# lauradarcy/gym-craftingworld

Hardware: AMD Instinct MI355X
Metric: env-steps/sec at 65536 envs, 1/2/4/8 MI355X; bit-exact vs CPU ref (higher is better)
Workload: dtype u8

## Files before the change

### gym_craftingworld_amd/_lib.py

```python
import ctypes as C
import os

_HERE = os.path.dirname(os.path.abspath(__file__))
LIB_PATH = os.path.join(_HERE, 'libcraftingworld.so')


def lib_path():
    return os.environ.get('CW_LIB_PATH') or LIB_PATH

CW_ABI_VERSION = 5
CW_MT_N = 624
CW_MAX_TASKS = 16
CW_MAX_MENUS = 256

CW_OK, CW_ERR_INVALID, CW_ERR_HIP, CW_ERR_STATE = 0, -1, -2, -3
CW_OBS_STATE, CW_OBS_PIXELS_FULL, CW_OBS_PIXELS_DIRTY = 0, 1, 2
CW_ACT_I32, CW_ACT_I64, CW_ACT_U8 = 0, 1, 2
CW_RASTER_RAY, CW_RASTER_ALT = 0, 1


class cw_task_menu(C.Structure):
    _fields_ = [('n_selected', C.c_int32), ('number_of_tasks', C.c_int32), ('stacking', C.c_int32),
                ('reward_subset', C.c_int32), ('selected_bits', C.c_int32 * CW_MAX_TASKS)]


class cw_config(C.Structure):
    _fields_ = [('abi_version', C.c_int32), ('num_envs', C.c_int32), ('size', C.c_int32),
                ('max_steps', C.c_int32), ('n_task_list', C.c_int32), ('fixed_init_state', C.c_int32),
                ('obs_mode', C.c_int32), ('auto_reset', C.c_int32), ('keep_terminal_obs', C.c_int32),
                ('raster', C.c_int32), ('host_outputs', C.c_int32), ('n_menus', C.c_int32),
                ('menus', C.POINTER(cw_task_menu)), ('env_menu', C.POINTER(C.c_uint8))]


class cw_buffer_table(C.Structure):
    _fields_ = [('obs', C.c_void_p), ('desired_goal', C.c_void_p), ('init_obs', C.c_void_p), ('terminal_obs', C.c_void_p),
                ('reward', C.c_void_p), ('done', C.c_void_p), ('achieved', C.c_void_p),
                ('desired', C.c_void_p), ('episode_length', C.c_void_p), ('episode_return', C.c_void_p), ('hdr', C.c_void_p),
                ('slot_pos', C.c_void_p), ('counters', C.c_void_p), ('frame_bytes', C.c_size_t),
                ('host_actions', C.c_void_p), ('host_onehot', C.c_void_p)]


class cw_state_view(C.Structure):
    _fields_ = [('grid', C.c_void_p), ('init_grid', C.c_void_p), ('goal_grid', C.c_void_p),
                ('agent_rc', C.c_void_p), ('init_agent_rc', C.c_void_p), ('goal_agent_rc', C.c_void_p),
                ('hold', C.c_void_p), ('achieved', C.c_void_p), ('desired', C.c_void_p),
                ('step_num', C.c_void_p), ('ep_no', C.c_void_p)]


class cw_profile(C.Structure):
    _fields_ = [('steps', C.c_int32), ('ms_step_kernel', C.c_float), ('ms_reset_kernel', C.c_float),
                ('ms_render_kernel', C.c_float), ('ms_render_kernel_max', C.c_float), ('ms_render_kernel_min', C.c_float),
                ('ms_render_kernel_median', C.c_float)]


class cw_tuner_state(C.Structure):
    _fields_ = [('period16', C.c_int32), ('period16_head', C.c_int32), ('period16_busy', C.c_int32), ('lookahead', C.c_int32), ('resident', C.c_int32),
                ('guard_slowdowns', C.c_int32)]


_VP = C.c_void_p
ABI = {
    'cw_create': (C.c_int, [C.POINTER(cw_config), C.c_int, C.POINTER(_VP)]),
    'cw_destroy': (C.c_int, [_VP]),
    'cw_seed_mt': (C.c_int, [_VP, _VP, _VP]),
    'cw_seed_int': (C.c_int, [_VP, _VP]),
    'cw_get_mt': (C.c_int, [_VP, _VP, _VP]),
    'cw_generate_fixed_states': (C.c_int, [_VP, _VP]),
    'cw_get_fixed_states': (C.c_int, [_VP, _VP]),
    'cw_reset': (C.c_int, [_VP, _VP]),
    'cw_reset_masked': (C.c_int, [_VP, _VP, _VP]),
    'cw_imagine_masked': (C.c_int, [_VP, _VP, _VP, C.c_int32, _VP, _VP, _VP]),
    'cw_sample_state_masked': (C.c_int, [_VP, _VP, C.c_int32, _VP, _VP]),
    'cw_step': (C.c_int, [_VP, _VP, C.c_int, _VP]),
    'cw_step_many': (C.c_int, [_VP, _VP, C.c_int, C.c_int32, _VP]),
    'cw_rollout': (C.c_int, [_VP, _VP, C.c_int32, _VP, _VP, _VP]),
    'cw_render': (C.c_int, [_VP, _VP, _VP]),
    'cw_render_onehot': (C.c_int, [_VP, _VP, C.c_int32, _VP, _VP]),
    'cw_export_grid': (C.c_int, [_VP, _VP, _VP]),
    'cw_export_onehot': (C.c_int, [_VP, _VP, _VP]),
    'cw_export_onehot_of': (C.c_int, [_VP, C.c_int, _VP, _VP]),
    'cw_get_state': (C.c_int, [_VP, C.POINTER(cw_state_view)]),
    'cw_set_state': (C.c_int, [_VP, C.POINTER(cw_state_view)]),
    'cw_checkpoint_bytes': (C.c_size_t, [_VP]),
    'cw_checkpoint_save': (C.c_int, [_VP, _VP, C.c_size_t]),
    'cw_checkpoint_load': (C.c_int, [_VP, _VP, C.c_size_t]),
    'cw_profile_begin': (C.c_int, [_VP, C.c_int]),
    'cw_profile_end': (C.c_int, [_VP, C.POINTER(cw_profile)]),
    'cw_tuner': (C.c_int, [_VP, C.POINTER(cw_tuner_state)]),
    'cw_step_resident': (C.c_int, [_VP, C.c_int32, C.c_int32]),
    'cw_resident_stop': (C.c_int, [_VP]),
    'cw_render_kernel_name': (C.c_char_p, [_VP]),
    'cw_buffers': (C.c_int, [_VP, C.POINTER(cw_buffer_table)]),
    'cw_synchronize': (C.c_int, [_VP, _VP]),
    'cw_num_envs': (C.c_int, [_VP]),
    'cw_abi_version': (C.c_int, []),
    'cw_last_error': (C.c_char_p, []),
}
class cwh_guard(C.Structure):
    _fields_ = [('rate', C.c_double), ('rate_top', C.c_double), ('ms_sum', C.c_double), ('prev_mean', C.c_double), ('ref_ms', C.c_double),
                ('ref_prev', C.c_double), ('ms_n', C.c_int32), ('late', C.c_int32), ('good', C.c_int32), ('slowdowns', C.c_int32),
                ('probes', C.c_int32), ('probe_need', C.c_int32), ('recover_need', C.c_int32), ('probing', C.c_int32), ('recovering', C.c_int32)]


class cwh_tuning(C.Structure):
    _fields_ = [(f, C.c_int32) for f in ('render_chunk_rounds', 'step_envs_per_wave', 'gather', 'gather_max_size', 'small_frame_bytes',
                                         'small_blocks_per_cu', 'small_launch_mb', 'reset_blocks_per_cu', 'guard', 'verbose', 'lookahead',
                                         'la_period', 'rollout_segment', 'pad')] + \
              [(f, C.c_double) for f in ('head_notch', 'busy_notch', 'period_ns', 'rate_tbs')]


cwh_lookup = C.CFUNCTYPE(_VP, _VP, C.c_char_p)

CWH_GUARD_NONE, CWH_GUARD_SLOWDOWN, CWH_GUARD_TRIAL_UP, CWH_GUARD_TRIAL_KEPT, CWH_GUARD_TRIAL_UNDONE = range(5)
CWH_CKPT_SECTIONS = 22

HOST_HELPERS = {
    'cwh_mt_from_numpy': (C.c_int, [_VP, C.c_int]),
    'cwh_mt_to_numpy': (None, [_VP, C.c_int, _VP]),
    'cwh_mt_init_genrand': (None, [_VP, C.c_uint32]),
    'cwh_mt_untwist': (None, [_VP]),
    'cwh_mt_rewind': (None, [_VP, C.POINTER(C.c_int32), C.c_uint32]),
    'cwh_dlpack_make': (_VP, [_VP, C.c_int, C.c_int, C.c_int, C.c_int, C.POINTER(C.c_int64)]),
    'cwh_slots_to_grid': (None, [_VP, C.c_uint32, C.c_int, _VP]),
    'cwh_ckpt_section_bytes': (C.c_int, [C.c_int64, C.c_int32, C.c_int32, C.POINTER(C.c_size_t), C.POINTER(C.c_uint64)]),
    'cwh_guard_init': (None, [C.POINTER(cwh_guard), C.c_double]),
    'cwh_guard_step': (C.c_int, [C.POINTER(cwh_guard), C.c_double, C.c_double]),
    'cwh_sweep_periods': (None, [C.c_double, C.c_int32, C.c_double, C.c_double, C.POINTER(C.c_int32), C.POINTER(C.c_int32), C.POINTER(C.c_int32)]),
    'cwh_guard_scheduled_ms': (C.c_double, [C.c_double, C.c_int32, C.c_int32, C.c_double]),
    'cwh_la_adapt': (C.c_int32, [C.c_int32, C.c_int32, C.c_uint64, C.POINTER(C.c_int32)]),
    'cwh_read_tuning': (None, [cwh_lookup, _VP, C.POINTER(cwh_tuning)]),
}


def bind_host_helpers(lib):
    for name, (res, args) in HOST_HELPERS.items():
        fn = getattr(lib, name)
        fn.restype = res
        fn.argtypes = args
    return lib

_libs = {}
_lib = None


class CraftingWorldError(RuntimeError):
    pass


def load():
    global _lib
    path = lib_path()
    if path in _libs:
        _lib = _libs[path]
        return _lib
    if not os.path.exists(path):
        raise CraftingWorldError(
            'HIP extension %s is missing; build it (python -c "import __graft_entry__ as g; g.build()"). '
            'There is no CPU fallback.' % path)
    try:
        import torch
    except ImportError:
        pass
    lib = C.CDLL(path)
    for table in (ABI, HOST_HELPERS):
        for name, (res, args) in table.items():
            fn = getattr(lib, name)
            fn.restype = res
            fn.argtypes = args
    if lib.cw_abi_version() != CW_ABI_VERSION:
        raise CraftingWorldError('%s ABI %d != binding %d' % (os.path.basename(path), lib.cw_abi_version(), CW_ABI_VERSION))
    _libs[path] = _lib = lib
    return lib


def check(rc, what, lib=None):
    if rc == CW_OK:
        return
    msg = ((lib or _lib or load()).cw_last_error() or b'').decode(errors='replace')
    if rc == CW_ERR_INVALID:
        raise ValueError('%s: %s' % (what, msg))
    raise CraftingWorldError('%s failed (%d): %s' % (what, rc, msg))
```

### gym_craftingworld_amd/csrc/cw_engine.cpp

```cpp
#include <hip/hip_runtime.h>

#include <cstdarg>
#include <climits>
#include <cstdio>
#include <cstdlib>
#include <cstring>
#include <new>
#include <algorithm>
#include <vector>

#include "../../include/craftingworld.h"
#include "cw_layout.h"
#include "cw_host.h"

extern "C" {
hipError_t cwk_launch_step(const CwParams *P, const CwTuning *T, const void *actions, int act_dtype, int obs_mode, int auto_reset, hipStream_t st,
                           hipEvent_t *ev);
hipError_t cwk_launch_refill(const CwParams *P, const CwTuning *T, int all_envs, hipStream_t st);
hipError_t cwk_launch_reset_all(const CwParams *P, const CwTuning *T, int obs_mode, hipStream_t st);
hipError_t cwk_launch_reset_masked(const CwParams *P, const CwTuning *T, const uint8_t *mask, int obs_mode, hipStream_t st);
hipError_t cwk_launch_imagine_masked(const CwParams *P, const CwTuning *T, const uint8_t *mask, const uint16_t *desired, int commit, int obs_mode,
                                     uint8_t *out_frames, uint8_t *out_onehot, hipStream_t st);
hipError_t cwk_launch_sample_state_masked(const CwParams *P, const CwTuning *T, const uint8_t *mask, int pooled, uint16_t *out_cells, hipStream_t st);
hipError_t cwk_launch_pool(const CwParams *P, const CwTuning *T, hipStream_t st);
hipError_t cwk_launch_seed(const CwParams *P, const uint32_t *seeds_dev, hipStream_t st);
hipError_t cwk_launch_resident(const CwParams *P, CwResident *R, uint32_t seq0, int paint_dirty, unsigned long long idle_ticks,
                               unsigned long long life_ticks, hipStream_t st);
hipError_t cwk_launch_render_onehot(const CwParams *P, const uint8_t *onehot, int n_states, uint16_t *out, hipStream_t st);
hipError_t cwk_launch_render_restore(const CwParams *P, const CwTuning *T, hipStream_t st);
hipError_t cwk_launch_rollout(const CwParams *P, const uint8_t *actions, int T, int32_t *rewards, uint8_t *dones, hipStream_t st);
hipError_t cwk_launch_render_ext(const CwParams *P, const CwTuning *T, uint8_t *out, hipStream_t st);
hipError_t cwk_launch_sweep_calib(const CwParams *P, const CwTuning *T, hipStream_t st);
void cwk_sweep_shape(const CwParams *P, const CwTuning *T, int *n_chunks, int *waves, int *jobs_per_wave);
hipError_t cwk_launch_idle(hipStream_t st);
hipError_t cwk_launch_export(const CwParams *P, const CwTuning *T, uint8_t *out, int onehot, int which, hipStream_t st);
}

#include <time.h>

static thread_local char g_err[512] = "";

static int fail(int code, const char *fmt, ...)
{
    va_list ap;
    va_start(ap, fmt);
    vsnprintf(g_err, sizeof(g_err), fmt, ap);
    va_end(ap);
    return code;
}

#define HIP_TRY(expr)                                                                           \
    do {                                                                                        \
        hipError_t _e = (expr);                                                                 \
        if (_e != hipSuccess)                                                                   \
            return fail(CW_ERR_HIP, "%s failed: %s (%s:%d)", #expr, hipGetErrorString(_e), __FILE__, __LINE__); \
    } while (0)

struct DeviceGuard {
    int prev = -1;
    bool ok = true;
    explicit DeviceGuard(int dev)
    {
        if (hipGetDevice(&prev) != hipSuccess) prev = -1;
        if (prev != dev) ok = (hipSetDevice(dev) == hipSuccess);
    }
    ~DeviceGuard()
    {
        int cur = -1;
        if (prev >= 0 && hipGetDevice(&cur) == hipSuccess && cur != prev) (void)hipSetDevice(prev);
    }
};

struct cw_engine {
    int device = 0;
    int obs_mode = 0;
    int auto_reset = 1;
    bool has_reset = false;
    CwParams P{};
    CwTuning tune{};
    std::vector<void *> allocs;
    std::vector<void *> host_allocs;
    int32_t *host_actions = nullptr;
    std::vector<CwMenuDev> menus;
    uint32_t *seed_scratch = nullptr;
    int n = 0, S = 0, ncell = 0, K = 0;
    CwResident *res = nullptr;
    hipStream_t res_stream = nullptr;
    bool res_running = false;
    uint32_t res_seq = 0;
    hipEvent_t last_work = nullptr;
    bool last_work_set = false;
    unsigned long long res_ticks_per_us = 100;
    std::vector<hipEvent_t> prof_ev;
    bool la_refill_all = false;
    unsigned la_steps = 0;
    unsigned la_period = 16;
    unsigned la_period_max = 16;
    bool la_adaptive = true;
    int rollout_segment = -1;
    unsigned long long *la_feedback = nullptr;
    unsigned long long la_slow_seen = 0;
    int32_t la_quiet = 0;
    bool in_step_many = false;
    bool capturing_now = false;
    int sweep_waves = 1024;
    double sweep_jobs = 0, sweep_rate = 0, sweep_beside_ms = 0;
    bool guard_on = false;
    double head_notch = 0.4, busy_notch = 0.75, tune_period_ns = -1, tune_rate_tbs = -1;
    bool tune_guard = true, tune_lookahead = true, verbose = false;
    enum { GUARD_RING = 32 };
    struct GuardSample { hipEvent_t ev[6]; int period16; } guard_ring[GUARD_RING] = {};
    unsigned guard_head = 0, guard_tail = 0;
    unsigned guard_step = 0;
    cwh_guard guard{};
    int prof_cap = 0, prof_n = 0;
    hipStream_t aux = nullptr;
    hipStream_t work[4] = {nullptr, nullptr, nullptr, nullptr};
    int n_work = 0;
    bool work_overflow = false;
    bool captured = false;
};
static inline bool stream_capturing(hipStream_t st)
{
    hipStreamCaptureStatus cap = hipStreamCaptureStatusNone;
    return hipStreamIsCapturing(st, &cap) == hipSuccess && cap != hipStreamCaptureStatusNone;
}
static inline void note_work(cw_engine *e, hipStream_t st)
{
    for (int i = 0; i < e->n_work; i++) if (e->work[i] == st) return;
    if (e->n_work < 4) e->work[e->n_work++] = st; else e->work_overflow = true;
}
static hipError_t quiesce(cw_engine *e)
{
    bool all = e->work_overflow || e->captured;
    for (int i = 0; i < e->n_work && !all; i++)
        if (hipStreamSynchronize(e->work[i]) != hipSuccess) { (void)hipGetLastError(); all = true; }
    e->n_work = 0;
    e->work_overflow = false;
    if (all) return hipDeviceSynchronize();
    return e->aux ? hipStreamSynchronize(e->aux) : hipSuccess;
}
struct AuxDrain {
    cw_engine *e;
    explicit AuxDrain(cw_engine *e_) : e(e_) {}
    ~AuxDrain() { if (e && e->aux) (void)hipStreamSynchronize(e->aux); }
};
static inline hipError_t aux_copy(cw_engine *e, void *dst, const void *src, size_t bytes, hipMemcpyKind kind)
{
    return bytes ? hipMemcpyAsync(dst, src, bytes, kind, e->aux) : hipSuccess;
}
static int la_period_for(int max_steps) { const int p = max_steps / 4; return p < 8 ? 8 : p > 64 ? 64 : p; }
static void la_adapt(cw_engine *e)
{
    const unsigned long long slow = __atomic_load_n(e->la_feedback, __ATOMIC_RELAXED);
    const unsigned long long delta = slow >= e->la_slow_seen ? slow - e->la_slow_seen : 0;
    e->la_slow_seen = slow;
    e->la_period = (unsigned)cwh_la_adapt((int32_t)e->la_period, (int32_t)e->la_period_max, delta, &e->la_quiet);
}

static int resident_park(cw_engine *e)
{
    if (!e->res_running) return CW_OK;
    const unsigned long long low = __atomic_load_n(&e->res->bell, __ATOMIC_RELAXED) & 0xFFFFFFFFull;
    __atomic_store_n(&e->res->bell, low | (1ull << 32), __ATOMIC_RELEASE);
    HIP_TRY(hipStreamSynchronize(e->res_stream));
    e->res_running = false;
    __atomic_store_n(&e->res->bell, low, __ATOMIC_RELEASE);
    __atomic_store_n(&e->res->exited, 0u, __ATOMIC_RELEASE);
    return CW_OK;
}
#define PARK(e) do { if ((e)->res_running) { const int _rc = resident_park(e); if (_rc != CW_OK) return _rc; } } while (0)


template <typename T>
static int dev_alloc(cw_engine *e, T **out, size_t count)
{
    void *p = nullptr;
    size_t bytes = count * sizeof(T);
    if (bytes == 0) bytes = 16;
    HIP_TRY(hipMalloc(&p, bytes));
    HIP_TRY(hipMemset(p, 0, bytes));
    e->allocs.push_back(p);
    *out = (T *)p;
    return CW_OK;
}

template <typename T>
static int host_alloc(cw_engine *e, T **out, size_t count)
{
    void *p = nullptr, *d = nullptr;
    size_t bytes = count * sizeof(T);
    if (bytes == 0) bytes = 16;
    HIP_TRY(hipHostMalloc(&p, bytes, hipHostMallocCoherent));
    e->host_allocs.push_back(p);
    memset(p, 0, bytes);
    HIP_TRY(hipHostGetDevicePointer(&d, p, 0));
    if (d != p) return fail(CW_ERR_HIP, "cw_create: mapped host memory has a different device address (no unified addressing)");
    *out = (T *)p;
    return CW_OK;
}

static void prof_free(cw_engine *e)
{
    for (hipEvent_t ev : e->prof_ev) (void)hipEventDestroy(ev);
    e->prof_ev.clear();
    e->prof_cap = e->prof_n = 0;
}

static int timed_render_stats(cw_engine *e, double *median, double *p90, double *mean = nullptr)
{
    enum { LAUNCHES = 24, SKIP = 4 };
    hipEvent_t evs[2 * LAUNCHES] = {};
    bool ok = true;
    for (hipEvent_t &ev : evs) ok = ok && hipEventCreate(&ev) == hipSuccess;
    for (int rep = 0; rep < LAUNCHES && ok; rep++)
        ok = hipEventRecord(evs[2 * rep], e->aux) == hipSuccess && cwk_launch_sweep_calib(&e->P, &e->tune, e->aux) == hipSuccess &&
             hipEventRecord(evs[2 * rep + 1], e->aux) == hipSuccess && cwk_launch_idle(e->aux) == hipSuccess;
    ok = ok && hipStreamSynchronize(e->aux) == hipSuccess;
    float ms[LAUNCHES];
    for (int rep = 0; rep < LAUNCHES && ok; rep++) ok = hipEventElapsedTime(&ms[rep], evs[2 * rep], evs[2 * rep + 1]) == hipSuccess;
    for (hipEvent_t &ev : evs) if (ev) (void)hipEventDestroy(ev);
    if (!ok) return fail(CW_ERR_HIP, "cw_create: render calibration failed");
    std::sort(ms + SKIP, ms + LAUNCHES);
    const int n = LAUNCHES - SKIP;
    *median = ms[SKIP + n / 2];
    *p90 = ms[SKIP + (9 * n) / 10 - 1];
    if (mean) { double acc = 0; for (int i = SKIP; i < LAUNCHES; i++) acc += ms[i]; *mean = acc / n; }
    return CW_OK;
}

static double sweep_period_ns(const cw_engine *e, double tb_per_s) { return (double)e->sweep_waves * 4096.0 / (tb_per_s * 1e12) * 1e9; }
static void set_sweep_rate(cw_engine *e, double tb_per_s)
{
    cwh_sweep_periods(tb_per_s, e->sweep_waves, e->head_notch, e->busy_notch, &e->tune.period16, &e->tune.period16_head, &e->tune.period16_busy);
}

static int calibrate_sweep(cw_engine *e)
{
    CwTuning &tn = e->tune;
    int n_chunks = 1, jobs_per_wave = 1;
    cwk_sweep_shape(&e->P, &tn, &n_chunks, &e->sweep_waves, &jobs_per_wave);
    e->sweep_jobs = (double)n_chunks * jobs_per_wave;
    if (e->tune_period_ns >= 0) {
        const double ns = e->tune_period_ns;
        set_sweep_rate(e, ns > 0 ? (double)e->sweep_waves * 4096.0 / (ns * 1e-9) * 1e-12 : 0.0);
        if (ns > 0) tn.period16 = (int)(ns * 1.6 + 0.5);
        return CW_OK;
    }
    set_sweep_rate(e, 7.0);
    if (e->host_actions) { set_sweep_rate(e, 0); return CW_OK; }
    if (e->obs_mode != CW_OBS_PIXELS_FULL || (double)e->n * e->P.frame_bytes < (double)(64ll << 20)) return CW_OK;
    static const double rates[] = {7.7, 7.4, 7.2, 7.0, 6.8, 6.6, 0.0};
    char log[1024] = "";
    size_t len = 0;
    int rc = CW_OK;
    double best_p90 = 0, med = 0, p90 = 0, mean = 0;
    rc = timed_render_stats(e, &med, &p90);
    set_sweep_rate(e, 6.4);
    if (rc == CW_OK) rc = timed_render_stats(e, &med, &p90);
    e->sweep_beside_ms = med - e->sweep_jobs * sweep_period_ns(e, 6.4) * 1e-6;
    if (e->tune_rate_tbs >= 0) e->sweep_rate = e->tune_rate_tbs;
    for (size_t i = 0; i < sizeof(rates) / sizeof(rates[0]) && rc == CW_OK && e->tune_rate_tbs < 0; i++) {
        set_sweep_rate(e, rates[i]);
        rc = timed_render_stats(e, &med, &p90, &mean);
        if (len < sizeof(log) - 56) len += (size_t)snprintf(log + len, sizeof(log) - len, " %.1f TB/s (%.0f ns): %.4f/%.4f/%.4f |", rates[i], tn.period16 / 1.6, med, p90, mean);
        if (rc == CW_OK && (best_p90 == 0 || p90 < 0.995 * best_p90)) { best_p90 = p90; e->sweep_rate = rates[i]; }
    }
    set_sweep_rate(e, e->sweep_rate);
    cwh_guard_init(&e->guard, e->sweep_rate);
    e->guard_on = rc == CW_OK && e->sweep_rate > 0 && e->auto_reset && e->tune_guard;
    if (e->guard_on)
        for (auto &smp : e->guard_ring)
            for (hipEvent_t &ev : smp.ev)
                if (hipEventCreate(&ev) != hipSuccess) e->guard_on = false;
    if (e->verbose)
        fprintf(stderr, "[craftingworld] sweep clock, ms per sweep (median/90th percentile/mean of 20; 0.0 TB/s = unclocked):%s -> %s%.0f ns\n", log,
                tn.period16 ? "" : "unclocked, ", tn.period16 / 1.6);
    return rc;
}

enum { CW_GUARD_EVERY = 64 };
static hipEvent_t *sweep_guard_tick(cw_engine *e, hipStream_t st)
{
    if (++e->guard_step % CW_GUARD_EVERY) return nullptr;
    while (e->guard_tail != e->guard_head && hipEventQuery(e->guard_ring[e->guard_tail % cw_engine::GUARD_RING].ev[5]) == hipSuccess) {
        cw_engine::GuardSample &smp = e->guard_ring[e->guard_tail++ % cw_engine::GUARD_RING];
        float ms = 0.f;
        if (hipEventElapsedTime(&ms, smp.ev[4], smp.ev[5]) != hipSuccess || ms <= 0.f || smp.period16 != e->tune.period16) continue;
        const double scheduled = cwh_guard_scheduled_ms(e->sweep_jobs, e->tune.period16, e->tune.period16_busy, e->sweep_beside_ms);
        const double rate_before = e->guard.rate, prev_mean = e->guard.prev_mean;
        const int recovering = e->guard.recovering;
        const int action = cwh_guard_step(&e->guard, ms, scheduled);
        if (e->guard.rate != rate_before) set_sweep_rate(e, e->guard.rate);
        if (e->verbose && action != CWH_GUARD_NONE) {
            static const char *what[] = {"", "three samples in a row late: a notch down", "trying a notch up", "the trial pays: kept", "the trial does not pay: undone"};
            fprintf(stderr, "[craftingworld] sweep clock: %s%s -- %.4f ms against %.4f scheduled (mean at the rate left %.4f): %.1f -> %.1f TB/s (%.0f ns)\n", what[action],
                    recovering ? " (on the way back to the best rate known)" : "", ms, scheduled, prev_mean, rate_before, e->guard.rate, e->tune.period16 / 1.6);
        }
    }
    if (e->guard_head - e->guard_tail >= (unsigned)cw_engine::GUARD_RING) return nullptr;
    cw_engine::GuardSample &slot = e->guard_ring[e->guard_head++ % cw_engine::GUARD_RING];
    slot.period16 = e->tune.period16;
    return slot.ev;
}

static void read_tuning(cw_engine *e)
{
    CwTuning &tn = e->tune;
    cwh_tuning t{};
    t.render_chunk_rounds = tn.render_chunk_rounds;
    t.step_envs_per_wave = tn.step_envs_per_wave;
    t.gather = tn.gather;
    t.gather_max_size = tn.gather_max_size;
    t.small_frame_bytes = tn.small_frame_bytes;
    t.small_blocks_per_cu = tn.small_blocks_per_cu;
    t.small_launch_mb = (int32_t)(tn.small_launch_bytes >> 20);
    t.reset_blocks_per_cu = tn.reset_blocks_per_cu;
    t.guard = 1;
    t.verbose = 0;
    t.lookahead = 1;
    t.la_period = 0;
    t.rollout_segment = e->rollout_segment;
    t.head_notch = e->head_notch;
    t.busy_notch = e->busy_notch;
    t.period_ns = -1;
    t.rate_tbs = -1;
    cwh_read_tuning([](void *, const char *k) -> const char * { return getenv(k); }, nullptr, &t);
    tn.render_chunk_rounds = t.render_chunk_rounds;
    tn.step_envs_per_wave = t.step_envs_per_wave;
    tn.gather = t.gather;
    tn.gather_max_size = t.gather_max_size;
    tn.small_frame_bytes = t.small_frame_bytes;
    tn.small_blocks_per_cu = t.small_blocks_per_cu;
    tn.small_launch_bytes = (long long)t.small_launch_mb << 20;
    tn.reset_blocks_per_cu = t.reset_blocks_per_cu;
    e->head_notch = t.head_notch;
    e->busy_notch = t.busy_notch;
    e->tune_period_ns = t.period_ns;
    e->tune_rate_tbs = t.rate_tbs;
    e->tune_guard = t.guard != 0;
    e->verbose = t.verbose != 0;
    e->tune_lookahead = t.lookahead != 0;
    e->la_adaptive = t.la_period == 0;
    e->la_period = e->la_period_max = (unsigned)(t.la_period ? t.la_period : la_period_for(e->P.max_steps));
    e->rollout_segment = t.rollout_segment;
}

extern "C" {

const char *cw_last_error(void) { return g_err; }
int cw_abi_version(void) { return CW_ABI_VERSION; }
int cw_num_envs(const cw_engine *e) { return e ? e->n : 0; }

int cw_create(const cw_config *cfg, int device, cw_engine **out)
{
    if (!cfg || !out) return fail(CW_ERR_INVALID, "cw_create: null argument");
    *out = nullptr;
    if (cfg->abi_version != CW_ABI_VERSION)
        return fail(CW_ERR_INVALID, "cw_create: abi_version %d != %d", cfg->abi_version, CW_ABI_VERSION);
    if (cfg->num_envs < 1) return fail(CW_ERR_INVALID, "cw_create: num_envs must be >= 1");
    if (cfg->size < 4 || cfg->size > 255)
        return fail(CW_ERR_INVALID, "cw_create: size must be in 4..255 (square grids only; non-square is a reference defect)");
    if (cfg->max_steps < 1 || cfg->max_steps > 65535) return fail(CW_ERR_INVALID, "cw_create: max_steps must be in 1..65535");
    if (cfg->n_task_list < 9 || cfg->n_task_list > CW_MAX_TASKS)
        return fail(CW_ERR_INVALID, "cw_create: len(task_list) must be in 9..%d", CW_MAX_TASKS);
    if (cfg->fixed_init_state < 0 || cfg->fixed_init_state > 64)
        return fail(CW_ERR_INVALID, "cw_create: fixed_init_state must be in 0..64");
    if (cfg->obs_mode < CW_OBS_STATE || cfg->obs_mode > CW_OBS_PIXELS_DIRTY) return fail(CW_ERR_INVALID, "cw_create: bad obs_mode");
    if (cfg->raster != CW_RASTER_RAY && cfg->raster != CW_RASTER_ALT) return fail(CW_ERR_INVALID, "cw_create: bad raster");
    if (cfg->n_menus < 1 || cfg->n_menus > CW_MAX_MENUS || !cfg->menus) return fail(CW_ERR_INVALID, "cw_create: n_menus must be in 1..%d", CW_MAX_MENUS);
    if ((double)cfg->num_envs * 48.0 * cfg->size * cfg->size > 1.0e12)
        return fail(CW_ERR_INVALID, "cw_create: num_envs x frame size exceeds 1 TB");

    std::vector<CwMenuDev> menus(cfg->n_menus);
    for (int m = 0; m < cfg->n_menus; m++) {
        const cw_task_menu &src = cfg->menus[m];
        if (src.n_selected < 1 || src.n_selected > CW_MAX_TASKS)
            return fail(CW_ERR_INVALID, "cw_create: menu %d: len(selected_tasks) must be in 1..%d", m, CW_MAX_TASKS);
        if (src.number_of_tasks < 1) return fail(CW_ERR_INVALID, "cw_create: menu %d: number_of_tasks must be >= 1", m);
        CwMenuDev d{};
        d.n_selected = src.n_selected;
        d.number_of_tasks = src.number_of_tasks > src.n_selected ? src.n_selected : src.number_of_tasks;
        d.stacking = src.stacking ? 1 : 0;
        d.reward_subset = src.reward_subset ? 1 : 0;
        for (int i = 0; i < src.n_selected; i++) {
            if (src.selected_bits[i] < 0 || src.selected_bits[i] >= cfg->n_task_list)
                return fail(CW_ERR_INVALID, "cw_create: menu %d: selected task %d is not in task_list", m, i);
            d.sel_bits |= (uint64_t)src.selected_bits[i] << (4 * i);
        }
        menus[m] = d;
    }
    if (cfg->env_menu)
        for (int i = 0; i < cfg->num_envs; i++)
            if (cfg->env_menu[i] >= cfg->n_menus) return fail(CW_ERR_INVALID, "cw_create: env_menu[%d] out of range", i);

    int ndev = 0;
    HIP_TRY(hipGetDeviceCount(&ndev));
    if (device < 0 || device >= ndev) return fail(CW_ERR_INVALID, "cw_create: device %d not present (%d devices)", device, ndev);
    DeviceGuard guard(device);
    if (!guard.ok) return fail(CW_ERR_HIP, "cw_create: hipSetDevice(%d) failed", device);

    cw_engine *e = new (std::nothrow) cw_engine();
    if (!e) return fail(CW_ERR_INVALID, "cw_create: out of host memory");
    e->device = device;
    e->obs_mode = cfg->obs_mode;
    e->auto_reset = cfg->auto_reset ? 1 : 0;
    e->n = cfg->num_envs;
    e->S = cfg->size;
    e->ncell = cfg->size * cfg->size;
    e->K = cfg->fixed_init_state;
    e->menus = menus;
    CwParams &P = e->P;
    const size_t N = (size_t)e->n;
    P.n_envs = e->n;
    P.size = e->S;
    P.ncell = e->ncell;
    P.max_steps = cfg->max_steps;
    read_tuning(e);
    hipDeviceProp_t prop;
    if (hipGetDeviceProperties(&prop, device) == hipSuccess && prop.multiProcessorCount > 0) e->tune.n_cu = prop.multiProcessorCount;
    P.task_mask = (1u << cfg->n_task_list) - 1u;
    P.pool_k = e->K;
    P.div_magic = (uint32_t)((1ull << 32) / (uint64_t)e->S) + 1u;
    P.raster = cfg->raster;
    P.frame_bytes = cfg->raster == CW_RASTER_ALT ? 27u * (uint32_t)e->S * (uint32_t)(e->S + 1) : 48u * (uint32_t)e->ncell;

    int rc = CW_OK;
#define ALLOC(field, count)                                     \
    if (rc == CW_OK) rc = dev_alloc(e, &P.field, (count))
    ALLOC(hdr, N);
    ALLOC(pos, N);
    ALLOC(init_pos, N);
    ALLOC(init_agent, N);
    ALLOC(goal_pos, N);
    ALLOC(goal_codes, N);
    ALLOC(goal_agent, N);
    ALLOC(ep_no, N);
    ALLOC(mt, N * CW_MT_N);
    ALLOC(mt_idx, N);
    ALLOC(pool, N * (size_t)e->K * 9);
    if (rc == CW_OK) rc = dev_alloc(e, &e->seed_scratch, N);
#define ALLOC_OUT(field, count)                                 \
    if (rc == CW_OK) rc = cfg->host_outputs ? host_alloc(e, &P.field, (count)) : dev_alloc(e, &P.field, (count))
    ALLOC_OUT(reward, N);
    ALLOC_OUT(done, N);
    ALLOC_OUT(achieved_out, N);
    ALLOC_OUT(desired_out, N);
    ALLOC_OUT(episode_length, N);
    ALLOC_OUT(episode_return, N);
    ALLOC(counters, 8);
    if (rc == CW_OK) {
        int pr_least = 0, pr_greatest = 0;
        if (hipDeviceGetStreamPriorityRange(&pr_least, &pr_greatest) != hipSuccess) pr_least = pr_greatest = 0;
        if (hipStreamCreateWithPriority(&e->aux, hipStreamNonBlocking, pr_greatest) != hipSuccess &&
            hipStreamCreateWithFlags(&e->aux, hipStreamNonBlocking) != hipSuccess)
            rc = fail(CW_ERR_HIP, "cw_create: no private stream");
    }
    if (cfg->obs_mode != CW_OBS_STATE) {
        ALLOC_OUT(obs, N * P.frame_bytes);
        ALLOC_OUT(desired_img, N * P.frame_bytes);
        ALLOC_OUT(init_img, N * P.frame_bytes);
        if (cfg->keep_terminal_obs && cfg->auto_reset) ALLOC_OUT(terminal_img, N * P.frame_bytes);
    }
    if (cfg->host_outputs && rc == CW_OK) rc = host_alloc(e, &e->host_actions, N);
    P.lookahead = (cfg->auto_reset && !cfg->host_outputs && e->tune_lookahead) ? 1 : 0;
    ALLOC(nx_init_pos, P.lookahead ? N * CW_LA_DEPTH : 1);
    ALLOC(nx_goal_pos, P.lookahead ? N * CW_LA_DEPTH : 1);
    ALLOC(nx_misc, P.lookahead ? N * CW_LA_DEPTH : 1);
    ALLOC(nx_ctl, P.lookahead ? N : 1);
    if (rc == CW_OK && P.lookahead && e->la_adaptive) {
        void *fb = nullptr;
        if (hipHostMalloc(&fb, 64, hipHostMallocCoherent) == hipSuccess) {
            memset(fb, 0, 64);
            e->host_allocs.push_back(fb);
            e->la_feedback = P.la_feedback = (unsigned long long *)fb;
        }
    }
#undef ALLOC_OUT
#undef ALLOC
    CwMenuDev *dmenus = nullptr;
    if (rc == CW_OK) rc = dev_alloc(e, &dmenus, menus.size());
    if (rc == CW_OK && hipMemcpy(dmenus, menus.data(), menus.size() * sizeof(CwMenuDev), hipMemcpyHostToDevice) != hipSuccess)
        rc = fail(CW_ERR_HIP, "cw_create: menu upload failed");
    P.menus = dmenus;
    if (rc == CW_OK) {
        std::vector<uint32_t> h(N * 4, 0u);
        for (size_t i = 0; i < N; i++) {
            h[i * 4 + 0] = (uint32_t)(cfg->env_menu ? cfg->env_menu[i] : 0) << 24;
            h[i * 4 + 3] = CW_CODES_INITIAL;
        }
        if (hipMemcpy(P.hdr, h.data(), h.size() * 4, hipMemcpyHostToDevice) != hipSuccess)
            rc = fail(CW_ERR_HIP, "cw_create: header upload failed");
    }
    if (rc != CW_OK) {
        if (e->aux) (void)hipStreamDestroy(e->aux);
        for (void *p : e->allocs) (void)hipFree(p);
        for (void *p : e->host_allocs) (void)hipHostFree(p);
        delete e;
        return rc;
    }
    if (cfg->host_outputs && e->n == 1 && !e->auto_reset && e->obs_mode != CW_OBS_PIXELS_FULL) {
        void *p = nullptr;
        if (hipHostMalloc(&p, sizeof(CwResident), hipHostMallocCoherent) == hipSuccess &&
            hipStreamCreateWithFlags(&e->res_stream, hipStreamNonBlocking) == hipSuccess) {
            memset(p, 0, sizeof(CwResident));
            e->host_allocs.push_back(p);
            e->res = (CwResident *)p;
            if (host_alloc(e, &e->P.res_onehot, (size_t)e->ncell * 12) != CW_OK) e->P.res_onehot = nullptr;
            int khz = 0;
            if (hipDeviceGetAttribute(&khz, hipDeviceAttributeWallClockRate, device) == hipSuccess && khz >= 1000) e->res_ticks_per_us = (unsigned long long)khz / 1000ull;
            if (hipEventCreateWithFlags(&e->last_work, hipEventDisableTiming) != hipSuccess) {
                e->last_work = nullptr;
                e->res = nullptr;
            }
        } else {
            if (p) (void)hipHostFree(p);
            e->res_stream = nullptr;
        }
    }
    *out = e;
    std::vector<uint32_t> seeds(N);
    for (size_t i = 0; i < N; i++) seeds[i] = (uint32_t)i;
    rc = cw_seed_int(e, seeds.data());
    if (rc == CW_OK) rc = calibrate_sweep(e);
    if (rc != CW_OK) {
        cw_destroy(e);
        *out = nullptr;
    }
    return rc;
}

int cw_destroy(cw_engine *e)
{
    if (!e) return CW_OK;
    DeviceGuard guard(e->device);
    if (!guard.ok) return fail(CW_ERR_HIP, "hipSetDevice(%d) failed", e->device);
    PARK(e);
    (void)resident_park(e);
    (void)quiesce(e);
    prof_free(e);
    if (e->aux) (void)hipStreamDestroy(e->aux);
    if (e->res_stream) (void)hipStreamDestroy(e->res_stream);
    if (e->last_work) (void)hipEventDestroy(e->last_work);
    for (auto &smp : e->guard_ring) for (hipEvent_t ev : smp.ev) if (ev) (void)hipEventDestroy(ev);
    for (void *p : e->allocs) (void)hipFree(p);
    for (void *p : e->host_allocs) (void)hipHostFree(p);
    delete e;
    return CW_OK;
}

static hipError_t lookahead_drop(cw_engine *e)
{
    if (!e->P.lookahead) return hipSuccess;
    hipError_t rc = hipMemsetAsync(e->P.nx_misc, 0, (size_t)e->n * CW_LA_DEPTH * sizeof(uint4), e->aux);
    if (rc == hipSuccess) rc = hipMemsetAsync(e->P.nx_ctl, 0, (size_t)e->n * sizeof(uint32_t), e->aux);
    e->la_refill_all = true;
    return rc;
}

int cw_seed_mt(cw_engine *e, const uint32_t *keys, const int32_t *pos)
{
    if (!e || !keys || !pos) return fail(CW_ERR_INVALID, "cw_seed_mt: null argument");
    DeviceGuard guard(e->device);
    if (!guard.ok) return fail(CW_ERR_HIP, "hipSetDevice(%d) failed", e->device);
    PARK(e);
    const size_t N = (size_t)e->n;
    for (size_t i = 0; i < N; i++)
        if (pos[i] < 0 || pos[i] > CW_MT_N) return fail(CW_ERR_INVALID, "cw_seed_mt: pos[%zu]=%d outside 0..624", i, pos[i]);
    HIP_TRY(quiesce(e));
    AuxDrain drain(e);
    HIP_TRY(aux_copy(e, e->P.mt, keys, N * CW_MT_N * sizeof(uint32_t), hipMemcpyHostToDevice));
    HIP_TRY(aux_copy(e, e->P.mt_idx, pos, N * sizeof(int32_t), hipMemcpyHostToDevice));
    HIP_TRY(cwk_launch_seed(&e->P, nullptr, e->aux));
    HIP_TRY(lookahead_drop(e));
    HIP_TRY(hipStreamSynchronize(e->aux));
    return CW_OK;
}

int cw_seed_int(cw_engine *e, const uint32_t *seeds)
{
    if (!e || !seeds) return fail(CW_ERR_INVALID, "cw_seed_int: null argument");
    DeviceGuard guard(e->device);
    if (!guard.ok) return fail(CW_ERR_HIP, "hipSetDevice(%d) failed", e->device);
    PARK(e);
    HIP_TRY(quiesce(e));
    AuxDrain drain(e);
    HIP_TRY(aux_copy(e, e->seed_scratch, seeds, (size_t)e->n * sizeof(uint32_t), hipMemcpyHostToDevice));
    HIP_TRY(cwk_launch_seed(&e->P, e->seed_scratch, e->aux));
    HIP_TRY(lookahead_drop(e));
    HIP_TRY(hipStreamSynchronize(e->aux));
    return CW_OK;
}

int cw_get_mt(cw_engine *e, uint32_t *keys, int32_t *pos)
{
    if (!e || !keys || !pos) return fail(CW_ERR_INVALID, "cw_get_mt: null argument");
    DeviceGuard guard(e->device);
    if (!guard.ok) return fail(CW_ERR_HIP, "hipSetDevice(%d) failed", e->device);
    PARK(e);
    const size_t N = (size_t)e->n;
    std::vector<uint32_t> words(N * CW_MT_N);
    std::vector<uint32_t> misc(e->P.lookahead ? N * 4 * CW_LA_DEPTH : 0);
    HIP_TRY(quiesce(e));
    AuxDrain drain(e);
    HIP_TRY(aux_copy(e, words.data(), e->P.mt, words.size() * sizeof(uint32_t), hipMemcpyDeviceToHost));
    HIP_TRY(aux_copy(e, pos, e->P.mt_idx, N * sizeof(int32_t), hipMemcpyDeviceToHost));
    if (e->P.lookahead) HIP_TRY(aux_copy(e, misc.data(), e->P.nx_misc, N * 16 * CW_LA_DEPTH, hipMemcpyDeviceToHost));
    HIP_TRY(hipStreamSynchronize(e->aux));
    for (size_t i = 0; i < N; i++) cwh_mt_to_numpy(&words[i * CW_MT_N], pos[i], keys + i * CW_MT_N);
    if (e->P.lookahead) {
        for (size_t i = 0; i < N; i++) {
            uint32_t ahead = 0;
            for (size_t d = 0; d < CW_LA_DEPTH; d++)
                if (misc[(d * N + i) * 4 + 2] >> 31) ahead += misc[(d * N + i) * 4 + 3];
            if (ahead) cwh_mt_rewind(keys + i * CW_MT_N, &pos[i], ahead);
        }
    }
    for (size_t i = 0; i < N; i++)
        if (pos[i] == 0) { cwh_mt_untwist(keys + i * CW_MT_N); pos[i] = CW_MT_N; }
    return CW_OK;
}

int cw_generate_fixed_states(cw_engine *e, cw_stream_t stream)
{
    if (!e) return fail(CW_ERR_INVALID, "cw_generate_fixed_states: null engine");
    if (e->K == 0) return CW_OK;
    DeviceGuard guard(e->device);
// ... 19 lines not shown
    PARK(e);
    note_work(e, (hipStream_t)stream);
    HIP_TRY(cwk_launch_reset_all(&e->P, &e->tune, e->obs_mode, (hipStream_t)stream));
    if (e->P.lookahead) {
        HIP_TRY(cwk_launch_refill(&e->P, &e->tune, 1, (hipStream_t)stream));
        e->la_refill_all = false;
        e->la_steps = 0;
    }
    e->has_reset = true;
    if (e->res && hipEventRecord(e->last_work, (hipStream_t)stream) == hipSuccess) e->last_work_set = true;
    return CW_OK;
}

int cw_reset_masked(cw_engine *e, const uint8_t *mask, cw_stream_t stream)
{
    if (!e || !mask) return fail(CW_ERR_INVALID, "cw_reset_masked: null %s", !e ? "engine" : "mask");
    if (!e->has_reset) return fail(CW_ERR_STATE, "cw_reset_masked called before cw_reset");
    DeviceGuard guard(e->device);
    if (!guard.ok) return fail(CW_ERR_HIP, "hipSetDevice(%d) failed", e->device);
    PARK(e);
    if (stream_capturing((hipStream_t)stream)) e->captured = true; else note_work(e, (hipStream_t)stream);
    HIP_TRY(cwk_launch_reset_masked(&e->P, &e->tune, mask, e->obs_mode, (hipStream_t)stream));
    if (e->res && hipEventRecord(e->last_work, (hipStream_t)stream) == hipSuccess) e->last_work_set = true;
    return CW_OK;
}

static int rewind_streams(cw_engine *e, hipStream_t st, const char *who)
{
    if (!e->P.lookahead) return CW_OK;
    if (stream_capturing(st)) return fail(CW_ERR_STATE, "%s: an engine that keeps look-ahead records rewinds its streams through the host and cannot be captured", who);
    std::vector<uint32_t> keys((size_t)e->n * CW_MT_N);
    std::vector<int32_t> pos((size_t)e->n);
    int rc = cw_get_mt(e, keys.data(), pos.data());
    if (rc == CW_OK) rc = cw_seed_mt(e, keys.data(), pos.data());
    return rc;
}

int cw_imagine_masked(cw_engine *e, const uint8_t *mask, const uint16_t *desired, int32_t commit, uint8_t *out_frames, uint8_t *out_onehot,
                      cw_stream_t stream)
{
    if (!e) return fail(CW_ERR_INVALID, "cw_imagine_masked: null engine");
    if (!commit && !out_frames && !out_onehot) return fail(CW_ERR_INVALID, "cw_imagine_masked: commit == 0 and no output pointer: nothing to do");
    if (!e->has_reset) return fail(CW_ERR_STATE, "cw_imagine_masked called before cw_reset");
    DeviceGuard guard(e->device);
    if (!guard.ok) return fail(CW_ERR_HIP, "hipSetDevice(%d) failed", e->device);
    PARK(e);
    const int rc = rewind_streams(e, (hipStream_t)stream, "cw_imagine_masked");
    if (rc != CW_OK) return rc;
    if (stream_capturing((hipStream_t)stream)) e->captured = true; else note_work(e, (hipStream_t)stream);
    HIP_TRY(cwk_launch_imagine_masked(&e->P, &e->tune, mask, desired, commit != 0, e->obs_mode, out_frames, out_onehot, (hipStream_t)stream));
    if (e->res && hipEventRecord(e->last_work, (hipStream_t)stream) == hipSuccess) e->last_work_set = true;
    return CW_OK;
}

int cw_sample_state_masked(cw_engine *e, const uint8_t *mask, int32_t pooled, uint16_t *out_cells, cw_stream_t stream)
{
    if (!e || !out_cells) return fail(CW_ERR_INVALID, "cw_sample_state_masked: null %s", !e ? "engine" : "out_cells");
    if (pooled && e->K == 0) return fail(CW_ERR_INVALID, "cw_sample_state_masked: pooled with fixed_init_state == 0");
    if (!e->has_reset) return fail(CW_ERR_STATE, "cw_sample_state_masked called before cw_reset");
    DeviceGuard guard(e->device);
    if (!guard.ok) return fail(CW_ERR_HIP, "hipSetDevice(%d) failed", e->device);
    PARK(e);
    const int rc = rewind_streams(e, (hipStream_t)stream, "cw_sample_state_masked");
    if (rc != CW_OK) return rc;
    if (stream_capturing((hipStream_t)stream)) e->captured = true; else note_work(e, (hipStream_t)stream);
    HIP_TRY(cwk_launch_sample_state_masked(&e->P, &e->tune, mask, pooled != 0, out_cells, (hipStream_t)stream));
    if (e->res && hipEventRecord(e->last_work, (hipStream_t)stream) == hipSuccess) e->last_work_set = true;
    return CW_OK;
}

int cw_step(cw_engine *e, const void *actions, int action_dtype, cw_stream_t stream)
{
    if (!e || !actions) return fail(CW_ERR_INVALID, "cw_step: null argument");
    if (action_dtype < CW_ACT_I32 || action_dtype > CW_ACT_U8) return fail(CW_ERR_INVALID, "cw_step: bad action dtype %d", action_dtype);
    if (!e->has_reset) return fail(CW_ERR_STATE, "cw_step called before cw_reset");
    DeviceGuard guard(e->device);
    if (!guard.ok) return fail(CW_ERR_HIP, "hipSetDevice(%d) failed", e->device);
    PARK(e);
    const bool capturing = e->in_step_many ? e->capturing_now : stream_capturing((hipStream_t)stream);
    if (capturing) e->captured = true;
    else if (e->n_work != 1 || e->work[0] != (hipStream_t)stream) note_work(e, (hipStream_t)stream);
    hipEvent_t *ev = (e->prof_n < e->prof_cap) ? &e->prof_ev[(size_t)e->prof_n * 6] : nullptr;
    const bool profiled = ev != nullptr;
    if (e->guard_on && !ev && !capturing) ev = sweep_guard_tick(e, (hipStream_t)stream);
    if (capturing && e->P.lookahead && !e->la_refill_all && e->la_steps + 1 < e->la_period && !e->in_step_many) e->la_steps = e->la_period;
    if (e->P.lookahead && (e->la_refill_all || ++e->la_steps >= e->la_period)) {
        if (e->la_feedback && !capturing) la_adapt(e);
        HIP_TRY(cwk_launch_refill(&e->P, &e->tune, e->la_refill_all ? 1 : 0, (hipStream_t)stream));
        e->la_refill_all = false;
        e->la_steps = 0;
    }
    HIP_TRY(cwk_launch_step(&e->P, &e->tune, actions, action_dtype, e->obs_mode, e->auto_reset, (hipStream_t)stream, ev));
    if (profiled) e->prof_n++;
    if (e->res && hipEventRecord(e->last_work, (hipStream_t)stream) == hipSuccess) e->last_work_set = true;
    return CW_OK;
}

int cw_step_many(cw_engine *e, const void *actions, int action_dtype, int32_t n_steps, cw_stream_t stream)
{
    if (!e || !actions) return fail(CW_ERR_INVALID, "cw_step_many: null argument");
    if (n_steps < 1) return fail(CW_ERR_INVALID, "cw_step_many: n_steps must be >= 1");
    if (action_dtype < CW_ACT_I32 || action_dtype > CW_ACT_U8) return fail(CW_ERR_INVALID, "cw_step_many: bad action dtype %d", action_dtype);
    e->capturing_now = stream_capturing((hipStream_t)stream);
    if (e->P.lookahead && e->capturing_now) e->la_steps = e->la_period;
    const size_t row = (size_t)e->n * (action_dtype == CW_ACT_I32 ? 4 : action_dtype == CW_ACT_I64 ? 8 : 1);
    e->in_step_many = true;
    int rc = CW_OK;
    for (int32_t t = 0; t < n_steps && rc == CW_OK; t++) rc = cw_step(e, (const unsigned char *)actions + (size_t)t * row, action_dtype, stream);
    e->in_step_many = false;
    return rc;
}

int cw_step_resident(cw_engine *e, int32_t action, int32_t want_onehot)
{
    if (!e) return fail(CW_ERR_INVALID, "cw_step_resident: null engine");
    if (!e->res) return fail(CW_ERR_INVALID, "cw_step_resident needs num_envs == 1, host_outputs, auto_reset == 0 and obs_mode state or pixels_dirty");
    if (!e->has_reset) return fail(CW_ERR_STATE, "cw_step_resident called before cw_reset");
    if (action < 0 || action > 127) return fail(CW_ERR_INVALID, "cw_step_resident: action %d outside 0..127", action);
    if (want_onehot && !e->P.res_onehot) return fail(CW_ERR_INVALID, "cw_step_resident: no host one-hot buffer on this engine");
    CwResident *R = e->res;
    const uint32_t seq = (++e->res_seq) & 0xFFFFFFu;
    __atomic_store_n(&R->bell, (unsigned long long)((seq << 8) | (want_onehot ? 0x80u : 0u) | (uint32_t)action), __ATOMIC_RELEASE);
    struct timespec t0;
    clock_gettime(CLOCK_MONOTONIC, &t0);
    for (unsigned spins = 0;; spins++) {
        if (e->res_running && __atomic_load_n(&R->ack, __ATOMIC_ACQUIRE) == seq) return CW_OK;
        if (!e->res_running || __atomic_load_n(&R->exited, __ATOMIC_ACQUIRE) != 0) {
            DeviceGuard guard(e->device);
            if (!guard.ok) return fail(CW_ERR_HIP, "hipSetDevice(%d) failed", e->device);
            if (e->res_running) HIP_TRY(hipStreamSynchronize(e->res_stream));
            e->res_running = false;
            if (__atomic_load_n(&R->ack, __ATOMIC_ACQUIRE) == seq) {
                __atomic_store_n(&R->exited, 0u, __ATOMIC_RELEASE);
                return CW_OK;
            }
            if (e->last_work_set) { HIP_TRY(hipStreamWaitEvent(e->res_stream, e->last_work, 0)); e->last_work_set = false; }
            __atomic_store_n(&R->exited, 0u, __ATOMIC_RELEASE);
            __atomic_store_n(&R->ack, (seq - 1u) & 0xFFFFFFu, __ATOMIC_RELEASE);
            HIP_TRY(cwk_launch_resident(&e->P, R, (seq - 1u) & 0xFFFFFFu, e->obs_mode == CW_OBS_PIXELS_DIRTY ? 1 : 0,
                                        500ull * e->res_ticks_per_us , 200000ull * e->res_ticks_per_us , e->res_stream));
            e->res_running = true;
            continue;
        }
        __builtin_ia32_pause();
        if ((spins & 1023u) == 1023u) {
            struct timespec t1;
            clock_gettime(CLOCK_MONOTONIC, &t1);
            if ((t1.tv_sec - t0.tv_sec) + 1e-9 * (t1.tv_nsec - t0.tv_nsec) > 5.0) {
                const uint32_t acked = __atomic_load_n(&R->ack, __ATOMIC_ACQUIRE);
                __atomic_store_n(&R->bell, (1ull << 32) | ((unsigned long long)acked << 8), __ATOMIC_RELEASE);
                const hipError_t he = hipStreamSynchronize(e->res_stream);
                e->res_running = false;
                const uint32_t now_acked = __atomic_load_n(&R->ack, __ATOMIC_ACQUIRE);
                __atomic_store_n(&R->bell, (unsigned long long)now_acked << 8, __ATOMIC_RELEASE);
                __atomic_store_n(&R->exited, 0u, __ATOMIC_RELEASE);
                e->res_seq = now_acked;
                if (he == hipSuccess && now_acked == seq) return CW_OK;
                return fail(CW_ERR_HIP, "cw_step_resident: no answer from the resident kernel within 5 s (request withdrawn, kernel parked: the step was not taken)");
            }
        }
    }
}

int cw_resident_stop(cw_engine *e)
{
    if (!e) return fail(CW_ERR_INVALID, "cw_resident_stop: null engine");
    DeviceGuard guard(e->device);
// ... 64 lines not shown

int cw_export_onehot(cw_engine *e, uint8_t *out, cw_stream_t stream)
{
    if (!e || !out) return fail(CW_ERR_INVALID, "cw_export_onehot: null argument");
    DeviceGuard guard(e->device);
    if (!guard.ok) return fail(CW_ERR_HIP, "hipSetDevice(%d) failed", e->device);
    PARK(e);
    note_work(e, (hipStream_t)stream);
    HIP_TRY(cwk_launch_export(&e->P, &e->tune, out, 1, 0, (hipStream_t)stream));
    return CW_OK;
}

int cw_export_onehot_of(cw_engine *e, int which, uint8_t *out, cw_stream_t stream)
{
    if (!e || !out) return fail(CW_ERR_INVALID, "cw_export_onehot_of: null argument");
    if (which < CW_STATE_CURRENT || which > CW_STATE_INIT) return fail(CW_ERR_INVALID, "cw_export_onehot_of: which must be CW_STATE_*");
    if (!e->has_reset) return fail(CW_ERR_STATE, "cw_export_onehot_of called before cw_reset");
    DeviceGuard guard(e->device);
    if (!guard.ok) return fail(CW_ERR_HIP, "hipSetDevice(%d) failed", e->device);
    PARK(e);
    note_work(e, (hipStream_t)stream);
    HIP_TRY(cwk_launch_export(&e->P, &e->tune, out, 1, which, (hipStream_t)stream));
    return CW_OK;
}

int cw_profile_begin(cw_engine *e, int max_steps)
{
    if (!e || max_steps < 1 || max_steps > 100000) return fail(CW_ERR_INVALID, "cw_profile_begin: bad argument");
    DeviceGuard guard(e->device);
    if (!guard.ok) return fail(CW_ERR_HIP, "hipSetDevice(%d) failed", e->device);
    PARK(e);
    prof_free(e);
    e->prof_ev.resize((size_t)max_steps * 6);
    for (auto &ev : e->prof_ev) HIP_TRY(hipEventCreate(&ev));
    e->prof_cap = max_steps;
    return CW_OK;
}

int cw_profile_end(cw_engine *e, cw_profile *out)
{
    if (!e || !out) return fail(CW_ERR_INVALID, "cw_profile_end: null argument");
    DeviceGuard guard(e->device);
    if (!guard.ok) return fail(CW_ERR_HIP, "hipSetDevice(%d) failed", e->device);
    PARK(e);
    memset(out, 0, sizeof(*out));
    const int n = e->prof_n;
    if (n > 0) {
        const bool side_recorded = e->obs_mode != CW_OBS_PIXELS_FULL;
        for (int k = 0; k < 6; k++)
            if (side_recorded || k >= 4) HIP_TRY(hipEventSynchronize(e->prof_ev[(size_t)(n - 1) * 6 + k]));
        double acc[3] = {0, 0, 0};
        float rmax = 0.f, rmin = 1e30f;
        std::vector<float> render_ms;
        render_ms.reserve((size_t)n);
        for (int i = 0; i < n; i++)
            for (int k = 0; k < 3; k++) {
                if (k != 2 && !side_recorded) continue;
                float ms = 0.f;
                HIP_TRY(hipEventElapsedTime(&ms, e->prof_ev[(size_t)i * 6 + 2 * k], e->prof_ev[(size_t)i * 6 + 2 * k + 1]));
                acc[k] += ms;
                if (k == 2) { rmax = ms > rmax ? ms : rmax; rmin = ms < rmin ? ms : rmin; render_ms.push_back(ms); }
            }
        out->steps = n;
        out->ms_step_kernel = (float)(acc[0] / n);
        out->ms_reset_kernel = (float)(acc[1] / n);
        out->ms_render_kernel = (float)(acc[2] / n);
        out->ms_render_kernel_max = rmax;
        out->ms_render_kernel_min = rmin;
        std::sort(render_ms.begin(), render_ms.end());
        out->ms_render_kernel_median = render_ms.empty() ? 0.f : render_ms[render_ms.size() / 2];
    }
    prof_free(e);
    return CW_OK;
}

const char *cw_render_kernel_name(const cw_engine *e)
{
    if (!e || e->obs_mode == CW_OBS_STATE) return "";
    if (e->obs_mode == CW_OBS_PIXELS_DIRTY) return e->auto_reset ? "cw_step_fused_kernel" : "cw_step_kernel";
    if (e->tune.gather && e->P.raster == CW_RASTER_RAY && e->S <= e->tune.gather_max_size) return "cw_render_gather_kernel";
    return "cw_render_pieces_kernel";
}

int cw_tuner(const cw_engine *e, cw_tuner_state *out)
{
    if (!e || !out) return fail(CW_ERR_INVALID, "cw_tuner: null argument");
    out->period16 = e->tune.period16;
    out->period16_head = e->tune.period16_head;
    out->period16_busy = e->tune.period16_busy;
    out->lookahead = e->P.lookahead;
    out->resident = e->res ? 1 : 0;
    out->guard_slowdowns = e->guard_on ? e->guard.slowdowns : -1;
    return CW_OK;
}

int cw_buffers(cw_engine *e, cw_buffer_table *out)
{
    if (!e || !out) return fail(CW_ERR_INVALID, "cw_buffers: null argument");
    const CwParams &P = e->P;
    out->obs = P.obs;
    out->desired_goal = P.desired_img;
    out->init_obs = P.init_img;
    out->terminal_obs = P.terminal_img;
    out->reward = P.reward;
    out->done = P.done;
    out->achieved = P.achieved_out;
    out->desired = P.desired_out;
    out->episode_length = P.episode_length;
    out->episode_return = P.episode_return;
    out->hdr = (uint8_t *)P.hdr;
    out->slot_pos = (uint16_t *)P.pos;
    out->counters = (uint64_t *)P.counters;
    out->frame_bytes = P.frame_bytes;
    out->host_actions = e->host_actions;
    out->host_onehot = P.res_onehot;
    return CW_OK;
}

int cw_synchronize(cw_engine *e, cw_stream_t stream)
{
    if (!e) return fail(CW_ERR_INVALID, "cw_synchronize: null engine");
    DeviceGuard guard(e->device);
    if (!guard.ok) return fail(CW_ERR_HIP, "hipSetDevice(%d) failed", e->device);
    PARK(e);
    HIP_TRY(hipStreamSynchronize((hipStream_t)stream));
    for (int i = 0; i < e->n_work; i++)
        if (e->work[i] == (hipStream_t)stream) { e->work[i] = e->work[--e->n_work]; break; }
    return CW_OK;
}

int cw_get_fixed_states(cw_engine *e, uint16_t *out)
{
    if (!e || !out) return fail(CW_ERR_INVALID, "cw_get_fixed_states: null argument");
    if (e->K == 0) return fail(CW_ERR_INVALID, "cw_get_fixed_states: the engine was created with fixed_init_state = 0");
    DeviceGuard guard(e->device);
    if (!guard.ok) return fail(CW_ERR_HIP, "hipSetDevice(%d) failed", e->device);
    PARK(e);
    HIP_TRY(quiesce(e));
    AuxDrain drain(e);
    HIP_TRY(aux_copy(e, out, e->P.pool, (size_t)e->n * e->K * 9 * sizeof(uint16_t), hipMemcpyDeviceToHost));
    HIP_TRY(hipStreamSynchronize(e->aux));
    return CW_OK;
}

int cw_get_state(cw_engine *e, cw_state_view *v)
{
    if (!e || !v) return fail(CW_ERR_INVALID, "cw_get_state: null argument");
    DeviceGuard guard(e->device);
    if (!guard.ok) return fail(CW_ERR_HIP, "hipSetDevice(%d) failed", e->device);
    PARK(e);
    const size_t N = (size_t)e->n;
    const int S = e->S, nc = e->ncell;
    std::vector<uint32_t> hdr(N * 4), goal_codes(N);
    std::vector<uint16_t> pos(N * 8), ipos(N * 8), gpos(N * 8), iagent(N), gagent(N);
    std::vector<int32_t> epno(N);
    HIP_TRY(quiesce(e));
    AuxDrain drain(e);
    HIP_TRY(aux_copy(e, hdr.data(), e->P.hdr, N * 16, hipMemcpyDeviceToHost));
    HIP_TRY(aux_copy(e, pos.data(), e->P.pos, N * 16, hipMemcpyDeviceToHost));
    HIP_TRY(aux_copy(e, ipos.data(), e->P.init_pos, N * 16, hipMemcpyDeviceToHost));
    HIP_TRY(aux_copy(e, gpos.data(), e->P.goal_pos, N * 16, hipMemcpyDeviceToHost));
    HIP_TRY(aux_copy(e, goal_codes.data(), e->P.goal_codes, N * 4, hipMemcpyDeviceToHost));
    HIP_TRY(aux_copy(e, iagent.data(), e->P.init_agent, N * 2, hipMemcpyDeviceToHost));
    HIP_TRY(aux_copy(e, gagent.data(), e->P.goal_agent, N * 2, hipMemcpyDeviceToHost));
    HIP_TRY(aux_copy(e, epno.data(), e->P.ep_no, N * 4, hipMemcpyDeviceToHost));
    HIP_TRY(hipStreamSynchronize(e->aux));
    for (size_t i = 0; i < N; i++) {
        const uint32_t *h = &hdr[i * 4];
        if (v->grid) cwh_slots_to_grid(&pos[i * 8], h[3], nc, v->grid + i * nc);
        if (v->init_grid) cwh_slots_to_grid(&ipos[i * 8], CW_CODES_INITIAL, nc, v->init_grid + i * nc);
        if (v->goal_grid) cwh_slots_to_grid(&gpos[i * 8], goal_codes[i], nc, v->goal_grid + i * nc);
        if (v->agent_rc) { v->agent_rc[i * 2] = h[0] & 0xFF; v->agent_rc[i * 2 + 1] = (h[0] >> 8) & 0xFF; }
        if (v->init_agent_rc) { v->init_agent_rc[i * 2] = (uint8_t)(iagent[i] / S); v->init_agent_rc[i * 2 + 1] = (uint8_t)(iagent[i] % S); }
        if (v->goal_agent_rc) { v->goal_agent_rc[i * 2] = (uint8_t)(gagent[i] / S); v->goal_agent_rc[i * 2 + 1] = (uint8_t)(gagent[i] % S); }
        if (v->hold) v->hold[i] = (h[0] >> 16) & 0xFF;
// ... 275 lines not shown
```

### gym_craftingworld_amd/csrc/cw_host.cpp

```cpp
#include "cw_host.h"

#include <algorithm>
#include <cerrno>
#include <climits>
#include <cmath>
#include <cstdlib>
#include <cstring>

static inline uint32_t mt_twist(uint32_t cur, uint32_t nxt, uint32_t far)
{
    const uint32_t y = (cur & 0x80000000u) | (nxt & 0x7fffffffu);
    return far ^ (y >> 1) ^ ((y & 1u) ? 0x9908b0dfu : 0u);
}

extern "C" {

int cwh_mt_from_numpy(uint32_t *s, int pos)
{
    if (pos < 0) pos = 0;
    if (pos > CWH_MT_N) pos = CWH_MT_N;
    for (int k = 0; k < pos; k++)
        s[k] = mt_twist(s[k], s[(k + 1) % CWH_MT_N], s[(k + 397) % CWH_MT_N]);
    return pos % CWH_MT_N;
}
// ... 25 lines not shown
    memset(prev, 0, sizeof(prev));
    for (int k = CWH_MT_N - 1; k >= 0; k--) {
        uint32_t t = key[k] ^ (k == CWH_MT_N - 1 ? key[396] : k >= CWH_MT_N - 397 ? key[k - (CWH_MT_N - 397)] : prev[k + 397]);
        const uint32_t odd = t >> 31;
        if (odd) t ^= 0x9908b0dfu;
        const uint32_t y = (t << 1) | odd;
        prev[k] |= y & 0x80000000u;
        if (k == CWH_MT_N - 1) key[0] = (key[0] & 0x80000000u) | (y & 0x7fffffffu);
        else prev[k + 1] |= y & 0x7fffffffu;
    }
    uint32_t t = prev[CWH_MT_N - 1] ^ prev[396];
    const uint32_t odd = t >> 31;
    if (odd) t ^= 0x9908b0dfu;
    prev[0] |= ((t << 1) | odd) & 0x7fffffffu;
    memcpy(key, prev, sizeof(prev));
}
void cwh_mt_rewind(uint32_t *key, int32_t *pos, uint32_t n)
{
    while (n > 0) {
        if ((uint32_t)*pos >= n) { *pos -= (int32_t)n; n = 0; }
        else { n -= (uint32_t)*pos; cwh_mt_untwist(key); *pos = CWH_MT_N; }
    }
}

struct CwDLDevice { int32_t device_type, device_id; };
struct CwDLDataType { uint8_t code, bits; uint16_t lanes; };
struct CwDLTensor { void *data; CwDLDevice device; int32_t ndim; CwDLDataType dtype; int64_t *shape, *strides; uint64_t byte_offset; };
struct CwDLManagedTensor { CwDLTensor dl_tensor; void *manager_ctx; void (*deleter)(CwDLManagedTensor *); };

static void cw_dl_deleter(CwDLManagedTensor *m)
{
    if (!m) return;
    free(m->dl_tensor.shape);
    free(m);
}

void *cwh_dlpack_make(void *data, int device_id, int code, int bits, int ndim, const int64_t *shape)
{
    CwDLManagedTensor *m = (CwDLManagedTensor *)calloc(1, sizeof(CwDLManagedTensor));
    int64_t *shp = (int64_t *)malloc(sizeof(int64_t) * (size_t)(ndim > 0 ? ndim : 1));
    if (!m || !shp) { free(m); free(shp); return nullptr; }
    for (int i = 0; i < ndim; i++) shp[i] = shape[i];
    m->dl_tensor.data = data;
    m->dl_tensor.device = CwDLDevice{10, device_id};
    m->dl_tensor.ndim = ndim;
    m->dl_tensor.dtype = CwDLDataType{(uint8_t)code, (uint8_t)bits, 1};
    m->dl_tensor.shape = shp;
    m->dl_tensor.strides = nullptr;
    m->dl_tensor.byte_offset = 0;
    m->deleter = cw_dl_deleter;
    return m;
}

void cwh_mt_init_genrand(uint32_t *s, uint32_t seed)
{
    s[0] = seed;
    for (int i = 1; i < CWH_MT_N; i++) s[i] = 1812433253u * (s[i - 1] ^ (s[i - 1] >> 30)) + (uint32_t)i;
}

}


extern "C" {

void cwh_slots_to_grid(const uint16_t *pos, uint32_t codes, int ncell, uint8_t *grid)
{
    memset(grid, 0, (size_t)ncell);
    for (int k = 0; k < 8; k++)
        if (pos[k] < (uint32_t)ncell) grid[pos[k]] = (uint8_t)((codes >> (4 * k)) & 15u);
}

int cwh_ckpt_section_bytes(int64_t n, int32_t k, int32_t la_depth, size_t *sizes, uint64_t *total)
{
    const size_t N = n > 0 ? (size_t)n : 0, K = k > 0 ? (size_t)k : 0, D = la_depth > 0 ? (size_t)la_depth : 0, la = D ? 1 : 0;
    const size_t sz[CWH_CKPT_SECTIONS] = {N * 16, N * 16, N * 16, N * 16, N * 4, N * 2, N * 2, N * 4, N * CWH_MT_N * 4, N * 4, N * K * 9 * 2,
                                          N * 4, N, N * 2, N * 2, N * 4, N * 4, 5 * 8,
                                          D * N * 16, D * N * 16, D * N * 16, la * N * 4};
    uint64_t sum = 0;
    for (int i = 0; i < CWH_CKPT_SECTIONS; i++) { if (sizes) sizes[i] = sz[i]; sum += sz[i]; }
    if (total) *total = sum;
    return CWH_CKPT_SECTIONS;
}

static double period_ns(int32_t sweep_waves, double tb_per_s) { return (double)sweep_waves * 4096.0 / (tb_per_s * 1e12) * 1e9; }
void cwh_sweep_periods(double rate, int32_t sweep_waves, double head_notch, double busy_notch, int32_t *period16, int32_t *period16_head, int32_t *period16_busy)
{
    const double head = rate - head_notch > CWH_GUARD_RATE_FLOOR ? rate - head_notch : CWH_GUARD_RATE_FLOOR;
    const double busy = rate - busy_notch > CWH_GUARD_RATE_FLOOR ? rate - busy_notch : CWH_GUARD_RATE_FLOOR;
    *period16 = rate > 0 ? (int32_t)(period_ns(sweep_waves, rate) * 1.6 + 0.5) : 0;
    *period16_head = rate > 0 ? (int32_t)(period_ns(sweep_waves, head) * 1.6 + 0.5) : 0;
    *period16_busy = rate > 0 ? (int32_t)(period_ns(sweep_waves, busy) * 1.6 + 0.5) : 0;
}
double cwh_guard_scheduled_ms(double sweep_jobs, int32_t period16, int32_t period16_busy, double beside_ms)
{
    return (sweep_jobs * (period16 / 1.6) + CWH_HEAD_JOBS * ((period16_busy - period16) / 1.6)) * 1e-6 + beside_ms;
}

static void guard_set_rate(cwh_guard *g, double rate)
{
    g->rate = rate;
    g->ms_sum = 0;
    g->ms_n = 0;
    g->good = g->late = 0;
    g->ref_ms = 0;
}
void cwh_guard_init(cwh_guard *g, double rate)
{
    memset(g, 0, sizeof(*g));
    g->rate = g->rate_top = rate;
    g->probe_need = CWH_GUARD_RECOVER;
    g->recover_need = CWH_GUARD_RECOVER;
}
int cwh_guard_step(cwh_guard *g, double ms, double scheduled)
{
    const double ref = std::max(scheduled, g->probing ? g->prev_mean : g->ref_ms);
    const bool late = ms > (g->probing ? 1.15 : 1.06) * ref;
    g->late = late ? g->late + 1 : 0;
    g->good = late ? std::max(0, g->good - 8) : g->good + 1;
    if (g->ms_n >= 128) { g->ms_sum *= 0.5; g->ms_n /= 2; }
    g->ms_sum += ms;
    g->ms_n++;
    const bool verdict_due = g->probing && g->ms_n >= CWH_GUARD_PROBE_SAMPLES;
    const double mean = g->ms_sum / g->ms_n;
    if (g->probing && (g->late >= 3 || (verdict_due && mean >= 0.998 * g->prev_mean))) {
        const double ref_prev = g->ref_prev;
        guard_set_rate(g, g->rate - CWH_GUARD_NOTCH);
        g->ref_ms = ref_prev;
        int32_t &need = g->recovering ? g->recover_need : g->probe_need;
        need = std::min(2 * need, (int32_t)CWH_GUARD_NEED_MAX);
        g->probing = g->recovering = 0;
        return CWH_GUARD_TRIAL_UNDONE;
    }
    if (verdict_due) {
        if (g->recovering) g->recover_need = CWH_GUARD_RECOVER;
        else { g->rate_top = g->rate; g->probe_need = CWH_GUARD_RECOVER / 4; }
        g->ref_ms = mean;
        g->probing = g->recovering = 0;
        return CWH_GUARD_TRIAL_KEPT;
    }
    if (!g->probing && g->late >= 3 && g->rate > CWH_GUARD_RATE_FLOOR + 0.1) {
        guard_set_rate(g, g->rate - CWH_GUARD_NOTCH);
        g->slowdowns++;
        return CWH_GUARD_SLOWDOWN;
    }
    if (!g->probing && g->ms_n >= CWH_GUARD_PROBE_SAMPLES && g->rate + 0.05 < CWH_GUARD_RATE_CEILING &&
        g->good >= (g->rate + 0.1 < g->rate_top ? g->recover_need : g->probe_need)) {
        g->recovering = g->rate + 0.1 < g->rate_top;
        g->prev_mean = mean;
        g->ref_prev = g->ref_ms;
        guard_set_rate(g, std::min(g->rate + CWH_GUARD_NOTCH, CWH_GUARD_RATE_CEILING));
        g->probing = 1;
        if (!g->recovering) g->probes++;
        return CWH_GUARD_TRIAL_UP;
    }
    return CWH_GUARD_NONE;
}

int32_t cwh_la_adapt(int32_t period, int32_t period_max, uint64_t slow_delta, int32_t *quiet)
{
    if (slow_delta * 8ull > (uint64_t)period) {
        *quiet = 0;
        if (period > CWH_LA_PERIOD_MIN) period = period / 2 < CWH_LA_PERIOD_MIN ? CWH_LA_PERIOD_MIN : period / 2;
    } else if (slow_delta * 32ull <= (uint64_t)period && ++*quiet >= CWH_LA_QUIET) {
        *quiet = 0;
        if (period < period_max) period = period * 2 > period_max ? period_max : period * 2;
    }
    return period;
}

}

static bool tail_is_blank(const char *end)
{
    while (*end == ' ' || (*end >= '\t' && *end <= '\r')) end++;
    return *end == '\0';
}
static void tune_int(cwh_lookup lookup, void *ctx, const char *name, int32_t *field, long lo, long hi)
{
    const char *s = lookup(ctx, name);
    if (!s) return;
    char *end = nullptr;
    errno = 0;
    const long v = strtol(s, &end, 10);
    if (end == s || errno == ERANGE || !tail_is_blank(end) || v < lo || v > hi) return;
    *field = (int32_t)v;
}
static void tune_real(cwh_lookup lookup, void *ctx, const char *name, double *field, double lo)
{
    const char *s = lookup(ctx, name);
    if (!s) return;
    char *end = nullptr;
    errno = 0;
    const double v = strtod(s, &end);
    if (end == s || errno == ERANGE || !tail_is_blank(end) || !std::isfinite(v) || v < lo) return;
    *field = v;
}

extern "C" void cwh_read_tuning(cwh_lookup lookup, void *ctx, cwh_tuning *t)
{
    tune_int(lookup, ctx, "CW_TUNE_RENDER_CHUNK_ROUNDS", &t->render_chunk_rounds, 0, INT32_MAX);
    int32_t epw = t->step_envs_per_wave;
    tune_int(lookup, ctx, "CW_TUNE_STEP_ENVS_PER_WAVE", &epw, 8, 64);
    if (epw == 8 || epw == 16 || epw == 32 || epw == 64) t->step_envs_per_wave = epw;
    tune_int(lookup, ctx, "CW_TUNE_GATHER", &t->gather, INT32_MIN, INT32_MAX);
    tune_int(lookup, ctx, "CW_TUNE_GATHER_MAX_SIZE", &t->gather_max_size, 0, 9);
    tune_int(lookup, ctx, "CW_TUNE_SMALL_FRAME_BYTES", &t->small_frame_bytes, 0, INT32_MAX);
    tune_int(lookup, ctx, "CW_TUNE_SMALL_BLOCKS", &t->small_blocks_per_cu, 1, 8);
    tune_int(lookup, ctx, "CW_TUNE_SMALL_LAUNCH_MB", &t->small_launch_mb, 0, INT32_MAX);
    tune_int(lookup, ctx, "CW_TUNE_RESET_BLOCKS", &t->reset_blocks_per_cu, 1, 16);
    tune_real(lookup, ctx, "CW_TUNE_HEAD_NOTCH", &t->head_notch, 0);
    tune_real(lookup, ctx, "CW_TUNE_BUSY_NOTCH", &t->busy_notch, 0);
    tune_real(lookup, ctx, "CW_TUNE_PERIOD_NS", &t->period_ns, 0);
    tune_real(lookup, ctx, "CW_TUNE_RATE_TBS", &t->rate_tbs, 0);
    tune_int(lookup, ctx, "CW_TUNE_GUARD", &t->guard, INT32_MIN, INT32_MAX);
    t->guard = t->guard != 0;
    if (lookup(ctx, "CW_TUNE_VERBOSE")) t->verbose = 1;
    tune_int(lookup, ctx, "CW_TUNE_LOOKAHEAD", &t->lookahead, INT32_MIN, INT32_MAX);
    t->lookahead = t->lookahead != 0;
    tune_int(lookup, ctx, "CW_TUNE_LA_PERIOD", &t->la_period, 1, INT32_MAX);
    tune_int(lookup, ctx, "CW_TUNE_ROLLOUT_SEGMENT", &t->rollout_segment, -1, INT32_MAX);
}
```

### gym_craftingworld_amd/csrc/cw_host.h

```cpp
#pragma once
#include <stddef.h>
#include <stdint.h>

#define CWH_MT_N 624

#ifdef __cplusplus
extern "C" {
#endif

int cwh_mt_from_numpy(uint32_t *s, int pos);
void cwh_mt_to_numpy(const uint32_t *s, int idx, uint32_t *key);
void cwh_mt_untwist(uint32_t *key);
void cwh_mt_rewind(uint32_t *key, int32_t *pos, uint32_t n);
void cwh_mt_init_genrand(uint32_t *s, uint32_t seed);

void *cwh_dlpack_make(void *data, int device_id, int code, int bits, int ndim, const int64_t *shape);

void cwh_slots_to_grid(const uint16_t *pos, uint32_t codes, int ncell, uint8_t *grid);

#define CWH_CKPT_SECTIONS 22
int cwh_ckpt_section_bytes(int64_t n, int32_t k, int32_t la_depth, size_t *sizes, uint64_t *total);

typedef struct cwh_guard {
    double rate;
    double rate_top;
    double ms_sum;
    double prev_mean;
    double ref_ms;
    double ref_prev;
    int32_t ms_n;
    int32_t late;
    int32_t good;
    int32_t slowdowns;
    int32_t probes;
    int32_t probe_need;
    int32_t recover_need;
    int32_t probing;
    int32_t recovering;
} cwh_guard;

enum { CWH_GUARD_NONE = 0, CWH_GUARD_SLOWDOWN = 1, CWH_GUARD_TRIAL_UP = 2, CWH_GUARD_TRIAL_KEPT = 3, CWH_GUARD_TRIAL_UNDONE = 4 };
#define CWH_GUARD_RECOVER 64
#define CWH_GUARD_PROBE_SAMPLES 32
#define CWH_GUARD_NEED_MAX 2048
#define CWH_GUARD_RATE_FLOOR 5.0
#define CWH_GUARD_RATE_CEILING 7.7
#define CWH_GUARD_NOTCH 0.2

void cwh_guard_init(cwh_guard *g, double rate);
int cwh_guard_step(cwh_guard *g, double ms, double scheduled_ms);
#define CWH_HEAD_JOBS 64
void cwh_sweep_periods(double rate, int32_t sweep_waves, double head_notch, double busy_notch, int32_t *period16, int32_t *period16_head, int32_t *period16_busy);
double cwh_guard_scheduled_ms(double sweep_jobs, int32_t period16, int32_t period16_busy, double beside_ms);

#define CWH_LA_PERIOD_MIN 8
#define CWH_LA_QUIET 8
int32_t cwh_la_adapt(int32_t period, int32_t period_max, uint64_t slow_delta, int32_t *quiet);

typedef struct cwh_tuning {
    int32_t render_chunk_rounds;
    int32_t step_envs_per_wave;
    int32_t gather;
    int32_t gather_max_size;
    int32_t small_frame_bytes;
    int32_t small_blocks_per_cu;
    int32_t small_launch_mb;
    int32_t reset_blocks_per_cu;
    int32_t guard;
    int32_t verbose;
    int32_t lookahead;
    int32_t la_period;
    int32_t rollout_segment;
    int32_t pad;
    double head_notch;
    double busy_notch;
    double period_ns;
    double rate_tbs;
} cwh_tuning;
typedef const char *(*cwh_lookup)(void *ctx, const char *name);
void cwh_read_tuning(cwh_lookup lookup, void *ctx, cwh_tuning *t);

#ifdef __cplusplus
}
#endif
```

### gym_craftingworld_amd/csrc/cw_kernels.hip

```cpp
#include <hip/hip_runtime.h>
#include <stdint.h>

#include "cw_layout.h"
#include "cw_mt.h"

#define CW_WAVE 64
#define CW_BALLOT(p) __builtin_amdgcn_ballot_w64(p)
#define CW_ALT_FRAME_PACE 2

#ifdef CW_TRACE
__device__ unsigned long long cw_trace_buf[1024 * 8];
#define CW_STAMP(env, k) do { if (lane == 0) { cw_trace_buf[((env) & 1023) * 8 + (k)] = wall_clock64(); \
                                               if ((k) == 0 || (k) == 5) cw_trace_buf[((env) & 1023) * 8 + 6 + ((k) ? 1 : 0)] = clock64(); } } while (0)
extern "C" hipError_t cwk_trace_read(unsigned long long *dst) { return hipMemcpyFromSymbol(dst, HIP_SYMBOL(cw_trace_buf), sizeof(cw_trace_buf)); }
#else
#define CW_STAMP(env, k) do { } while (0)
#endif

enum { EMPTY = 0, STICKS = 1, AXE = 2, HAMMER = 3, ROCK = 4, TREE = 5, BREAD = 6, HOUSE = 7, WHEAT = 8 };
enum { T_MAKEBREAD = 0, T_EATBREAD = 1, T_BUILDHOUSE = 2, T_CHOPTREE = 3, T_CHOPROCK = 4,
       T_GOTOHOUSE = 5, T_MOVEAXE = 6, T_MOVEHAMMER = 7, T_MOVESTICKS = 8 };

typedef uint32_t u32x3 __attribute__((ext_vector_type(3)));
typedef u32x3 u32x3_a4 __attribute__((aligned(4)));

__device__ __forceinline__ void unpack_pos(const uint4 &v, uint32_t sp[8])
{
    sp[0] = v.x & 0xFFFFu; sp[1] = v.x >> 16;
    sp[2] = v.y & 0xFFFFu; sp[3] = v.y >> 16;
    sp[4] = v.z & 0xFFFFu; sp[5] = v.z >> 16;
    sp[6] = v.w & 0xFFFFu; sp[7] = v.w >> 16;
}
__device__ __forceinline__ uint4 pack_pos(const uint32_t sp[8])
{
    return make_uint4(sp[0] | (sp[1] << 16), sp[2] | (sp[3] << 16), sp[4] | (sp[5] << 16), sp[6] | (sp[7] << 16));
}
__device__ __forceinline__ int slot_at(const uint32_t sp[8], uint32_t cell)
{
    int idx = -1;
#pragma unroll
    for (int k = 0; k < 8; k++) idx = (sp[k] == cell) ? k : idx;
    return idx;
}
__device__ __forceinline__ uint32_t code_of(uint32_t codes, int idx)
{
    return idx < 0 ? 0u : ((codes >> (4 * idx)) & 15u);
}
__device__ __forceinline__ uint32_t rgb_of_code(uint32_t code)
{
    uint32_t c = 0;
    c = code == 1 ? (110u | (69u << 8) | (39u << 16)) : c;
    c = code == 2 ? (255u | (105u << 8) | (180u << 16)) : c;
    c = code == 3 ? (100u | (100u << 8) | (200u << 16)) : c;
    c = code == 4 ? (100u | (100u << 8) | (100u << 16)) : c;
    c = code == 5 ? (0u | (128u << 8) | (0u << 16)) : c;
    c = code == 6 ? (205u | (133u << 8) | (63u << 16)) : c;
    c = code == 7 ? (197u | (91u << 8) | (97u << 16)) : c;
    c = code == 8 ? (240u | (230u << 8) | (140u << 16)) : c;
    return c;
}

__device__ __forceinline__ u32x3 cell_row_dwords(uint32_t rgb)
{
    u32x3 d;
    d.x = rgb | (rgb << 24);
    d.y = (rgb >> 8) | (rgb << 16);
    d.z = (rgb >> 16) | (rgb << 8);
    return d;
}
__device__ __forceinline__ u32x3 overlay_dwords(u32x3 d, uint32_t o)
{
    d.x = (d.x & 0x00FFFFFFu) | (o << 24);
    d.y = (o >> 8) | (o << 16);
    d.z = (d.z & 0xFFFFFF00u) | (o >> 16);
    return d;
}
__device__ __forceinline__ u32x3 onehot_dwords(uint32_t bits)
{
    u32x3 d;
    d.x = (bits & 1u) | ((bits >> 1 & 1u) << 8) | ((bits >> 2 & 1u) << 16) | ((bits >> 3 & 1u) << 24);
    d.y = (bits >> 4 & 1u) | ((bits >> 5 & 1u) << 8) | ((bits >> 6 & 1u) << 16) | ((bits >> 7 & 1u) << 24);
    d.z = (bits >> 8 & 1u) | ((bits >> 9 & 1u) << 8) | ((bits >> 10 & 1u) << 16) | ((bits >> 11 & 1u) << 24);
    return d;
}

__device__ __forceinline__ void paint_cell(uint8_t *frame, int S, uint32_t cell, uint32_t code,
                                           bool agent_here, uint32_t hold, uint32_t div_magic, bool mark_rows_only = false)
{
    const uint32_t r = __umulhi(cell, div_magic);
// ... 587 lines not shown
#pragma unroll
    for (int k = 0; k < 8; k++) {
        fp[k] = __builtin_amdgcn_readlane(v_fp, k);
        goal_codes |= __builtin_amdgcn_readlane(v_fc, k) << (4 * k);
    }
    goal_pos = pack_pos(fp);
}

template <typename MenuFn>
__device__ __forceinline__ CwResetOut reset_env_wave(const CwParams &P, int env, MenuFn menu_fn, uint32_t *lds_mt, int lane)
{
    CW_STAMP(env, 0);
    const CwMtWave::Pending pend = CwMtWave::load_issue(P.mt + (size_t)env * CW_MT_WORDS, P.mt_idx + env, lane);
    const uint32_t menu_id = menu_fn();
    const CwMenuDev M = P.menus[menu_id];
    CwMtWave mt;
    mt.load_commit(lds_mt, pend, lane);
    CW_STAMP(env, 1);

    const uint32_t desired = draw_tasks_wave(mt, M);

    CW_STAMP(env, 2);
    const uint32_t v_tok = place_env_wave(P, env, mt, P.pool_k != 0, lane);
    const uint32_t init_agent = __builtin_amdgcn_readlane(v_tok, 8);
    uint32_t v_fp = lane < 8 ? v_tok : (uint32_t)CW_POS_GONE;
    uint32_t v_fc = lane < 8 ? (uint32_t)lane + 1u : 0u;
    uint32_t ip[8];
#pragma unroll
    for (int k = 0; k < 8; k++) ip[k] = __builtin_amdgcn_readlane(v_tok, k);
    const uint4 init_packed = pack_pos(ip);
    CW_STAMP(env, 3);

    const uint32_t agent = imagine_env_wave(P, mt, v_fp, v_fc, init_agent, init_agent, desired);

    CW_STAMP(env, 4);
    const uint32_t draws = mt.draws();
    mt.store(P.mt + (size_t)env * CW_MT_WORDS, P.mt_idx + env, lane);
    CW_STAMP(env, 5);
    CwResetOut r;
    r.init_pos = init_packed;
    r.init_agent = init_agent;
    pack_goal_wave(v_fp, v_fc, r.goal_pos, r.goal_codes);
    r.goal_agent = agent;
    r.desired = desired;
    r.subset = M.reward_subset ? 1u : 0u;
    r.draws = draws;
    return r;
}

__device__ __forceinline__ uint4 reset_header(const CwParams &P, const CwResetOut &r, uint32_t menu_id)
{
    const uint32_t ar = __umulhi(r.init_agent, P.div_magic);
    const uint32_t ac = r.init_agent - ar * P.size;
    uint4 h;
    h.x = ar | (ac << 8) | (menu_id << 24);
    h.y = r.desired << 16;
    h.z = (CW_FLAG_RESET | (r.subset ? CW_FLAG_SUBSET : 0u)) << 16;
    h.w = CW_CODES_INITIAL;
    return h;
}
__device__ __forceinline__ void store_episode_records(const CwParams &P, int env, const CwResetOut &r, bool count_episode)
{
    P.goal_pos[env] = r.goal_pos;
    P.goal_codes[env] = r.goal_codes;
    P.goal_agent[env] = (uint16_t)r.goal_agent;
    P.init_pos[env] = r.init_pos;
    P.init_agent[env] = (uint16_t)r.init_agent;
    if (count_episode) P.ep_no[env] += 1;
}

__device__ __forceinline__ void store_next_record(const CwParams &P, int env, int slot, const CwResetOut &r)
{
    const size_t at = (size_t)slot * P.n_envs + env;
    P.nx_init_pos[at] = r.init_pos;
    P.nx_goal_pos[at] = r.goal_pos;
    P.nx_misc[at] = make_uint4(r.init_agent | (r.goal_agent << 16), r.goal_codes, r.desired | (r.subset << 16) | 0x80000000u, r.draws);
}
__global__ __launch_bounds__(CW_RESET_WAVES *CW_WAVE) void cw_reset_kernel(CwParams P)
{
    __shared__ uint32_t s_mt[CW_RESET_WAVES][CW_MT_WORDS];
    const int lane = threadIdx.x & (CW_WAVE - 1);
    const int wave_in_block = __builtin_amdgcn_readfirstlane(threadIdx.x / CW_WAVE);
    const int n_waves = (int)gridDim.x * CW_RESET_WAVES;
    for (int env = (int)blockIdx.x * CW_RESET_WAVES + wave_in_block; env < P.n_envs; env += n_waves) {
        const uint4 v_h = P.hdr[env];
        const uint32_t menu_id = __builtin_amdgcn_readfirstlane(v_h.x) >> 24;
        const bool count_episode = (__builtin_amdgcn_readfirstlane(v_h.z) & 0xFFFFu) != 0;
        const uint32_t ctl = P.lookahead ? __builtin_amdgcn_readfirstlane(P.nx_ctl[env]) : 0u;
        if (P.lookahead && (__builtin_amdgcn_readfirstlane(P.nx_misc[(size_t)(ctl & 0xFFu) * P.n_envs + env].z) >> 31)) {
            if (lane == 0) {
                uint4 h = v_h;
                uint32_t sp[8];
                pop_next_episode(P, env, ctl, h, sp, count_episode);
                P.pos[env] = pack_pos(sp);
                P.hdr[env] = h;
                P.achieved_out[env] = 0;
                P.desired_out[env] = (uint16_t)(h.y >> 16);
            }
            continue;
        }
        const CwResetOut r = reset_env_wave(P, env, [&]() { return menu_id; }, s_mt[wave_in_block], lane);
        if (lane == 0) {
            store_episode_records(P, env, r, count_episode);
            P.pos[env] = r.init_pos;
            P.hdr[env] = reset_header(P, r, menu_id);
            P.achieved_out[env] = 0;
            P.desired_out[env] = (uint16_t)r.desired;
        }
    }
}

template <bool PAINT>
__global__ __launch_bounds__(CW_RESET_WAVES *CW_WAVE) void cw_reset_masked_kernel(CwParams P, const uint8_t *__restrict__ mask, int epb)
{
    __shared__ uint32_t s_mt[CW_RESET_WAVES][CW_MT_WORDS];
    const int lane = threadIdx.x & (CW_WAVE - 1);
    const int wave_in_block = __builtin_amdgcn_readfirstlane(threadIdx.x / CW_WAVE);
    for (int base = (int)blockIdx.x * epb; base < P.n_envs; base += (int)gridDim.x * epb) {
        const int mine = base + lane;
        const bool in_chunk = lane < epb && mine < P.n_envs;
        const uint32_t v_sel = in_chunk ? (uint32_t)mask[mine] : 0u;
        unsigned long long m = CW_BALLOT(v_sel != 0u);
        for (int rank = 0; m; rank++) {
            const int l = __builtin_ctzll(m);
            m &= m - 1;
            if ((rank & (CW_RESET_WAVES - 1)) != wave_in_block) continue;
            const int env = base + l;
            const uint4 v_h = P.hdr[env];
            const uint32_t menu_id = __builtin_amdgcn_readfirstlane(v_h.x) >> 24;
            const bool count_episode = (__builtin_amdgcn_readfirstlane(v_h.z) & 0xFFFFu) != 0;
            const uint32_t ctl = P.lookahead ? __builtin_amdgcn_readfirstlane(P.nx_ctl[env]) : 0u;
            uint4 ipos, gpos;
            uint32_t iagent, gagent, gcodes;
            if (P.lookahead && (__builtin_amdgcn_readfirstlane(P.nx_misc[(size_t)(ctl & 0xFFu) * P.n_envs + env].z) >> 31)) {
                uint4 h = v_h;
                uint32_t sp[8] = {0, 0, 0, 0, 0, 0, 0, 0};
                CwGoalState goal;
                goal.pos = make_uint4(0, 0, 0, 0); goal.codes = 0; goal.agent = 0;
                if (lane == 0) {
                    pop_next_episode(P, env, ctl, h, sp, count_episode, PAINT ? &goal : nullptr);
                    P.pos[env] = pack_pos(sp);
                    P.hdr[env] = h;
                    P.achieved_out[env] = 0;
                    P.desired_out[env] = (uint16_t)(h.y >> 16);
                }
                if constexpr (PAINT) {
                    const uint4 p0 = pack_pos(sp);
                    ipos = make_uint4(__builtin_amdgcn_readfirstlane(p0.x), __builtin_amdgcn_readfirstlane(p0.y), __builtin_amdgcn_readfirstlane(p0.z),
                                      __builtin_amdgcn_readfirstlane(p0.w));
                    gpos = make_uint4(__builtin_amdgcn_readfirstlane(goal.pos.x), __builtin_amdgcn_readfirstlane(goal.pos.y),
                                      __builtin_amdgcn_readfirstlane(goal.pos.z), __builtin_amdgcn_readfirstlane(goal.pos.w));
                    iagent = agent_cell_of(P, __builtin_amdgcn_readfirstlane(h.x));
                    gagent = __builtin_amdgcn_readfirstlane(goal.agent);
                    gcodes = __builtin_amdgcn_readfirstlane(goal.codes);
                }
            } else {
                const CwResetOut r = reset_env_wave(P, env, [&]() { return menu_id; }, s_mt[wave_in_block], lane);
                if (lane == 0) {
                    store_episode_records(P, env, r, count_episode);
                    P.pos[env] = r.init_pos;
                    P.hdr[env] = reset_header(P, r, menu_id);
                    P.achieved_out[env] = 0;
                    P.desired_out[env] = (uint16_t)r.desired;
                    if (P.lookahead) note_slow_reset(P, env, ctl);
                }
                ipos = r.init_pos; gpos = r.goal_pos;
// ... 324 lines not shown
        if (s_cnt[0]) atomicAdd(&P.counters[1], (unsigned long long)s_cnt[0]);
        if (s_cnt[1]) atomicAdd(&P.counters[2], (unsigned long long)s_cnt[1]);
        if (s_cnt[2]) atomicAdd(&P.counters[3], (unsigned long long)s_cnt[2]);
    }
    constexpr int jpe = TERM ? 3 : 2;
    int jmine = 0;
    if constexpr (PAINT != 0) {
        int jbase = 0;
        if (m_all) {
            if (lane == 0) jbase = atomicAdd(s_njobs, jpe * __popcll(m_all));
            jbase = __shfl(jbase, 0);
        }
        jmine = jbase + jpe * __popcll(m_all & ((1ull << lane) - 1ull));
        if constexpr (TERM) if (done) {
            CwPaintJob &j = s_jobs[jmine + 2];
            j.pos = pack_pos(sp_last);
            j.codes = h_last.w;
            j.agent_hold_kind = agent_cell_of(P, h_last.x) | (hold_of(h_last.x) << 16) | (CW_JOB_TERMINAL << 24);
            j.env = (uint32_t)env;
        }
        if (popped) {
            CwPaintJob &j0 = s_jobs[jmine], &j1 = s_jobs[jmine + 1];
            j0.pos = pack_pos(sp);
            j0.codes = CW_CODES_INITIAL;
            j0.agent_hold_kind = agent_cell_of(P, h.x) | (CW_JOB_INIT << 24);
            j0.env = (uint32_t)env;
            j1.pos = goal.pos;
            j1.codes = goal.codes;
            j1.agent_hold_kind = goal.agent | (CW_JOB_GOAL << 24);
            j1.env = (uint32_t)env;
        }
    }
    unsigned long long m = m_all & ~m_pop;
    while (m) {
        const int l = __builtin_ctzll(m);
        m &= m - 1;
        const int env_l = env0 + l;
        const uint32_t menu_id = __builtin_amdgcn_readlane(h.x, l) >> 24;
        const CwResetOut r = reset_env_wave(P, env_l, [&]() { return menu_id; }, s_mt_wave, lane);
        if (lane == 0) {
            store_episode_records(P, env_l, r, true);
            if (P.lookahead) note_slow_reset(P, env_l, __builtin_amdgcn_readlane(ctl, l));
        }
        if (lane == l) {
            h = reset_header(P, r, menu_id);
            unpack_pos(r.init_pos, sp);
            if constexpr (PAINT != 0) {
                CwPaintJob &j0 = s_jobs[jmine], &j1 = s_jobs[jmine + 1];
                j0.pos = r.init_pos; j0.codes = CW_CODES_INITIAL; j0.agent_hold_kind = r.init_agent | (CW_JOB_INIT << 24); j0.env = (uint32_t)env_l;
                j1.pos = r.goal_pos; j1.codes = r.goal_codes; j1.agent_hold_kind = r.goal_agent | (CW_JOB_GOAL << 24); j1.env = (uint32_t)env_l;
            }
        }
    }
    if (live) {
        P.hdr[env] = h;
        P.pos[env] = pack_pos(sp);
    }
    if constexpr (PAINT == 0) return;
    __syncthreads();
    const int n_jobs = *s_njobs;
    for (int jq = wave_in_block; jq < n_jobs; jq += CW_RESET_WAVES) {
        const CwPaintJob &j = s_jobs[jq];
        uint32_t jp[8];
        unpack_pos(make_uint4(__builtin_amdgcn_readfirstlane(j.pos.x), __builtin_amdgcn_readfirstlane(j.pos.y), __builtin_amdgcn_readfirstlane(j.pos.z),
                              __builtin_amdgcn_readfirstlane(j.pos.w)), jp);
        const uint32_t codes = __builtin_amdgcn_readfirstlane(j.codes), ahk = __builtin_amdgcn_readfirstlane(j.agent_hold_kind);
        const size_t off = (size_t)__builtin_amdgcn_readfirstlane(j.env) * P.frame_bytes;
        const uint32_t kind = ahk >> 24;
        uint8_t *d0, *d1 = nullptr;
        if (kind == CW_JOB_INIT) { d0 = P.init_img + off; if (paint == 1) d1 = P.obs + off; }
        else if (kind == CW_JOB_GOAL) d0 = P.desired_img + off;
        else d0 = P.terminal_img + off;
        paint_state_frame(P, d0, jp, codes, ahk & 0xFFFFu, (ahk >> 16) & 0xFFu, lane, d1);
    }
}
template <int PAINT, bool TERM>
__global__ __launch_bounds__(CW_RESET_WAVES *CW_WAVE) void cw_step_fused_kernel(CwParams P, const void *actions, int act_dtype, int epw)
{
    __shared__ uint32_t s_mt[CW_RESET_WAVES][CW_MT_WORDS];
    __shared__ CwPaintJob s_jobs[PAINT != 0 ? CW_RESET_WAVES * CW_WAVE * (TERM ? 3 : 2) : 1];
    __shared__ int s_njobs;
    __shared__ int s_cnt[3];
    const int wave_in_block = __builtin_amdgcn_readfirstlane(threadIdx.x / CW_WAVE);
    fused_step<PAINT, TERM>(P, actions, act_dtype, epw, blockIdx.x * CW_RESET_WAVES + wave_in_block, s_mt[wave_in_block], s_jobs, &s_njobs, s_cnt);
}
typedef void (*CwStepFusedKernel)(CwParams, const void *, int, int);
static CwStepFusedKernel cw_step_fused_variant(int paint, bool term)
{
    if (paint == 0) return cw_step_fused_kernel<0, false>;
    if (paint == 1) return term ? cw_step_fused_kernel<1, true> : cw_step_fused_kernel<1, false>;
    return term ? cw_step_fused_kernel<2, true> : cw_step_fused_kernel<2, false>;
}

__global__ __launch_bounds__(CW_RESET_WAVES *CW_WAVE) void cw_pool_kernel(CwParams P)
{
    __shared__ uint32_t s_mt[CW_RESET_WAVES][CW_MT_WORDS];
    const int lane = threadIdx.x & (CW_WAVE - 1);
    const int wave_in_block = __builtin_amdgcn_readfirstlane(threadIdx.x / CW_WAVE);
    const int n_waves = gridDim.x * CW_RESET_WAVES;
    for (int env = blockIdx.x * CW_RESET_WAVES + wave_in_block; env < P.n_envs; env += n_waves) {
        CwMtWave mt;
        mt.load(s_mt[wave_in_block], P.mt + (size_t)env * CW_MT_WORDS, P.mt_idx + env, lane);
        for (int k = 0; k < P.pool_k; k++) {
            const uint32_t v_tok = shuffle_tokens(mt, P.ncell);
            uint16_t *pp = P.pool + ((size_t)env * P.pool_k + k) * 9;
            if (lane < 9) pp[lane] = (uint16_t)v_tok;
        }
        mt.store(P.mt + (size_t)env * CW_MT_WORDS, P.mt_idx + env, lane);
    }
}

__global__ __launch_bounds__(256) void cw_render_frames_kernel(CwParams P, uint8_t *out)
{
    const int lane = threadIdx.x & (CW_WAVE - 1);
    const int wave = (blockIdx.x * blockDim.x + threadIdx.x) / CW_WAVE;
    const int n_waves = gridDim.x * blockDim.x / CW_WAVE;
    for (int env = wave; env < P.n_envs; env += n_waves) {
        uint32_t sp[8], codes, agent_cell, hold;
        load_state_uniform(P, env, CW_SRC_CURRENT, sp, codes, agent_cell, hold);
        paint_state_frame(P, out + (size_t)env * P.frame_bytes, sp, codes, agent_cell, hold, lane);
    }
}

#define CW_PIECE 4096u
#define CW_PIECE_STORES 4
#ifndef CW_HEAD_JOBS
#define CW_HEAD_JOBS 64
#endif
#define CW_BUSY_FINISHED 16ull
__device__ __attribute__((noinline)) void piece_fill_partial(uint8_t *dst_base, uint32_t a0, uint32_t a1, int lane)
{
    for (int s = 0; s < CW_PIECE_STORES; s++) {
        const uint32_t c = a0 + 1024u * s + 16u * lane;
        if (c + 16u <= a1) *(uint4 *)(dst_base + c) = make_uint4(0, 0, 0, 0);
        else for (uint32_t b = c; b < a1; b++) dst_base[b] = 0;
    }
}
template <int RASTER, int FPJ>
__device__ __forceinline__ void render_pieces(const CwParams &P, uint8_t *frames, int src, int period16, int head_extra16, int env_lo, int env_n)
{
    constexpr int JPB = CW_WAVE / FPJ;
    const int lane = threadIdx.x & (CW_WAVE - 1);
    const int wpb = blockDim.x / CW_WAVE;
    const int wave_in_block = __builtin_amdgcn_readfirstlane(threadIdx.x / CW_WAVE);
    const int n_waves = (int)gridDim.x * wpb;
    const int wave = (int)blockIdx.x * wpb + wave_in_block;
    const uint32_t S = (uint32_t)P.size, FB = P.frame_bytes, row_bytes = (RASTER == 1 ? 9u : 12u) * S;
    uint8_t *const dst_base = frames + (size_t)env_lo * FB;
    const uint32_t total = (uint32_t)env_n * FB;
    const int n_jobs = (int)((total + CW_PIECE - 1u) / CW_PIECE);
    if (wave >= n_jobs) return;
    const int q_mine = (n_jobs + n_waves - 1) / n_waves;
    const uint32_t half = (uint32_t)lane >> 5, pl = (uint32_t)lane & 31u;
    const uint32_t slot = RASTER == 1 ? (pl & 7u) : (pl >> 2), dy = pl & 3u;
    const uint32_t v_cpv = cpv_color(lane & 15), v_rgb = rgb_of_code((uint32_t)lane & 15u);
    const uint32_t m_slot = (RASTER != 1 || pl < 8u) ? 0xFFFFFFFFu : 0u, m_agent = pl == 8u ? 0xFFFFFFFFu : 0u, m_held = pl == 9u ? 0xFFFFFFFFu : 0u;
    const uint32_t m_flag = (pl >= 10u && pl < 19u) ? 0xFFFFFFFFu : 0u;
    const uint32_t sh_pos = 16u * (slot & 1u), sh_item = 4u * slot;
    const uint32_t m_p0 = (slot & 6u) == 0u ? 0xFFFFFFFFu : 0u, m_p1 = (slot & 6u) == 2u ? 0xFFFFFFFFu : 0u;
    const uint32_t m_p2 = (slot & 6u) == 4u ? 0xFFFFFFFFu : 0u, m_p3 = (slot & 6u) == 6u ? 0xFFFFFFFFu : 0u;
    const uint32_t fj = pl >= 10u ? pl - 10u : 0u, fjr = (fj >= 6u) ? 2u : (fj >= 3u) ? 1u : 0u;
    const uint32_t off_flag = (3u * S + fjr) * row_bytes + 9u + 3u * (fj - 3u * fjr);
    const bool marks = slot == 0u && (dy == 1u || dy == 2u);
    __builtin_amdgcn_s_setprio(3);
    struct Rec { int f; uint32_t hx, hw, o2; uint4 p; };
    auto fetch = [&](int base) {
        Rec r;
        const int i = base + lane / FPJ;
        const int id = i * n_waves + wave;
        r.f = -1; r.hx = 0; r.hw = 0; r.o2 = 0;
        r.p = make_uint4(0, 0, 0, 0);
        if (i < q_mine && id < n_jobs) {
            const int f = (int)(((uint32_t)id * CW_PIECE) / FB) + (lane % FPJ);
            if (f < env_n) {
                r.f = f;
                const int e = env_lo + f;
                if (src == CW_SRC_CURRENT) {
                    const uint32_t *h = (const uint32_t *)(P.hdr + e);
                    r.hx = h[0];
                    r.hw = h[3];
                    r.p = P.pos[e];
                } else {
                    r.hx = src == CW_SRC_INIT ? (uint32_t)P.init_agent[e] : (uint32_t)P.goal_agent[e];
                    r.hw = src == CW_SRC_INIT ? CW_CODES_INITIAL : P.goal_codes[e];
                    r.p = src == CW_SRC_INIT ? P.init_pos[e] : P.goal_pos[e];
                }
            }
        }
        if (src == CW_SRC_CURRENT) r.hx &= 0x00FFFFFFu;
        else { const uint32_t ar = __umulhi(r.hx, P.div_magic); r.hx = ar | ((r.hx - ar * S) << 8); }
        if (RASTER != 1) { const uint32_t hold = (r.hx >> 16) & 0xFFu; r.o2 = hold ? rgb_of_code(hold) : 0x00FFFFFFu; }
        return r;
    };
    Rec nxt = fetch(0);
    uint32_t t_next16 = ((uint32_t)__builtin_amdgcn_s_memrealtime() << 4) + (uint32_t)(((long long)wave * period16) / n_waves);
    for (int base = 0; base < q_mine; base += JPB) {
        const Rec cur = nxt;
        if (base + JPB < q_mine) nxt = fetch(base + JPB);
        const int in_batch = min(q_mine - base, JPB);
        for (int k = 0; k < in_batch; k++) {
            const int f0 = __builtin_amdgcn_readlane(cur.f, FPJ * k);
            if (f0 < 0) continue;
            const uint32_t a0 = (uint32_t)((base + k) * n_waves + wave) * CW_PIECE;
            const uint32_t a1 = min(a0 + CW_PIECE, total);
            const uint32_t win = a1 - a0;
            uint32_t hx = 0, hw = 0, o2 = 0, pd = 0;
            auto gather = [&](int pair) {
                const int from = (int)(((uint32_t)(FPJ * k + 2 * pair) + half) << 2);
                hx = (uint32_t)__builtin_amdgcn_ds_bpermute(from, (int)cur.hx);
                hw = (uint32_t)__builtin_amdgcn_ds_bpermute(from, (int)cur.hw);
                o2 = RASTER != 1 ? (uint32_t)__builtin_amdgcn_ds_bpermute(from, (int)cur.o2) : 0u;
                pd = ((uint32_t)__builtin_amdgcn_ds_bpermute(from, (int)cur.p.x) & m_p0) | ((uint32_t)__builtin_amdgcn_ds_bpermute(from, (int)cur.p.y) & m_p1) |
                     ((uint32_t)__builtin_amdgcn_ds_bpermute(from, (int)cur.p.z) & m_p2) | ((uint32_t)__builtin_amdgcn_ds_bpermute(from, (int)cur.p.w) & m_p3);
            };
            if (RASTER != 1) gather(0);
            if (period16) {
                const uint32_t now16 = (uint32_t)__builtin_amdgcn_s_memrealtime() << 4;
                const int wait16 = (int)(t_next16 - now16);
                if (wait16 > 0) {
                    for (int z = (wait16 * 5) >> 8; z > 0; z--) __builtin_amdgcn_s_sleep(1);
                    while ((int)(t_next16 - ((uint32_t)__builtin_amdgcn_s_memrealtime() << 4)) > 0) { }
                } else if (wait16 < -period16) t_next16 = now16 - (uint32_t)period16;
                t_next16 += (uint32_t)(period16 + (base + k < CW_HEAD_JOBS ? head_extra16 : 0));
            }
            uint8_t *const job = dst_base + a0;
            if (win == CW_PIECE) {
#pragma unroll
                for (int s = 0; s < CW_PIECE_STORES; s++) *(uint4 *)(job + 1024 * s + 16 * lane) = make_uint4(0, 0, 0, 0);
            } else piece_fill_partial(dst_base, a0, a1, lane);
#pragma unroll
            for (int pair = 0; pair < FPJ / 2; pair++) {
                if (FPJ > 2 && pair > 0 && ((uint32_t)f0 + 2u * pair >= (uint32_t)env_n || ((uint32_t)f0 + 2u * pair) * FB >= a1)) break;
                if (RASTER == 1 || pair > 0) gather(pair);
                const uint32_t fi = (uint32_t)f0 + 2u * (uint32_t)pair + half;
                const uint32_t f_base = __umul24(fi, FB);
                const bool frame_on = fi < (uint32_t)env_n && f_base < a1;
                const uint32_t hold = (hx >> 16) & 0xFFu;
                if (RASTER == 1) {
                    const uint32_t agent_cell = __umul24(hx & 0xFFu, S) + ((hx >> 8) & 0xFFu);
                    const uint32_t pos = (((pd >> sh_pos) & 0xFFFFu) & m_slot) | (agent_cell & ~m_slot);
                    const uint32_t item = (((hw >> sh_item) & 15u) & m_slot) | (9u & m_agent) | (hold & m_held);
                    const uint32_t r = __umulhi(pos, P.div_magic), c = pos - __umul24(r, S), kk = item - 1u;
                    const uint32_t k3 = (kk >= 6u) ? 2u : (kk >= 3u) ? 1u : 0u;
                    const uint32_t off_obj = __umul24(3u * r + k3, row_bytes) + 9u * c + 3u * (kk - 3u * k3);
                    const uint32_t col_obj = (uint32_t)__builtin_amdgcn_ds_bpermute((int)((kk & 15u) << 2), (int)v_cpv);
                    const bool is_obj = (m_flag == 0u) && pl < 10u && item != 0 && pos < (uint32_t)P.ncell;
                    const bool is_flag = (m_flag & hold) != 0;
                    uint32_t p_off = is_obj ? off_obj : is_flag ? off_flag : 0xFFFFFFFFu;
                    uint32_t p_val = is_obj ? col_obj : 0x00FFFFFFu;
                    const uint32_t held_off = (uint32_t)__builtin_amdgcn_ds_bpermute((int)((((uint32_t)lane & 32u) + 9u) << 2), (int)p_off);
                    const bool twice = pl < 8u && p_off != 0xFFFFFFFFu && p_off == held_off;
                    p_val = twice ? (((2u * (p_val & 0xFFu)) & 0xFFu) | ((2u * (p_val & 0xFF00u)) & 0xFF00u) | ((2u * (p_val & 0xFF0000u)) & 0xFF0000u)) : p_val;
                    const unsigned long long m_twice = CW_BALLOT(twice);
                    p_off = (pl == 9u && ((m_twice >> (32u * half)) & 0xFFFFFFFFull)) ? 0xFFFFFFFFu : p_off;
                    if (frame_on && p_off != 0xFFFFFFFFu) {
                        const uint32_t at = f_base + p_off;
                        if (at - a0 < win) dst_base[at] = (uint8_t)p_val;
                        if (at + 1u - a0 < win) dst_base[at + 1u] = (uint8_t)(p_val >> 8);
                        if (at + 2u - a0 < win) dst_base[at + 2u] = (uint8_t)(p_val >> 16);
                    }
                } else {
                    const uint32_t pos = (pd >> sh_pos) & 0xFFFFu, code = (hw >> sh_item) & 15u;
                    const uint32_t rgb = (uint32_t)__builtin_amdgcn_ds_bpermute((int)(code << 2), (int)v_rgb);
                    const uint32_t r = __umulhi(pos, P.div_magic), c = pos - __umul24(r, S);
                    const uint32_t seg = f_base + __umul24(4u * r + dy, row_bytes) + 12u * c;
                    const u32x3 d = cell_row_dwords(rgb);
                    const bool is_obj = frame_on && code != 0 && pos < (uint32_t)P.ncell;
                    const bool in0 = seg - a0 < win, in2 = seg + 8u - a0 < win;
                    if (is_obj && in0 && in2) *(u32x3_a4 *)(dst_base + seg) = d;
                    else if (is_obj) {
                        if (in0) *(uint32_t *)(dst_base + seg) = d.x;
                        if (seg + 4u - a0 < win) *(uint32_t *)(dst_base + seg + 4u) = d.y;
                        if (in2) *(uint32_t *)(dst_base + seg + 8u) = d.z;
                    }
                    const uint32_t aseg = f_base + __umul24(4u * (hx & 0xFFu) + dy, row_bytes) + 12u * ((hx >> 8) & 0xFFu);
                    const uint32_t o = dy == 2u ? o2 : 0x00FFFFFFu;
                    const bool is_mark = frame_on && marks;
                    if (is_mark && aseg - a0 < win) dst_base[aseg + 3u] = (uint8_t)o;
                    if (is_mark && aseg + 4u - a0 < win) *(uint32_t *)(dst_base + aseg + 4u) = (o >> 8) | (o << 16);
                    if (is_mark && aseg + 8u - a0 < win) dst_base[aseg + 8u] = (uint8_t)(o >> 16);
                }
            }
        }
    }
}
template <int RASTER, int FPJ>
__global__ __launch_bounds__(256) void cw_render_pieces_kernel(CwParams P, uint8_t *frames, int src, int period16, int period16_head, int period16_busy,
                                                               int chunk, int env_lo, int env_n)
{
    const unsigned long long done_now = P.counters[1];
    const unsigned long long finished = src == CW_SRC_CURRENT ? done_now - P.counters[4] : (unsigned long long)P.n_envs;
    const bool busy = finished >= CW_BUSY_FINISHED, storm = finished * 8ull >= (unsigned long long)P.n_envs;
    render_pieces<RASTER, FPJ>(P, frames, src, __builtin_amdgcn_readfirstlane(storm ? period16_busy : period16),
                               __builtin_amdgcn_readfirstlane(!storm && (chunk & 1) ? (busy ? period16_busy : period16_head) - period16 : 0), env_lo, env_n);
    if (src == CW_SRC_CURRENT && (chunk & 2) && blockIdx.x == 0 && threadIdx.x == 0) P.counters[4] = done_now;
}
#define CW_GATHER_MAX_S 9
template <int NF>
__global__ __launch_bounds__(256) void cw_render_gather_kernel(CwParams P, uint8_t *frames, int src, int period16, int env_lo, int env_n)
{
    constexpr int JPB = CW_WAVE / NF;
    constexpr int COL_WORDS = (NF * CW_GATHER_MAX_S * CW_GATHER_MAX_S + 255) / 256 * 256;
    __shared__ uint32_t s_col[256 / CW_WAVE][COL_WORDS];
    __shared__ uint32_t s_slot[CW_GATHER_MAX_S * CW_GATHER_MAX_S * 3];
    const int lane = threadIdx.x & (CW_WAVE - 1);
    const int wpb = blockDim.x / CW_WAVE;
    const int wave_in_block = __builtin_amdgcn_readfirstlane(threadIdx.x / CW_WAVE);
    const int n_waves = (int)gridDim.x * wpb;
    const int wave = (int)blockIdx.x * wpb + wave_in_block;
    const uint32_t S = (uint32_t)P.size, ncell = (uint32_t)P.ncell, FB = P.frame_bytes, row_bytes = 12u * S, Q = FB >> 4;
    for (uint32_t q = threadIdx.x; q < Q; q += blockDim.x) {
        const uint32_t o = 16u * q, y = o / row_bytes, x = o - y * row_bytes, c0 = x / 12u, ph = (x - 12u * c0) >> 2;
        const uint32_t cell_a = (y >> 2) * S + c0;
        uint32_t cell_b, dy_b;
        if (c0 + 1u < S) { cell_b = cell_a + 1u; dy_b = y & 3u; }
        else { const uint32_t y2 = min(y + 1u, 4u * S - 1u); cell_b = (y2 >> 2) * S; dy_b = y2 & 3u; }
        s_slot[q] = cell_a | (cell_b << 8) | ((y & 3u) << 16) | (dy_b << 18) | (ph << 20);
    }
    __syncthreads();
    uint8_t *const dst_base = frames + (size_t)env_lo * FB;
    const uint32_t total = (uint32_t)env_n * FB;
    const int n_jobs = (int)((total + CW_PIECE - 1u) / CW_PIECE);
    if (wave >= n_jobs) return;
    const int q_mine = (n_jobs + n_waves - 1) / n_waves;
    uint32_t *const col = s_col[wave_in_block];
    const uint32_t v_rgb = rgb_of_code((uint32_t)lane & 15u);
    const uint32_t fr = (uint32_t)lane >> 3, slot = (uint32_t)lane & 7u;
    const uint32_t sh_pos = 16u * (slot & 1u), sh_item = 4u * slot;
    const uint32_t m_p0 = (slot & 6u) == 0u ? 0xFFFFFFFFu : 0u, m_p1 = (slot & 6u) == 2u ? 0xFFFFFFFFu : 0u;
    const uint32_t m_p2 = (slot & 6u) == 4u ? 0xFFFFFFFFu : 0u, m_p3 = (slot & 6u) == 6u ? 0xFFFFFFFFu : 0u;
    const uint32_t q_magic = (uint32_t)((1ull << 32) / Q) + 1u;
    const int zero_rounds = __builtin_amdgcn_readfirstlane((int)((((CW_PIECE - 1u) / FB + 2u) * ncell + 255u) / 256u));
    __builtin_amdgcn_s_setprio(3);
    struct Rec { int f; uint32_t hx, hw; uint4 p; };
    auto fetch = [&](int base) {
        Rec r;
        const int i = base + lane / NF;
        const int id = i * n_waves + wave;
        r.f = -1; r.hx = 0; r.hw = 0;
        r.p = make_uint4(0, 0, 0, 0);
        if (i < q_mine && id < n_jobs) {
            const int f = (int)(((uint32_t)id * CW_PIECE) / FB) + (lane % NF);
            if (f < env_n) {
                r.f = f;
                const int e = env_lo + f;
                if (src == CW_SRC_CURRENT) {
                    const uint32_t *h = (const uint32_t *)(P.hdr + e);
                    r.hx = h[0];
                    r.hw = h[3];
                    r.p = P.pos[e];
                } else {
                    r.hx = src == CW_SRC_INIT ? (uint32_t)P.init_agent[e] : (uint32_t)P.goal_agent[e];
                    r.hw = src == CW_SRC_INIT ? CW_CODES_INITIAL : P.goal_codes[e];
                    r.p = src == CW_SRC_INIT ? P.init_pos[e] : P.goal_pos[e];
                }
            }
        }
        if (src == CW_SRC_CURRENT) r.hx &= 0x00FFFFFFu;
        else { const uint32_t ar = __umulhi(r.hx, P.div_magic); r.hx = ar | ((r.hx - ar * S) << 8); }
        return r;
    };
    Rec nxt = fetch(0);
    uint32_t t_next16 = ((uint32_t)__builtin_amdgcn_s_memrealtime() << 4) + (uint32_t)(((long long)wave * period16) / n_waves);
    for (int base = 0; base < q_mine; base += JPB) {
        const Rec cur = nxt;
        if (base + JPB < q_mine) nxt = fetch(base + JPB);
        const int in_batch = min(q_mine - base, JPB);
        for (int k = 0; k < in_batch; k++) {
            const int f0 = __builtin_amdgcn_readlane(cur.f, NF * k);
            if (f0 < 0) continue;
            const uint32_t a0 = (uint32_t)((base + k) * n_waves + wave) * CW_PIECE;
            const uint32_t a1 = min(a0 + CW_PIECE, total);
            for (int z = 0; z < zero_rounds; z++) *(uint4 *)(col + 256 * z + 4 * lane) = make_uint4(0, 0, 0, 0);
            {
                const int from = (int)(((uint32_t)(NF * k) + (fr & (uint32_t)(NF - 1))) << 2);
                const uint32_t hx = (uint32_t)__builtin_amdgcn_ds_bpermute(from, (int)cur.hx), hw = (uint32_t)__builtin_amdgcn_ds_bpermute(from, (int)cur.hw);
                const int ff = __builtin_amdgcn_ds_bpermute(from, cur.f);
                const uint32_t pd = ((uint32_t)__builtin_amdgcn_ds_bpermute(from, (int)cur.p.x) & m_p0) | ((uint32_t)__builtin_amdgcn_ds_bpermute(from, (int)cur.p.y) & m_p1) |
// ... 142 lines not shown
                const uint32_t cnt = (uint32_t)c[k] + (k < 3 ? (uint32_t)c[9 + k] : 0u), col = cpv_color(k);
                uint16_t *px = img + ((size_t)(3u * cr + k / 3) * row_px + 3u * cc + k % 3) * 3;
                px[0] = (uint16_t)(cnt * (col & 0xFFu)); px[1] = (uint16_t)(cnt * ((col >> 8) & 0xFFu)); px[2] = (uint16_t)(cnt * (col >> 16));
            }
        }
        for (uint32_t j = (uint32_t)lane; j < 3u * row_px; j += CW_WAVE) {
            const uint32_t x = j % row_px;
            const uint16_t v = (any_held && x >= 3u && x < 6u) ? 255 : 0;
            uint16_t *px = img + ((size_t)(3u * S) * row_px + j) * 3;
            px[0] = v; px[1] = v; px[2] = v;
        }
    }
}

__global__ __launch_bounds__(256) void cw_seed_kernel(CwParams P, const uint32_t *seeds)
{
    const int i = blockIdx.x * blockDim.x + threadIdx.x;
    if (i >= P.n_envs) return;
    uint32_t *s = P.mt + (size_t)i * CW_MT_WORDS;
    int pos;
    if (seeds) {
        uint32_t x = seeds[i];
        s[0] = x;
        for (int k = 1; k < CW_MT_WORDS; k++) {
            x = 1812433253u * (x ^ (x >> 30)) + (uint32_t)k;
            s[k] = x;
        }
        pos = CW_MT_WORDS;
    } else {
        pos = min(max(P.mt_idx[i], 0), CW_MT_WORDS);
    }
    uint32_t cur = s[0];
    for (int k = 0; k < pos; k++) {
        const uint32_t nxt = s[k + 1 == CW_MT_WORDS ? 0 : k + 1];
        const uint32_t far = s[k + 397 >= CW_MT_WORDS ? k + 397 - CW_MT_WORDS : k + 397];
        const uint32_t y = (cur & 0x80000000u) | (nxt & 0x7fffffffu);
        s[k] = far ^ (y >> 1) ^ ((y & 1u) ? 0x9908b0dfu : 0u);
        cur = nxt;
    }
    P.mt_idx[i] = pos == CW_MT_WORDS ? 0 : pos;
}

static inline int cw_frames_per_job(uint32_t frame_bytes)
{
    const int most = (int)((CW_PIECE - 1u) / frame_bytes) + 2;
    int fpj = 2;
    while (fpj < most) fpj <<= 1;
    return fpj;
}
static inline int cw_piece_chunks(const CwParams &P, const CwTuning &tn, int *per)
{
    const long long waves = (long long)tn.n_cu * (256 / CW_WAVE);
    const long long cap = (long long)(tn.render_chunk_rounds > 0 ? tn.render_chunk_rounds : 1 << 20) * waves * 3072;
    const long long bytes = (long long)P.n_envs * P.frame_bytes;
    int n = (int)((bytes + cap - 1) / cap);
    if (n < 1) n = 1;
    *per = (P.n_envs + n - 1) / n;
    if (n > 1 || bytes >= (1ll << 32)) {
        *per = (int)(((long long)*per + 4095) / 4096 * 4096);
        while ((long long)*per * P.frame_bytes >= (1ll << 32) && *per > 4096) *per = (*per / 2 + 4095) / 4096 * 4096;
    }
    return (P.n_envs + *per - 1) / *per;
}
static inline int cw_render_grid(const CwTuning &tn, long long jobs)
{
    long long blocks = (jobs + 3) / 4;
    if (blocks > tn.n_cu) blocks = tn.n_cu;
    if (blocks < 1) blocks = 1;
    return (int)blocks;
}
static inline bool cw_use_gather(const CwParams &P, const CwTuning &tn) { return tn.gather && P.raster == 0 && P.size <= tn.gather_max_size; }
static inline int cw_sweep_blocks(const CwParams &P, const CwTuning &tn, long long pieces)
{
    const bool small = (int)P.frame_bytes < tn.small_frame_bytes && (cw_use_gather(P, tn) || pieces * (long long)CW_PIECE < tn.small_launch_bytes);
    const int per_cu = small && pieces > 4ll * tn.n_cu * tn.small_blocks_per_cu ? tn.small_blocks_per_cu : 1;
    return cw_render_grid(tn, pieces) * per_cu;
}
typedef void (*CwSweepKernel)(CwParams, uint8_t *, int, int, int, int, int, int, int);
static CwSweepKernel cw_sweep_kernel(int raster, int fpj)
{
    if (raster == 1) return fpj <= 2 ? cw_render_pieces_kernel<1, 2> : fpj <= 4 ? cw_render_pieces_kernel<1, 4> : fpj <= 8 ? cw_render_pieces_kernel<1, 8> : cw_render_pieces_kernel<1, 16>;
    return fpj <= 2 ? cw_render_pieces_kernel<0, 2> : fpj <= 4 ? cw_render_pieces_kernel<0, 4> : fpj <= 8 ? cw_render_pieces_kernel<0, 8> : cw_render_pieces_kernel<0, 16>;
}
static void cw_launch_sweep(const CwParams &P, const CwTuning &tn, uint8_t *frames, int src, hipStream_t st)
{
    int per = 0;
    const int n_chunks = cw_piece_chunks(P, tn, &per);
    const CwSweepKernel k = cw_sweep_kernel(P.raster, cw_frames_per_job(P.frame_bytes));
    for (int c = 0; c < n_chunks; c++) {
        const int env_n = min(per, P.n_envs - c * per);
        const long long pieces = ((long long)env_n * P.frame_bytes + CW_PIECE - 1) / CW_PIECE;
        if (cw_use_gather(P, tn)) {
            const int grid = cw_sweep_blocks(P, tn, pieces);
            if (cw_frames_per_job(P.frame_bytes) <= 4)
                hipLaunchKernelGGL(cw_render_gather_kernel<4>, dim3(grid), dim3(256), 0, st, P, frames, src, tn.period16, c * per, env_n);
            else
                hipLaunchKernelGGL(cw_render_gather_kernel<8>, dim3(grid), dim3(256), 0, st, P, frames, src, tn.period16, c * per, env_n);
            continue;
        }
        hipLaunchKernelGGL(k, dim3(cw_sweep_blocks(P, tn, pieces)), dim3(256), 0, st, P, frames, src, tn.period16, tn.period16_head, tn.period16_busy, (c == 0 ? 1 : 0) | (c == n_chunks - 1 ? 2 : 0), c * per, env_n);
    }
}

static inline int cw_wave_blocks(int waves) { return (waves + CW_RESET_WAVES - 1) / CW_RESET_WAVES; }
static inline int cw_reset_grid(const CwTuning &tn, int jobs)
{
    int blocks = cw_wave_blocks(jobs);
    if (blocks > tn.n_cu * tn.reset_blocks_per_cu) blocks = tn.n_cu * tn.reset_blocks_per_cu;
    if (blocks < 1) blocks = 1;
    return blocks;
}

static int cw_envs_per_wave(int n, int most = 64)
{
    int epw = most;
    while (epw > 8 && (n + epw - 1) / epw < 1024) epw >>= 1;
    return epw;
}

extern "C" {

hipError_t cwk_launch_step(const CwParams *P, const CwTuning *T, const void *actions, int act_dtype, int obs_mode,
                           int auto_reset, hipStream_t st, hipEvent_t *ev )
{
    const CwTuning &tn = *T;
    const int n = P->n_envs;
    const bool ev_all = ev && obs_mode != 1;
    if (ev_all) (void)hipEventRecord(ev[0], st);
    if (auto_reset) {
        const int epw = cw_envs_per_wave(n, tn.step_envs_per_wave);
        const int waves = (n + epw - 1) / epw;
        const int paint = obs_mode == 2 ? 1 : obs_mode == 1 ? 2 : 0;
        hipLaunchKernelGGL(cw_step_fused_variant(paint, paint != 0 && P->terminal_img != nullptr), dim3(cw_wave_blocks(waves)), dim3(CW_RESET_WAVES * CW_WAVE),
                           0, st, *P, actions, act_dtype, epw);
    } else {
        hipLaunchKernelGGL(cw_step_kernel, dim3((n + 255) / 256), dim3(256), 0, st, *P, actions, act_dtype, obs_mode == 2 ? 1 : 0);
    }
    if (ev_all) (void)hipEventRecord(ev[1], st);
    if (ev) for (int k = 2; k < 5; k++) (void)hipEventRecord(ev[k], st);
    if (obs_mode == 1) cw_launch_sweep(*P, tn, P->obs, CW_SRC_CURRENT, st);
    if (ev) (void)hipEventRecord(ev[5], st);
    return hipGetLastError();
}

hipError_t cwk_launch_refill(const CwParams *P, const CwTuning *T, int all_envs, hipStream_t st)
{
    hipLaunchKernelGGL(cw_refill_kernel, dim3(cw_reset_grid(*T, P->n_envs)), dim3(CW_RESET_WAVES * CW_WAVE), 0, st, *P, all_envs);
    return hipGetLastError();
}

hipError_t cwk_launch_rollout(const CwParams *P, const uint8_t *actions, int T, int32_t *rewards, uint8_t *dones, hipStream_t st)
{
    const int epw = cw_envs_per_wave(P->n_envs);
    const int waves = (P->n_envs + epw - 1) / epw;
    hipLaunchKernelGGL(cw_rollout_kernel, dim3(cw_wave_blocks(waves)), dim3(CW_RESET_WAVES * CW_WAVE), 0, st, *P, actions, T, rewards, dones, epw);
    return hipGetLastError();
}

hipError_t cwk_launch_render_restore(const CwParams *P, const CwTuning *T, hipStream_t st)
{
    cw_launch_sweep(*P, *T, P->obs, CW_SRC_CURRENT, st);
    cw_launch_sweep(*P, *T, P->init_img, CW_SRC_INIT, st);
    cw_launch_sweep(*P, *T, P->desired_img, CW_SRC_GOAL, st);
    return hipGetLastError();
}

hipError_t cwk_launch_reset_all(const CwParams *P, const CwTuning *T, int obs_mode, hipStream_t st)
{
    hipLaunchKernelGGL(cw_reset_kernel, dim3(cw_reset_grid(*T, P->n_envs)), dim3(CW_RESET_WAVES * CW_WAVE), 0, st, *P);
    if (obs_mode != 0) return cwk_launch_render_restore(P, T, st);
    return hipGetLastError();
}

hipError_t cwk_launch_reset_masked(const CwParams *P, const CwTuning *T, const uint8_t *mask, int obs_mode, hipStream_t st)
{
    const int most = T->n_cu * T->reset_blocks_per_cu;
    int epb = CW_WAVE;
    while (epb > CW_RESET_WAVES && (P->n_envs + epb - 1) / epb < most) epb >>= 1;
    const int blocks = cw_reset_grid(*T, ((P->n_envs + epb - 1) / epb) * CW_RESET_WAVES);
    if (obs_mode != 0) hipLaunchKernelGGL(cw_reset_masked_kernel<true>, dim3(blocks), dim3(CW_RESET_WAVES * CW_WAVE), 0, st, *P, mask, epb);
    else hipLaunchKernelGGL(cw_reset_masked_kernel<false>, dim3(blocks), dim3(CW_RESET_WAVES * CW_WAVE), 0, st, *P, mask, epb);
    return hipGetLastError();
}

static int cw_masked_epb(const CwParams *P, const CwTuning *T)
{
    const int most = T->n_cu * T->reset_blocks_per_cu;
    int epb = CW_WAVE;
    while (epb > CW_RESET_WAVES && (P->n_envs + epb - 1) / epb < most) epb >>= 1;
    return epb;
}
hipError_t cwk_launch_imagine_masked(const CwParams *P, const CwTuning *T, const uint8_t *mask, const uint16_t *desired, int commit, int obs_mode,
                                     uint8_t *out_frames, uint8_t *out_onehot, hipStream_t st)
{
    const int epb = cw_masked_epb(P, T);
    const int blocks = cw_reset_grid(*T, ((P->n_envs + epb - 1) / epb) * CW_RESET_WAVES);
    const int paint_goal = obs_mode != 0;
    if (out_frames || (commit && paint_goal))
        hipLaunchKernelGGL(cw_imagine_masked_kernel<true>, dim3(blocks), dim3(CW_RESET_WAVES * CW_WAVE), 0, st, *P, mask, desired, commit, paint_goal,
                           out_frames, out_onehot, epb);
    else
        hipLaunchKernelGGL(cw_imagine_masked_kernel<false>, dim3(blocks), dim3(CW_RESET_WAVES * CW_WAVE), 0, st, *P, mask, desired, commit, paint_goal,
                           out_frames, out_onehot, epb);
    return hipGetLastError();
}
hipError_t cwk_launch_sample_state_masked(const CwParams *P, const CwTuning *T, const uint8_t *mask, int pooled, uint16_t *out_cells, hipStream_t st)
{
    const int epb = cw_masked_epb(P, T);
    const int blocks = cw_reset_grid(*T, ((P->n_envs + epb - 1) / epb) * CW_RESET_WAVES);
    hipLaunchKernelGGL(cw_sample_state_masked_kernel, dim3(blocks), dim3(CW_RESET_WAVES * CW_WAVE), 0, st, *P, mask, pooled, out_cells, epb);
    return hipGetLastError();
}

hipError_t cwk_launch_render_onehot(const CwParams *P, const uint8_t *onehot, int n_states, uint16_t *out, hipStream_t st)
{
    int blocks = (n_states + 3) / 4;
    if (blocks > 1024) blocks = 1024;
    if (blocks < 1) blocks = 1;
    if (P->raster == 1) hipLaunchKernelGGL(cw_render_onehot_alt_kernel, dim3(blocks), dim3(256), 0, st, onehot, n_states, P->size, P->div_magic, out);
    else hipLaunchKernelGGL(cw_render_onehot_kernel, dim3(blocks), dim3(256), 0, st, onehot, n_states, P->size, P->div_magic, out);
    return hipGetLastError();
}

hipError_t cwk_launch_resident(const CwParams *P, CwResident *R, uint32_t seq0, int paint_dirty, unsigned long long idle_ticks,
                               unsigned long long life_ticks, hipStream_t st)
{
    hipLaunchKernelGGL(cw_resident_kernel, dim3(1), dim3(CW_WAVE), 0, st, *P, R, seq0, paint_dirty, idle_ticks, life_ticks);
    return hipGetLastError();
}

hipError_t cwk_launch_seed(const CwParams *P, const uint32_t *seeds_dev, hipStream_t st)
{
    hipLaunchKernelGGL(cw_seed_kernel, dim3((P->n_envs + 255) / 256), dim3(256), 0, st, *P, seeds_dev);
    return hipGetLastError();
}

hipError_t cwk_launch_pool(const CwParams *P, const CwTuning *T, hipStream_t st)
{
    const int n = P->n_envs;
    hipLaunchKernelGGL(cw_pool_kernel, dim3(cw_reset_grid(*T, n)), dim3(CW_RESET_WAVES * CW_WAVE), 0, st, *P);
    return hipGetLastError();
}

void cwk_sweep_shape(const CwParams *P, const CwTuning *T, int *n_chunks, int *waves, int *jobs_per_wave)
{
    int per = 0;
    *n_chunks = cw_piece_chunks(*P, *T, &per);
    const long long pieces = ((long long)min(per, P->n_envs) * P->frame_bytes + CW_PIECE - 1) / CW_PIECE;
    *waves = cw_sweep_blocks(*P, *T, pieces) * (256 / CW_WAVE);
    *jobs_per_wave = (int)((pieces + *waves - 1) / *waves);
}

hipError_t cwk_launch_sweep_calib(const CwParams *P, const CwTuning *T, hipStream_t st)
{
    cw_launch_sweep(*P, *T, P->obs, CW_SRC_CURRENT, st);
    return hipGetLastError();
}

__global__ void cw_idle_kernel(int n)
{
    for (int i = 0; i < n; i++) __builtin_amdgcn_s_sleep(127);
}
hipError_t cwk_launch_idle(hipStream_t st)
{
    hipLaunchKernelGGL(cw_idle_kernel, dim3(1), dim3(64), 0, st, 3);
    return hipGetLastError();
}

hipError_t cwk_launch_render_ext(const CwParams *P, const CwTuning *T, uint8_t *out, hipStream_t st)
{
    if (((uintptr_t)out & 15u) == 0) cw_launch_sweep(*P, *T, out, CW_SRC_CURRENT, st);
    else hipLaunchKernelGGL(cw_render_frames_kernel, dim3(cw_render_grid(*T, P->n_envs)), dim3(256), 0, st, *P, out);
    return hipGetLastError();
}

hipError_t cwk_launch_export(const CwParams *P, const CwTuning *T, uint8_t *out, int onehot, int which, hipStream_t st)
{
    const size_t total = (size_t)P->n_envs * P->ncell;
    const size_t cap = (size_t)T->n_cu * 32;
    int blocks = (int)((total + 255) / 256 < cap ? (total + 255) / 256 : cap);
    if (blocks < 1) blocks = 1;
    if (onehot) hipLaunchKernelGGL(cw_export_onehot_kernel, dim3(blocks), dim3(256), 0, st, *P, out, which);
    else hipLaunchKernelGGL(cw_export_grid_kernel, dim3(blocks), dim3(256), 0, st, *P, out);
    return hipGetLastError();
}

}
```

### gym_craftingworld_amd/csrc/cw_layout.h

```cpp
#pragma once
#include <stdint.h>

#define CW_POS_GONE 0xFFFFu
#define CW_POS_HELD 0xFFFEu

#define CW_FLAG_RESET 0x1u
#define CW_FLAG_SUBSET 0x2u


#define CW_CODES_INITIAL 0x87654321u
#define CW_CTL_QUEUED 0x100u
#define CW_LA_DEPTH 4

struct CwMenuDev {
    uint64_t sel_bits;
    int32_t n_selected;
    int32_t number_of_tasks;
    int32_t stacking;
    int32_t reward_subset;
};

struct CwTuning {
    int n_cu = 256;
    int period16 = 0;
    int period16_head = 0;
    int period16_busy = 0;
    int render_chunk_rounds = 896;
    int gather = 1;
    int gather_max_size = 7;
    int small_frame_bytes = 4096;
    int small_blocks_per_cu = 4;
    long long small_launch_bytes = 320ll << 20;
    int step_envs_per_wave = 64;
    int reset_blocks_per_cu = 4;
};

struct CwResident {
    unsigned long long bell;
    uint32_t pad0[30];
    uint32_t ack;
    uint32_t exited;
    uint32_t pad1[30];
};

struct CwParams {
    uint4 *hdr;
    uint4 *pos;
    uint4 *init_pos;
    uint16_t *init_agent;
    uint4 *goal_pos;
    uint32_t *goal_codes;
    uint16_t *goal_agent;
    int32_t *ep_no;
    uint32_t *mt;
    int32_t *mt_idx;
    uint16_t *pool;
    int32_t *reward;
    uint8_t *done;
    uint16_t *achieved_out;
    uint16_t *desired_out;
    int32_t *episode_length;
    int32_t *episode_return;
    uint8_t *obs;
    uint8_t *desired_img;
    uint8_t *init_img;
    uint8_t *terminal_img;
    uint4 *nx_init_pos;
    uint4 *nx_goal_pos;
    uint4 *nx_misc;
    uint32_t *nx_ctl;
    int32_t lookahead;
    unsigned long long *la_feedback;
    unsigned long long *counters;
    const CwMenuDev *menus;
    int32_t n_envs;
    int32_t size;
    int32_t ncell;
    int32_t max_steps;
    uint32_t task_mask;
    int32_t pool_k;
    uint32_t div_magic;
    uint32_t frame_bytes;
    int32_t raster;
    uint8_t *res_onehot;
};
```

### gym_craftingworld_amd/vec_env.py

```python
import atexit
import ctypes as C
import sys
import weakref

import numpy as np
import torch

from . import _lib as L
from . import seeding
from ._wrap import tensor_view
from .spaces import Box, Dict, Discrete, MultiDiscrete, batch_space

TASK_LIST = ['MakeBread', 'EatBread', 'BuildHouse', 'ChopTree', 'ChopRock', 'GoToHouse', 'MoveAxe',
             'MoveHammer', 'MoveSticks']
OBJECTS = ['sticks', 'axe', 'hammer', 'rock', 'tree', 'bread', 'house', 'wheat']
PICKUPABLE = ['sticks', 'axe', 'hammer']
ACTION_NAMES = ['up', 'right', 'down', 'left', 'pickup', 'drop']
UP, RIGHT, DOWN, LEFT, PICKUP, DROP = range(6)
COLORS = [(110, 69, 39), (255, 105, 180), (100, 100, 200), (100, 100, 100), (0, 128, 0), (205, 133, 63), (197, 91, 97), (240, 230, 140)]
COLORS_N = [(0, 0, 0)] + COLORS
COLORS_H = [tuple(255 - c for c in COLORS[k]) for k in range(3)]
STATE_W = STATE_H = 21
MAX_STEPS = 300

# ... 492 lines not shown
                'cw_render_onehot', self._lib)
        self._states_keepalive = oh
        return out

    def grid(self, out=None):
        if out is None:
            out = torch.empty((self.num_envs, self.size, self.size), dtype=torch.uint8, device=self.device)
        L.check(self._lib.cw_export_grid(self._h, C.c_void_p(out.data_ptr()), self._stream()), 'cw_export_grid', self._lib)
        return out

    def one_hot(self, out=None, which='current'):
        if out is None:
            out = torch.empty((self.num_envs, self.size, self.size, 12), dtype=torch.uint8, device=self.device)
        w = {'current': 0, 'goal': 1, 'init': 2}[which]
        L.check(self._lib.cw_export_onehot_of(self._h, w, C.c_void_p(out.data_ptr()), self._stream()), 'cw_export_onehot_of', self._lib)
        return out

    def mask_to_vector(self, mask):
        bits = torch.arange(len(self.task_list), device=mask.device, dtype=torch.int32)
        return ((mask.to(torch.int32).unsqueeze(1) >> bits) & 1).to(torch.uint8)

    def fixed_states(self):
        out = np.empty((self.num_envs, max(self.fixed_init_state, 1), 9), dtype=np.uint16)
        self._settle()
        L.check(self._lib.cw_get_fixed_states(self._h, out.ctypes.data_as(C.c_void_p)), 'cw_get_fixed_states', self._lib)
        return out

    def get_state(self):
        N, S = self.num_envs, self.size
        out = dict(grid=np.empty((N, S, S), np.uint8), init_grid=np.empty((N, S, S), np.uint8),
                   goal_grid=np.empty((N, S, S), np.uint8), agent_rc=np.empty((N, 2), np.uint8),
                   init_agent_rc=np.empty((N, 2), np.uint8), goal_agent_rc=np.empty((N, 2), np.uint8),
                   hold=np.empty(N, np.uint8), achieved=np.empty(N, np.uint16), desired=np.empty(N, np.uint16),
                   step_num=np.empty(N, np.int32), ep_no=np.empty(N, np.int32))
        view = L.cw_state_view(**{k: a.ctypes.data_as(C.c_void_p) for k, a in out.items()})
        self._settle()
        L.check(self._lib.cw_get_state(self._h, C.byref(view)), 'cw_get_state', self._lib)
        return out

    def set_state(self, **fields):
        dt = dict(grid=np.uint8, init_grid=np.uint8, goal_grid=np.uint8, agent_rc=np.uint8, init_agent_rc=np.uint8,
                  goal_agent_rc=np.uint8, hold=np.uint8, achieved=np.uint16, desired=np.uint16, step_num=np.int32,
                  ep_no=np.int32)
        keep = {}
        view = L.cw_state_view()
        for k, a in fields.items():
            if k not in dt:
                raise ValueError('cannot set %r' % k)
            keep[k] = np.ascontiguousarray(a, dtype=dt[k])
            if keep[k].shape[0] != self.num_envs:
                raise ValueError('%s must have num_envs rows' % k)
            setattr(view, k, keep[k].ctypes.data_as(C.c_void_p))
        self._settle()
        L.check(self._lib.cw_set_state(self._h, C.byref(view)), 'cw_set_state', self._lib)

    def save_checkpoint(self, path):
        n = int(self._lib.cw_checkpoint_bytes(self._h))
        buf = np.empty(n, dtype=np.uint8)
        self._settle()
        L.check(self._lib.cw_checkpoint_save(self._h, buf.ctypes.data_as(C.c_void_p), n), 'cw_checkpoint_save', self._lib)
        with open(path, 'wb') as f:
            buf.tofile(f)

    def load_checkpoint(self, path):
        buf = np.fromfile(path, dtype=np.uint8)
        self._settle()
        L.check(self._lib.cw_checkpoint_load(self._h, buf.ctypes.data_as(C.c_void_p), buf.size), 'cw_checkpoint_load', self._lib)
        self._has_reset = True

    def profile_begin(self, max_steps):
        L.check(self._lib.cw_profile_begin(self._h, int(max_steps)), 'cw_profile_begin', self._lib)

    def render_kernel_name(self):
        return (self._lib.cw_render_kernel_name(self._h) or b'').decode()

    def profile_end(self):
        p = L.cw_profile()
        L.check(self._lib.cw_profile_end(self._h, C.byref(p)), 'cw_profile_end', self._lib)
        return {k: getattr(p, k) for k, _ in p._fields_}

    def tuner_state(self):
        t = L.cw_tuner_state()
        L.check(self._lib.cw_tuner(self._h, C.byref(t)), 'cw_tuner', self._lib)
        return {k: int(getattr(t, k)) for k, _ in t._fields_}

    def compute_reward_batch(self, achieved_mask, desired_mask, subset=None):
        full = (1 << len(self.task_list)) - 1
        a = achieved_mask.to(torch.int32) & full
        d = desired_mask.to(torch.int32) & full
        if subset is None:
            subset = bool(self._menus[0].reward_subset)
        if subset:
            hit = ((d & ~a) == 0) & (((~(d ^ a)) & full) != 0)
        else:
            hit = a == d
        return torch.where(hit, torch.full_like(a, self.MAX_STEPS), torch.full_like(a, -1))

    def compute_reward(self, achieved_goal, desired_goal, info=None):
        a = np.asarray(achieved_goal).reshape(-1)
        d = np.asarray(desired_goal).reshape(-1)
        if self._menus[0].reward_subset:
            return self.MAX_STEPS if np.max(d.astype(np.int64) - a.astype(np.int64)) == 0 else -1
        return self.MAX_STEPS if np.array_equal(a, d) else -1
```

### include/craftingworld.h

```cpp
#ifndef CRAFTINGWORLD_H
#define CRAFTINGWORLD_H

#include <stddef.h>
#include <stdint.h>

#ifdef __cplusplus
extern "C" {
#endif

#define CW_ABI_VERSION 5
#define CW_MT_N 624
#define CW_MAX_TASKS 16
#define CW_MAX_MENUS 256
#define CW_NUM_OBJECTS 8

#define CW_OK 0
#define CW_ERR_INVALID (-1)
#define CW_ERR_HIP (-2)
#define CW_ERR_STATE (-3)

enum { CW_EMPTY = 0, CW_STICKS = 1, CW_AXE = 2, CW_HAMMER = 3, CW_ROCK = 4, CW_TREE = 5,
       CW_BREAD = 6, CW_HOUSE = 7, CW_WHEAT = 8 };

enum {
// ... 52 lines not shown
    uint16_t *slot_pos;
    uint64_t *counters;
    size_t frame_bytes;
    int32_t *host_actions;
    uint8_t *host_onehot;
} cw_buffer_table;

typedef struct cw_state_view {
    uint8_t *grid;
    uint8_t *init_grid;
    uint8_t *goal_grid;
    uint8_t *agent_rc;
    uint8_t *init_agent_rc;
    uint8_t *goal_agent_rc;
    uint8_t *hold;
    uint16_t *achieved;
    uint16_t *desired;
    int32_t *step_num;
    int32_t *ep_no;
} cw_state_view;

int cw_create(const cw_config *cfg, int device, cw_engine **out);
int cw_destroy(cw_engine *e);

int cw_seed_mt(cw_engine *e, const uint32_t *keys, const int32_t *pos);
int cw_seed_int(cw_engine *e, const uint32_t *seeds);
int cw_get_mt(cw_engine *e, uint32_t *keys, int32_t *pos);

int cw_generate_fixed_states(cw_engine *e, cw_stream_t stream);
int cw_get_fixed_states(cw_engine *e, uint16_t *out);

int cw_reset(cw_engine *e, cw_stream_t stream);

int cw_reset_masked(cw_engine *e, const uint8_t *mask, cw_stream_t stream);

int cw_imagine_masked(cw_engine *e, const uint8_t *mask, const uint16_t *desired, int32_t commit,
                      uint8_t *out_frames, uint8_t *out_onehot, cw_stream_t stream);

int cw_sample_state_masked(cw_engine *e, const uint8_t *mask, int32_t pooled, uint16_t *out_cells, cw_stream_t stream);

int cw_step(cw_engine *e, const void *actions, int action_dtype, cw_stream_t stream);

int cw_step_many(cw_engine *e, const void *actions, int action_dtype, int32_t n_steps, cw_stream_t stream);

int cw_rollout(cw_engine *e, const uint8_t *actions, int32_t n_steps, int32_t *rewards, uint8_t *dones,
               cw_stream_t stream);

int cw_step_resident(cw_engine *e, int32_t action, int32_t want_onehot );
int cw_resident_stop(cw_engine *e);

int cw_render(cw_engine *e, uint8_t *out_frames, cw_stream_t stream);

int cw_render_onehot(cw_engine *e, const uint8_t *onehot, int32_t n_states, uint16_t *out_frames, cw_stream_t stream);

int cw_export_grid(cw_engine *e, uint8_t *out, cw_stream_t stream);
int cw_export_onehot(cw_engine *e, uint8_t *out, cw_stream_t stream);
enum { CW_STATE_CURRENT = 0, CW_STATE_GOAL = 1, CW_STATE_INIT = 2 };
int cw_export_onehot_of(cw_engine *e, int which, uint8_t *out, cw_stream_t stream);

int cw_get_state(cw_engine *e, cw_state_view *host);
int cw_set_state(cw_engine *e, const cw_state_view *host);

size_t cw_checkpoint_bytes(cw_engine *e);
int cw_checkpoint_save(cw_engine *e, void *buf, size_t capacity);
int cw_checkpoint_load(cw_engine *e, const void *buf, size_t length);

typedef struct cw_profile {
    int32_t steps;
    float ms_step_kernel;
    float ms_reset_kernel;
    float ms_render_kernel;
    float ms_render_kernel_max;
    float ms_render_kernel_min;
    float ms_render_kernel_median;
} cw_profile;
int cw_profile_begin(cw_engine *e, int max_steps);
int cw_profile_end(cw_engine *e, cw_profile *out);
const char *cw_render_kernel_name(const cw_engine *e);

typedef struct cw_tuner_state {
    int32_t period16, period16_head, period16_busy, lookahead, resident, guard_slowdowns;
} cw_tuner_state;
int cw_tuner(const cw_engine *e, cw_tuner_state *out);

int cw_buffers(cw_engine *e, cw_buffer_table *out);
int cw_synchronize(cw_engine *e, cw_stream_t stream);
int cw_num_envs(const cw_engine *e);
int cw_abi_version(void);
const char *cw_last_error(void);

#ifdef __cplusplus
}
#endif
#endif
```

Before: 319.4 million.

## Move sweep-rate guard from host event ring to device-side clock block

Replaces the host-side guard, which recorded HIP events every 64 steps and adapted the sweep rate on the host, with a device-resident clock block. Render kernels now read their period values from device memory and stamp entry and exit times with s_memrealtime. An extra block in the fused step kernel appears to run the guard update on the GPU. This removes host event recording and polling from the step path and lets rate changes take effect without a host round trip. In exchange it adds atomics, a block barrier and a global read to each render launch, and calibration now uses a stamp-based median.

```diff
diff --git a/gym_craftingworld_amd/_lib.py b/gym_craftingworld_amd/_lib.py
--- a/gym_craftingworld_amd/_lib.py
+++ b/gym_craftingworld_amd/_lib.py
@@ -56,6 +56,11 @@
 class cw_tuner_state(C.Structure):
     _fields_ = [('period16', C.c_int32), ('period16_head', C.c_int32), ('period16_busy', C.c_int32), ('lookahead', C.c_int32), ('resident', C.c_int32),
                 ('guard_slowdowns', C.c_int32)]
+
+
+class cw_clock_info(C.Structure):
+    _fields_ = [(f, C.c_int32) for f in ('guard_on', 'rate_milli', 'rate_top_milli', 'settle_left', 'probes')] + \
+               [(f, C.c_uint32) for f in ('launches', 'samples', 'last_sweep_ticks')]
 
 
 _VP = C.c_void_p
@@ -87,6 +92,7 @@
     'cw_profile_begin': (C.c_int, [_VP, C.c_int]),
     'cw_profile_end': (C.c_int, [_VP, C.POINTER(cw_profile)]),
     'cw_tuner': (C.c_int, [_VP, C.POINTER(cw_tuner_state)]),
+    'cw_clock_state': (C.c_int, [_VP, C.POINTER(cw_clock_info)]),
     'cw_step_resident': (C.c_int, [_VP, C.c_int32, C.c_int32]),
     'cw_resident_stop': (C.c_int, [_VP]),
     'cw_render_kernel_name': (C.c_char_p, [_VP]),
@@ -99,7 +105,15 @@
 class cwh_guard(C.Structure):
     _fields_ = [('rate', C.c_double), ('rate_top', C.c_double), ('ms_sum', C.c_double), ('prev_mean', C.c_double), ('ref_ms', C.c_double),
                 ('ref_prev', C.c_double), ('ms_n', C.c_int32), ('late', C.c_int32), ('good', C.c_int32), ('slowdowns', C.c_int32),
-                ('probes', C.c_int32), ('probe_need', C.c_int32), ('recover_need', C.c_int32), ('probing', C.c_int32), ('recovering', C.c_int32)]
+                ('probes', C.c_int32), ('probe_need', C.c_int32), ('recover_need', C.c_int32), ('probing', C.c_int32), ('recovering', C.c_int32),
+                ('settle_left', C.c_int32), ('settle_samples', C.c_int32)]
+
+
+class cw_clock(C.Structure):
+    _fields_ = [('period16', C.c_int32), ('period16_head', C.c_int32), ('period16_busy', C.c_int32), ('sample_now', C.c_int32),
+                ('t_min', C.c_uint64), ('t_max', C.c_uint64), ('storm', C.c_int32), ('on', C.c_int32), ('stride', C.c_int32), ('phase', C.c_int32),
+                ('launch', C.c_uint32), ('samples', C.c_uint32), ('last_ticks', C.c_uint32), ('sweep_waves', C.c_int32), ('skip', C.c_int32), ('pad', C.c_int32),
+                ('sweep_jobs', C.c_double), ('beside_ms', C.c_double), ('head_notch', C.c_double), ('busy_notch', C.c_double), ('g', cwh_guard)]
 
 
 class cwh_tuning(C.Structure):
@@ -113,6 +127,7 @@
 
 CWH_GUARD_NONE, CWH_GUARD_SLOWDOWN, CWH_GUARD_TRIAL_UP, CWH_GUARD_TRIAL_KEPT, CWH_GUARD_TRIAL_UNDONE = range(5)
 CWH_CKPT_SECTIONS = 22
+CWH_GUARD_SETTLE_SAMPLES, CW_CLOCK_STRIDE, CW_CLOCK_SKIP, CW_CLOCK_GAP_TICKS = 128, 61, 8, 5000
 
 HOST_HELPERS = {
     'cwh_mt_from_numpy': (C.c_int, [_VP, C.c_int]),
@@ -125,6 +140,10 @@
     'cwh_ckpt_section_bytes': (C.c_int, [C.c_int64, C.c_int32, C.c_int32, C.POINTER(C.c_size_t), C.POINTER(C.c_uint64)]),
     'cwh_guard_init': (None, [C.POINTER(cwh_guard), C.c_double]),
     'cwh_guard_step': (C.c_int, [C.POINTER(cwh_guard), C.c_double, C.c_double]),
+    'cwh_guard_settle': (None, [C.POINTER(cwh_guard), C.c_int32]),
+    'cwh_clock_init': (None, [C.POINTER(cw_clock), C.c_double, C.c_int32, C.c_int32, C.c_double, C.c_double, C.c_double, C.c_double]),
+    'cwh_clock_tick': (C.c_int, [C.POINTER(cw_clock), C.c_uint64]),
+    'cwh_clock_bytes': (C.c_size_t, []),
     'cwh_sweep_periods': (None, [C.c_double, C.c_int32, C.c_double, C.c_double, C.POINTER(C.c_int32), C.POINTER(C.c_int32), C.POINTER(C.c_int32)]),
     'cwh_guard_scheduled_ms': (C.c_double, [C.c_double, C.c_int32, C.c_int32, C.c_double]),
     'cwh_la_adapt': (C.c_int32, [C.c_int32, C.c_int32, C.c_uint64, C.POINTER(C.c_int32)]),
diff --git a/gym_craftingworld_amd/csrc/cw_engine.cpp b/gym_craftingworld_amd/csrc/cw_engine.cpp
--- a/gym_craftingworld_amd/csrc/cw_engine.cpp
+++ b/gym_craftingworld_amd/csrc/cw_engine.cpp
@@ -33,6 +33,7 @@
 hipError_t cwk_launch_sweep_calib(const CwParams *P, const CwTuning *T, hipStream_t st);
 void cwk_sweep_shape(const CwParams *P, const CwTuning *T, int *n_chunks, int *waves, int *jobs_per_wave);
 hipError_t cwk_launch_idle(hipStream_t st);
+hipError_t cwk_launch_stamps_collect(const CwParams *P, unsigned long long *out2, hipStream_t st);
 hipError_t cwk_launch_export(const CwParams *P, const CwTuning *T, uint8_t *out, int onehot, int which, hipStream_t st);
 }
 
@@ -108,11 +109,6 @@
     bool guard_on = false;
     double head_notch = 0.4, busy_notch = 0.75, tune_period_ns = -1, tune_rate_tbs = -1;
     bool tune_guard = true, tune_lookahead = true, verbose = false;
-    enum { GUARD_RING = 32 };
-    struct GuardSample { hipEvent_t ev[6]; int period16; } guard_ring[GUARD_RING] = {};
-    unsigned guard_head = 0, guard_tail = 0;
-    unsigned guard_step = 0;
-    cwh_guard guard{};
     int prof_cap = 0, prof_n = 0;
     hipStream_t aux = nullptr;
     hipStream_t work[4] = {nullptr, nullptr, nullptr, nullptr};
@@ -229,10 +225,27 @@
     return CW_OK;
 }
 
+static inline cw_clock *clock_block(const cw_engine *e) { return (cw_clock *)(e->P.counters + CW_CLOCK_WORD); }
 static double sweep_period_ns(const cw_engine *e, double tb_per_s) { return (double)e->sweep_waves * 4096.0 / (tb_per_s * 1e12) * 1e9; }
 static void set_sweep_rate(cw_engine *e, double tb_per_s)
 {
     cwh_sweep_periods(tb_per_s, e->sweep_waves, e->head_notch, e->busy_notch, &e->tune.period16, &e->tune.period16_head, &e->tune.period16_busy);
+}
+
+static int stamped_render_median(cw_engine *e, double *median)
+{
+    enum { LAUNCHES = 24, SKIP = 4 };
+    unsigned long long *dev = (unsigned long long *)e->seed_scratch, host[2 * LAUNCHES];
+    bool ok = (size_t)e->n * sizeof(uint32_t) >= sizeof(host) && cwk_launch_stamps_collect(&e->P, nullptr, e->aux) == hipSuccess;
+    for (int rep = 0; rep < LAUNCHES && ok; rep++)
+        ok = cwk_launch_sweep_calib(&e->P, &e->tune, e->aux) == hipSuccess && cwk_launch_stamps_collect(&e->P, dev + 2 * rep, e->aux) == hipSuccess;
+    ok = ok && hipMemcpyAsync(host, dev, sizeof(host), hipMemcpyDeviceToHost, e->aux) == hipSuccess && hipStreamSynchronize(e->aux) == hipSuccess;
+    if (!ok) return fail(CW_ERR_HIP, "cw_create: render calibration (stamps) failed");
+    double ms[LAUNCHES];
+    for (int rep = 0; rep < LAUNCHES; rep++) ms[rep] = host[2 * rep + 1] > host[2 * rep] ? (double)(host[2 * rep + 1] - host[2 * rep]) * 1e-5 : 0.0;
+    std::sort(ms + SKIP, ms + LAUNCHES);
+    *median = ms[SKIP + (LAUNCHES - SKIP) / 2];
+    return CW_OK;
 }
 
 static int calibrate_sweep(cw_engine *e)
@@ -257,7 +270,7 @@
     double best_p90 = 0, med = 0, p90 = 0, mean = 0;
     rc = timed_render_stats(e, &med, &p90);
     set_sweep_rate(e, 6.4);
-    if (rc == CW_OK) rc = timed_render_stats(e, &med, &p90);
+    if (rc == CW_OK) rc = stamped_render_median(e, &med);
     e->sweep_beside_ms = med - e->sweep_jobs * sweep_period_ns(e, 6.4) * 1e-6;
     if (e->tune_rate_tbs >= 0) e->sweep_rate = e->tune_rate_tbs;
     for (size_t i = 0; i < sizeof(rates) / sizeof(rates[0]) && rc == CW_OK && e->tune_rate_tbs < 0; i++) {
@@ -267,41 +280,18 @@
         if (rc == CW_OK && (best_p90 == 0 || p90 < 0.995 * best_p90)) { best_p90 = p90; e->sweep_rate = rates[i]; }
     }
     set_sweep_rate(e, e->sweep_rate);
-    cwh_guard_init(&e->guard, e->sweep_rate);
     e->guard_on = rc == CW_OK && e->sweep_rate > 0 && e->auto_reset && e->tune_guard;
-    if (e->guard_on)
-        for (auto &smp : e->guard_ring)
-            for (hipEvent_t &ev : smp.ev)
-                if (hipEventCreate(&ev) != hipSuccess) e->guard_on = false;
+    if (e->guard_on) {
+        cw_clock c;
+        cwh_clock_init(&c, e->sweep_rate, 1, e->sweep_waves, e->sweep_jobs, e->sweep_beside_ms, e->head_notch, e->busy_notch);
+        if (hipMemcpyAsync(clock_block(e), &c, sizeof(c), hipMemcpyHostToDevice, e->aux) != hipSuccess || hipStreamSynchronize(e->aux) != hipSuccess)
+            return fail(CW_ERR_HIP, "cw_create: the clock block could not be written");
+        tn.guard = 1;
+    }
     if (e->verbose)
         fprintf(stderr, "[craftingworld] sweep clock, ms per sweep (median/90th percentile/mean of 20; 0.0 TB/s = unclocked):%s -> %s%.0f ns\n", log,
                 tn.period16 ? "" : "unclocked, ", tn.period16 / 1.6);
     return rc;
-}
-
-enum { CW_GUARD_EVERY = 64 };
-static hipEvent_t *sweep_guard_tick(cw_engine *e, hipStream_t st)
-{
-    if (++e->guard_step % CW_GUARD_EVERY) return nullptr;
-    while (e->guard_tail != e->guard_head && hipEventQuery(e->guard_ring[e->guard_tail % cw_engine::GUARD_RING].ev[5]) == hipSuccess) {
-        cw_engine::GuardSample &smp = e->guard_ring[e->guard_tail++ % cw_engine::GUARD_RING];
-        float ms = 0.f;
-        if (hipEventElapsedTime(&ms, smp.ev[4], smp.ev[5]) != hipSuccess || ms <= 0.f || smp.period16 != e->tune.period16) continue;
-        const double scheduled = cwh_guard_scheduled_ms(e->sweep_jobs, e->tune.period16, e->tune.period16_busy, e->sweep_beside_ms);
-        const double rate_before = e->guard.rate, prev_mean = e->guard.prev_mean;
-        const int recovering = e->guard.recovering;
-        const int action = cwh_guard_step(&e->guard, ms, scheduled);
-        if (e->guard.rate != rate_before) set_sweep_rate(e, e->guard.rate);
-        if (e->verbose && action != CWH_GUARD_NONE) {
-            static const char *what[] = {"", "three samples in a row late: a notch down", "trying a notch up", "the trial pays: kept", "the trial does not pay: undone"};
-            fprintf(stderr, "[craftingworld] sweep clock: %s%s -- %.4f ms against %.4f scheduled (mean at the rate left %.4f): %.1f -> %.1f TB/s (%.0f ns)\n", what[action],
-                    recovering ? " (on the way back to the best rate known)" : "", ms, scheduled, prev_mean, rate_before, e->guard.rate, e->tune.period16 / 1.6);
-        }
-    }
-    if (e->guard_head - e->guard_tail >= (unsigned)cw_engine::GUARD_RING) return nullptr;
-    cw_engine::GuardSample &slot = e->guard_ring[e->guard_head++ % cw_engine::GUARD_RING];
-    slot.period16 = e->tune.period16;
-    return slot.ev;
 }
 
 static void read_tuning(cw_engine *e)
@@ -448,7 +438,7 @@
     ALLOC_OUT(desired_out, N);
     ALLOC_OUT(episode_length, N);
     ALLOC_OUT(episode_return, N);
-    ALLOC(counters, 8);
+    ALLOC(counters, CW_CLOCK_WORD + (sizeof(cw_clock) + 7) / 8);
     if (rc == CW_OK) {
         int pr_least = 0, pr_greatest = 0;
         if (hipDeviceGetStreamPriorityRange(&pr_least, &pr_greatest) != hipSuccess) pr_least = pr_greatest = 0;
@@ -542,7 +532,6 @@
     if (e->aux) (void)hipStreamDestroy(e->aux);
     if (e->res_stream) (void)hipStreamDestroy(e->res_stream);
     if (e->last_work) (void)hipEventDestroy(e->last_work);
-    for (auto &smp : e->guard_ring) for (hipEvent_t ev : smp.ev) if (ev) (void)hipEventDestroy(ev);
     for (void *p : e->allocs) (void)hipFree(p);
     for (void *p : e->host_allocs) (void)hipHostFree(p);
     delete e;
@@ -728,7 +717,6 @@
     else if (e->n_work != 1 || e->work[0] != (hipStream_t)stream) note_work(e, (hipStream_t)stream);
     hipEvent_t *ev = (e->prof_n < e->prof_cap) ? &e->prof_ev[(size_t)e->prof_n * 6] : nullptr;
     const bool profiled = ev != nullptr;
-    if (e->guard_on && !ev && !capturing) ev = sweep_guard_tick(e, (hipStream_t)stream);
     if (capturing && e->P.lookahead && !e->la_refill_all && e->la_steps + 1 < e->la_period && !e->in_step_many) e->la_steps = e->la_period;
     if (e->P.lookahead && (e->la_refill_all || ++e->la_steps >= e->la_period)) {
         if (e->la_feedback && !capturing) la_adapt(e);
@@ -959,6 +947,15 @@
     return "cw_render_pieces_kernel";
 }
 
+static int read_clock_block(const cw_engine *e, cw_clock *c)
+{
+    DeviceGuard guard(e->device);
+    if (!guard.ok) return fail(CW_ERR_HIP, "hipSetDevice(%d) failed", e->device);
+    HIP_TRY(hipMemcpyAsync(c, clock_block(e), sizeof(*c), hipMemcpyDeviceToHost, e->aux));
+    HIP_TRY(hipStreamSynchronize(e->aux));
+    return CW_OK;
+}
+
 int cw_tuner(const cw_engine *e, cw_tuner_state *out)
 {
     if (!e || !out) return fail(CW_ERR_INVALID, "cw_tuner: null argument");
@@ -967,7 +964,35 @@
     out->period16_busy = e->tune.period16_busy;
     out->lookahead = e->P.lookahead;
     out->resident = e->res ? 1 : 0;
-    out->guard_slowdowns = e->guard_on ? e->guard.slowdowns : -1;
+    out->guard_slowdowns = -1;
+    if (e->guard_on) {
+        cw_clock c;
+        const int rc = read_clock_block(e, &c);
+        if (rc != CW_OK) return rc;
+        out->period16 = c.period16;
+        out->period16_head = c.period16_head;
+        out->period16_busy = c.period16_busy;
+        out->guard_slowdowns = c.g.slowdowns;
+    }
+    return CW_OK;
+}
+
+int cw_clock_state(const cw_engine *e, cw_clock_info *out)
+{
+    if (!e || !out) return fail(CW_ERR_INVALID, "cw_clock_state: null argument");
+    memset(out, 0, sizeof(*out));
+    if (!e->guard_on) return CW_OK;
+    cw_clock c;
+    const int rc = read_clock_block(e, &c);
+    if (rc != CW_OK) return rc;
+    out->guard_on = 1;
+    out->rate_milli = (int32_t)(c.g.rate * 1000.0 + 0.5);
+    out->rate_top_milli = (int32_t)(c.g.rate_top * 1000.0 + 0.5);
+    out->launches = c.launch;
+    out->samples = c.samples;
+    out->settle_left = c.g.settle_left;
+    out->probes = c.g.probes;
+    out->last_sweep_ticks = c.last_ticks;
     return CW_OK;
 }
 
diff --git a/gym_craftingworld_amd/csrc/cw_guard.h b/gym_craftingworld_amd/csrc/cw_guard.h
--- /dev/null
+++ b/gym_craftingworld_amd/csrc/cw_guard.h
@@ -0,0 +1,188 @@
+#pragma once
+#include <stdint.h>
+
+#if defined(__HIPCC__) || defined(__CUDACC__)
+#define CWG_HD __host__ __device__
+#else
+#define CWG_HD
+#endif
+
+typedef struct cwh_guard {
+    double rate;
+    double rate_top;
+    double ms_sum;
+    double prev_mean;
+    double ref_ms;
+    double ref_prev;
+    int32_t ms_n;
+    int32_t late;
+    int32_t good;
+    int32_t slowdowns;
+    int32_t probes;
+    int32_t probe_need;
+    int32_t recover_need;
+    int32_t probing;
+    int32_t recovering;
+    int32_t settle_left;
+    int32_t settle_samples;
+} cwh_guard;
+
+enum { CWH_GUARD_NONE = 0, CWH_GUARD_SLOWDOWN = 1, CWH_GUARD_TRIAL_UP = 2, CWH_GUARD_TRIAL_KEPT = 3, CWH_GUARD_TRIAL_UNDONE = 4 };
+#define CWH_GUARD_RECOVER 64
+#define CWH_GUARD_PROBE_SAMPLES 32
+#define CWH_GUARD_NEED_MAX 2048
+#define CWH_GUARD_RATE_FLOOR 5.0
+#define CWH_GUARD_RATE_CEILING 7.7
+#define CWH_GUARD_NOTCH 0.2
+#define CWH_GUARD_SETTLE_DIV 4
+#define CWH_GUARD_SETTLE_PROBE_SAMPLES 16
+#define CWH_GUARD_SETTLE_SAMPLES 128
+#define CW_CLOCK_STRIDE 61
+#define CW_CLOCK_SKIP 8
+#define CW_CLOCK_GAP_TICKS 5000
+#define CWH_HEAD_JOBS 64
+
+typedef struct cw_clock {
+    int32_t period16, period16_head, period16_busy;
+    int32_t sample_now;
+    unsigned long long t_min, t_max;
+    int32_t storm;
+    int32_t on;
+    int32_t stride, phase;
+    uint32_t launch;
+    uint32_t samples;
+    uint32_t last_ticks;
+    int32_t sweep_waves;
+    int32_t skip, pad;
+    double sweep_jobs, beside_ms, head_notch, busy_notch;
+    cwh_guard g;
+} cw_clock;
+
+#ifdef __cplusplus
+static CWG_HD inline double cwg_period_ns(int32_t sweep_waves, double tb_per_s) { return (double)sweep_waves * 4096.0 / (tb_per_s * 1e12) * 1e9; }
+static CWG_HD inline void cwg_sweep_periods(double rate, int32_t sweep_waves, double head_notch, double busy_notch, int32_t *period16, int32_t *period16_head,
+                                            int32_t *period16_busy)
+{
+    const double head = rate - head_notch > CWH_GUARD_RATE_FLOOR ? rate - head_notch : CWH_GUARD_RATE_FLOOR;
+    const double busy = rate - busy_notch > CWH_GUARD_RATE_FLOOR ? rate - busy_notch : CWH_GUARD_RATE_FLOOR;
+    *period16 = rate > 0 ? (int32_t)(cwg_period_ns(sweep_waves, rate) * 1.6 + 0.5) : 0;
+    *period16_head = rate > 0 ? (int32_t)(cwg_period_ns(sweep_waves, head) * 1.6 + 0.5) : 0;
+    *period16_busy = rate > 0 ? (int32_t)(cwg_period_ns(sweep_waves, busy) * 1.6 + 0.5) : 0;
+}
+static CWG_HD inline double cwg_scheduled_ms(double sweep_jobs, int32_t period16, int32_t period16_busy, double beside_ms)
+{
+    return (sweep_jobs * (period16 / 1.6) + CWH_HEAD_JOBS * ((period16_busy - period16) / 1.6)) * 1e-6 + beside_ms;
+}
+
+static CWG_HD inline void cwg_guard_set_rate(cwh_guard *g, double rate)
+{
+    g->rate = rate;
+    g->ms_sum = 0;
+    g->ms_n = 0;
+    g->good = g->late = 0;
+    g->ref_ms = 0;
+}
+static CWG_HD inline void cwg_guard_init(cwh_guard *g, double rate)
+{
+    cwh_guard z = {};
+    *g = z;
+    g->rate = g->rate_top = rate;
+    g->probe_need = CWH_GUARD_RECOVER;
+    g->recover_need = CWH_GUARD_RECOVER;
+}
+static CWG_HD inline void cwg_guard_settle(cwh_guard *g, int32_t samples) { g->settle_left = g->settle_samples = samples > 0 ? samples : 0; }
+static CWG_HD inline int cwg_guard_step(cwh_guard *g, double ms, double scheduled)
+{
+    const bool settling = g->settle_left > 0;
+    if (settling) g->settle_left--;
+    const int32_t trial_samples = settling ? CWH_GUARD_SETTLE_PROBE_SAMPLES : CWH_GUARD_PROBE_SAMPLES;
+    const double yard = g->probing ? g->prev_mean : g->ref_ms;
+    const double ref = scheduled > yard ? scheduled : yard;
+    const bool late = ms > (g->probing ? 1.15 : 1.06) * ref;
+    g->late = late ? g->late + 1 : 0;
+    g->good = late ? (g->good > 8 ? g->good - 8 : 0) : g->good + 1;
+    if (g->ms_n >= 128) { g->ms_sum *= 0.5; g->ms_n /= 2; }
+    g->ms_sum += ms;
+    g->ms_n++;
+    const bool verdict_due = g->probing && g->ms_n >= trial_samples;
+    const double mean = g->ms_sum / g->ms_n;
+    if (g->probing && (g->late >= 3 || (verdict_due && mean >= 0.998 * g->prev_mean))) {
+        const double ref_prev = g->ref_prev;
+        cwg_guard_set_rate(g, g->rate - CWH_GUARD_NOTCH);
+        g->ref_ms = ref_prev;
+        int32_t *need = g->recovering ? &g->recover_need : &g->probe_need;
+        *need = 2 * *need < CWH_GUARD_NEED_MAX ? 2 * *need : CWH_GUARD_NEED_MAX;
+        g->probing = g->recovering = 0;
+        return CWH_GUARD_TRIAL_UNDONE;
+    }
+    if (verdict_due) {
+        if (g->recovering && g->rate + 0.1 >= g->rate_top) g->settle_left = 0;
+        if (g->recovering) g->recover_need = CWH_GUARD_RECOVER;
+        else { g->rate_top = g->rate; g->probe_need = CWH_GUARD_RECOVER / 4; }
+        g->ref_ms = mean;
+        g->probing = g->recovering = 0;
+        return CWH_GUARD_TRIAL_KEPT;
+    }
+    if (!g->probing && g->late >= 3 && g->rate > CWH_GUARD_RATE_FLOOR + 0.1) {
+        cwg_guard_set_rate(g, g->rate - CWH_GUARD_NOTCH);
+        g->slowdowns++;
+        g->settle_left = g->settle_samples;
+        return CWH_GUARD_SLOWDOWN;
+    }
+    const int32_t need = g->rate + 0.1 < g->rate_top ? g->recover_need : g->probe_need;
+    if (!g->probing && g->ms_n >= trial_samples && g->rate + 0.05 < CWH_GUARD_RATE_CEILING && g->good >= (settling ? need / CWH_GUARD_SETTLE_DIV : need)) {
+        g->recovering = g->rate + 0.1 < g->rate_top;
+        g->prev_mean = mean;
+        g->ref_prev = g->ref_ms;
+        cwg_guard_set_rate(g, g->rate + CWH_GUARD_NOTCH < CWH_GUARD_RATE_CEILING ? g->rate + CWH_GUARD_NOTCH : CWH_GUARD_RATE_CEILING);
+        g->probing = 1;
+        if (!g->recovering) g->probes++;
+        return CWH_GUARD_TRIAL_UP;
+    }
+    if (settling && !g->probing && g->rate + 0.05 >= CWH_GUARD_RATE_CEILING && g->good >= CWH_GUARD_RECOVER / CWH_GUARD_SETTLE_DIV) g->settle_left = 0;
+    return CWH_GUARD_NONE;
+}
+
+static CWG_HD inline void cwg_clock_init(cw_clock *c, double rate, int32_t on, int32_t sweep_waves, double sweep_jobs, double beside_ms, double head_notch,
+                                         double busy_notch)
+{
+    cw_clock z = {};
+    *c = z;
+    c->on = on;
+    c->stride = CW_CLOCK_STRIDE;
+    c->sweep_waves = sweep_waves;
+    c->sweep_jobs = sweep_jobs;
+    c->beside_ms = beside_ms;
+    c->head_notch = head_notch;
+    c->busy_notch = busy_notch;
+    cwg_guard_init(&c->g, rate);
+    if (on) cwg_guard_settle(&c->g, CWH_GUARD_SETTLE_SAMPLES);
+    cwg_sweep_periods(rate, sweep_waves, head_notch, busy_notch, &c->period16, &c->period16_head, &c->period16_busy);
+    c->t_min = ~0ull;
+    c->skip = CW_CLOCK_SKIP;
+}
+static CWG_HD inline int cwg_clock_tick(cw_clock *c, unsigned long long now)
+{
+    if (!c->on) return -1;
+    int action = -1;
+    const unsigned long long t0 = c->t_min, t1 = c->t_max;
+    if (c->sample_now && !c->storm && t1 > t0) {
+        const unsigned long long ticks = t1 - t0;
+        c->last_ticks = ticks < 0xFFFFFFFFull ? (uint32_t)ticks : 0xFFFFFFFFu;
+        const double rate_before = c->g.rate;
+        action = cwg_guard_step(&c->g, (double)ticks * 1e-5, cwg_scheduled_ms(c->sweep_jobs, c->period16, c->period16_busy, c->beside_ms));
+        c->samples++;
+        if (c->g.rate != rate_before)
+            cwg_sweep_periods(c->g.rate, c->sweep_waves, c->head_notch, c->busy_notch, &c->period16, &c->period16_head, &c->period16_busy);
+    }
+    const bool settling = c->g.settle_left > 0;
+    if (settling && t1 != 0 && now > t1 + CW_CLOCK_GAP_TICKS) c->skip = CW_CLOCK_SKIP;
+    c->t_min = ~0ull;
+    c->t_max = 0;
+    c->storm = 0;
+    c->launch++;
+    c->sample_now = c->skip > 0 ? 0 : (settling || (int32_t)(c->launch % (uint32_t)c->stride) == c->phase);
+    if (c->skip > 0) c->skip--;
+    return action;
+}
+#endif
diff --git a/gym_craftingworld_amd/csrc/cw_host.cpp b/gym_craftingworld_amd/csrc/cw_host.cpp
--- a/gym_craftingworld_amd/csrc/cw_host.cpp
+++ b/gym_craftingworld_amd/csrc/cw_host.cpp
@@ -131,79 +131,23 @@
     return CWH_CKPT_SECTIONS;
 }
 
-static double period_ns(int32_t sweep_waves, double tb_per_s) { return (double)sweep_waves * 4096.0 / (tb_per_s * 1e12) * 1e9; }
 void cwh_sweep_periods(double rate, int32_t sweep_waves, double head_notch, double busy_notch, int32_t *period16, int32_t *period16_head, int32_t *period16_busy)
 {
-    const double head = rate - head_notch > CWH_GUARD_RATE_FLOOR ? rate - head_notch : CWH_GUARD_RATE_FLOOR;
-    const double busy = rate - busy_notch > CWH_GUARD_RATE_FLOOR ? rate - busy_notch : CWH_GUARD_RATE_FLOOR;
-    *period16 = rate > 0 ? (int32_t)(period_ns(sweep_waves, rate) * 1.6 + 0.5) : 0;
-    *period16_head = rate > 0 ? (int32_t)(period_ns(sweep_waves, head) * 1.6 + 0.5) : 0;
-    *period16_busy = rate > 0 ? (int32_t)(period_ns(sweep_waves, busy) * 1.6 + 0.5) : 0;
+    cwg_sweep_periods(rate, sweep_waves, head_notch, busy_notch, period16, period16_head, period16_busy);
 }
 double cwh_guard_scheduled_ms(double sweep_jobs, int32_t period16, int32_t period16_busy, double beside_ms)
 {
-    return (sweep_jobs * (period16 / 1.6) + CWH_HEAD_JOBS * ((period16_busy - period16) / 1.6)) * 1e-6 + beside_ms;
-}
-
-static void guard_set_rate(cwh_guard *g, double rate)
-{
-    g->rate = rate;
-    g->ms_sum = 0;
-    g->ms_n = 0;
-    g->good = g->late = 0;
-    g->ref_ms = 0;
-}
-void cwh_guard_init(cwh_guard *g, double rate)
-{
-    memset(g, 0, sizeof(*g));
-    g->rate = g->rate_top = rate;
-    g->probe_need = CWH_GUARD_RECOVER;
-    g->recover_need = CWH_GUARD_RECOVER;
-}
-int cwh_guard_step(cwh_guard *g, double ms, double scheduled)
-{
-    const double ref = std::max(scheduled, g->probing ? g->prev_mean : g->ref_ms);
-    const bool late = ms > (g->probing ? 1.15 : 1.06) * ref;
-    g->late = late ? g->late + 1 : 0;
-    g->good = late ? std::max(0, g->good - 8) : g->good + 1;
-    if (g->ms_n >= 128) { g->ms_sum *= 0.5; g->ms_n /= 2; }
-    g->ms_sum += ms;
-    g->ms_n++;
-    const bool verdict_due = g->probing && g->ms_n >= CWH_GUARD_PROBE_SAMPLES;
-    const double mean = g->ms_sum / g->ms_n;
-    if (g->probing && (g->late >= 3 || (verdict_due && mean >= 0.998 * g->prev_mean))) {
-        const double ref_prev = g->ref_prev;
-        guard_set_rate(g, g->rate - CWH_GUARD_NOTCH);
-        g->ref_ms = ref_prev;
-        int32_t &need = g->recovering ? g->recover_need : g->probe_need;
-        need = std::min(2 * need, (int32_t)CWH_GUARD_NEED_MAX);
-        g->probing = g->recovering = 0;
-        return CWH_GUARD_TRIAL_UNDONE;
-    }
-    if (verdict_due) {
-        if (g->recovering) g->recover_need = CWH_GUARD_RECOVER;
-        else { g->rate_top = g->rate; g->probe_need = CWH_GUARD_RECOVER / 4; }
-        g->ref_ms = mean;
-        g->probing = g->recovering = 0;
-        return CWH_GUARD_TRIAL_KEPT;
-    }
-    if (!g->probing && g->late >= 3 && g->rate > CWH_GUARD_RATE_FLOOR + 0.1) {
-        guard_set_rate(g, g->rate - CWH_GUARD_NOTCH);
-        g->slowdowns++;
-        return CWH_GUARD_SLOWDOWN;
-    }
-    if (!g->probing && g->ms_n >= CWH_GUARD_PROBE_SAMPLES && g->rate + 0.05 < CWH_GUARD_RATE_CEILING &&
-        g->good >= (g->rate + 0.1 < g->rate_top ? g->recover_need : g->probe_need)) {
-        g->recovering = g->rate + 0.1 < g->rate_top;
-        g->prev_mean = mean;
-        g->ref_prev = g->ref_ms;
-        guard_set_rate(g, std::min(g->rate + CWH_GUARD_NOTCH, CWH_GUARD_RATE_CEILING));
-        g->probing = 1;
-        if (!g->recovering) g->probes++;
-        return CWH_GUARD_TRIAL_UP;
-    }
-    return CWH_GUARD_NONE;
-}
+    return cwg_scheduled_ms(sweep_jobs, period16, period16_busy, beside_ms);
+}
+void cwh_guard_init(cwh_guard *g, double rate) { cwg_guard_init(g, rate); }
+void cwh_guard_settle(cwh_guard *g, int32_t samples) { cwg_guard_settle(g, samples); }
+int cwh_guard_step(cwh_guard *g, double ms, double scheduled) { return cwg_guard_step(g, ms, scheduled); }
+void cwh_clock_init(cw_clock *c, double rate, int32_t on, int32_t sweep_waves, double sweep_jobs, double beside_ms, double head_notch, double busy_notch)
+{
+    cwg_clock_init(c, rate, on, sweep_waves, sweep_jobs, beside_ms, head_notch, busy_notch);
+}
+int cwh_clock_tick(cw_clock *c, unsigned long long now) { return cwg_clock_tick(c, now); }
+size_t cwh_clock_bytes(void) { return sizeof(cw_clock); }
 
 int32_t cwh_la_adapt(int32_t period, int32_t period_max, uint64_t slow_delta, int32_t *quiet)
 {
diff --git a/gym_craftingworld_amd/csrc/cw_host.h b/gym_craftingworld_amd/csrc/cw_host.h
--- a/gym_craftingworld_amd/csrc/cw_host.h
+++ b/gym_craftingworld_amd/csrc/cw_host.h
@@ -1,6 +1,7 @@
 #pragma once
 #include <stddef.h>
 #include <stdint.h>
+#include "cw_guard.h"
 
 #define CWH_MT_N 624
 
@@ -21,37 +22,14 @@
 #define CWH_CKPT_SECTIONS 22
 int cwh_ckpt_section_bytes(int64_t n, int32_t k, int32_t la_depth, size_t *sizes, uint64_t *total);
 
-typedef struct cwh_guard {
-    double rate;
-    double rate_top;
-    double ms_sum;
-    double prev_mean;
-    double ref_ms;
-    double ref_prev;
-    int32_t ms_n;
-    int32_t late;
-    int32_t good;
-    int32_t slowdowns;
-    int32_t probes;
-    int32_t probe_need;
-    int32_t recover_need;
-    int32_t probing;
-    int32_t recovering;
-} cwh_guard;
-
-enum { CWH_GUARD_NONE = 0, CWH_GUARD_SLOWDOWN = 1, CWH_GUARD_TRIAL_UP = 2, CWH_GUARD_TRIAL_KEPT = 3, CWH_GUARD_TRIAL_UNDONE = 4 };
-#define CWH_GUARD_RECOVER 64
-#define CWH_GUARD_PROBE_SAMPLES 32
-#define CWH_GUARD_NEED_MAX 2048
-#define CWH_GUARD_RATE_FLOOR 5.0
-#define CWH_GUARD_RATE_CEILING 7.7
-#define CWH_GUARD_NOTCH 0.2
-
 void cwh_guard_init(cwh_guard *g, double rate);
+void cwh_guard_settle(cwh_guard *g, int32_t samples);
 int cwh_guard_step(cwh_guard *g, double ms, double scheduled_ms);
-#define CWH_HEAD_JOBS 64
 void cwh_sweep_periods(double rate, int32_t sweep_waves, double head_notch, double busy_notch, int32_t *period16, int32_t *period16_head, int32_t *period16_busy);
 double cwh_guard_scheduled_ms(double sweep_jobs, int32_t period16, int32_t period16_busy, double beside_ms);
+void cwh_clock_init(cw_clock *c, double rate, int32_t on, int32_t sweep_waves, double sweep_jobs, double beside_ms, double head_notch, double busy_notch);
+int cwh_clock_tick(cw_clock *c, unsigned long long now);
+size_t cwh_clock_bytes(void);
 
 #define CWH_LA_PERIOD_MIN 8
 #define CWH_LA_QUIET 8
diff --git a/gym_craftingworld_amd/csrc/cw_kernels.hip b/gym_craftingworld_amd/csrc/cw_kernels.hip
--- a/gym_craftingworld_amd/csrc/cw_kernels.hip
+++ b/gym_craftingworld_amd/csrc/cw_kernels.hip
@@ -3,8 +3,10 @@
 
 #include "cw_layout.h"
 #include "cw_mt.h"
+#include "cw_guard.h"
 
 #define CW_WAVE 64
+static __host__ __device__ inline cw_clock *cw_clock_of(const CwParams &P) { return (cw_clock *)(P.counters + CW_CLOCK_WORD); }
 #define CW_BALLOT(p) __builtin_amdgcn_ballot_w64(p)
 #define CW_ALT_FRAME_PACE 2
 
@@ -758,6 +760,10 @@
     const int lane = threadIdx.x & (CW_WAVE - 1);
     const int wave_in_block = __builtin_amdgcn_readfirstlane(threadIdx.x / CW_WAVE);
     const int n_waves = (int)gridDim.x * CW_RESET_WAVES;
+    if (blockIdx.x == 0 && threadIdx.x == 0) {
+        cw_clock *const c = cw_clock_of(P);
+        if (c->on) { c->g.settle_left = c->g.settle_samples; c->skip = CW_CLOCK_SKIP; }
+    }
     for (int env = (int)blockIdx.x * CW_RESET_WAVES + wave_in_block; env < P.n_envs; env += n_waves) {
         const uint4 v_h = P.hdr[env];
         const uint32_t menu_id = __builtin_amdgcn_readfirstlane(v_h.x) >> 24;
@@ -1248,6 +1254,12 @@
     __shared__ int s_njobs;
     __shared__ int s_cnt[3];
     const int wave_in_block = __builtin_amdgcn_readfirstlane(threadIdx.x / CW_WAVE);
+    if constexpr (PAINT == 2) {
+        if (blockIdx.x == gridDim.x - 1) {
+            if (threadIdx.x == 0) (void)cwg_clock_tick(cw_clock_of(P), __builtin_amdgcn_s_memrealtime());
+            return;
+        }
+    }
     fused_step<PAINT, TERM>(P, actions, act_dtype, epw, blockIdx.x * CW_RESET_WAVES + wave_in_block, s_mt[wave_in_block], s_jobs, &s_njobs, s_cnt);
 }
 typedef void (*CwStepFusedKernel)(CwParams, const void *, int, int);
@@ -1303,7 +1315,7 @@
     }
 }
 template <int RASTER, int FPJ>
-__device__ __forceinline__ void render_pieces(const CwParams &P, uint8_t *frames, int src, int period16, int head_extra16, int env_lo, int env_n)
+__device__ __forceinline__ unsigned long long render_pieces(const CwParams &P, uint8_t *frames, int src, int period16, int head_extra16, int env_lo, int env_n)
 {
     constexpr int JPB = CW_WAVE / FPJ;
     const int lane = threadIdx.x & (CW_WAVE - 1);
@@ -1315,7 +1327,7 @@
     uint8_t *const dst_base = frames + (size_t)env_lo * FB;
     const uint32_t total = (uint32_t)env_n * FB;
     const int n_jobs = (int)((total + CW_PIECE - 1u) / CW_PIECE);
-    if (wave >= n_jobs) return;
+    if (wave >= n_jobs) return ~0ull;
     const int q_mine = (n_jobs + n_waves - 1) / n_waves;
     const uint32_t half = (uint32_t)lane >> 5, pl = (uint32_t)lane & 31u;
     const uint32_t slot = RASTER == 1 ? (pl & 7u) : (pl >> 2), dy = pl & 3u;
@@ -1359,7 +1371,8 @@
         return r;
     };
     Rec nxt = fetch(0);
-    uint32_t t_next16 = ((uint32_t)__builtin_amdgcn_s_memrealtime() << 4) + (uint32_t)(((long long)wave * period16) / n_waves);
+    const unsigned long long t_entry = __builtin_amdgcn_s_memrealtime();
+    uint32_t t_next16 = ((uint32_t)t_entry << 4) + (uint32_t)(((long long)wave * period16) / n_waves);
     for (int base = 0; base < q_mine; base += JPB) {
         const Rec cur = nxt;
         if (base + JPB < q_mine) nxt = fetch(base + JPB);
@@ -1449,17 +1462,41 @@
             }
         }
     }
+    return t_entry;
 }
 template <int RASTER, int FPJ>
 __global__ __launch_bounds__(256) void cw_render_pieces_kernel(CwParams P, uint8_t *frames, int src, int period16, int period16_head, int period16_busy,
                                                                int chunk, int env_lo, int env_n)
 {
+    cw_clock *const clk = cw_clock_of(P);
+    bool stamp = (chunk & 8) != 0;
+    if (chunk & 4) {
+        const int4 c = *(const int4 *)clk;
+        period16 = c.x; period16_head = c.y; period16_busy = c.z;
+        stamp = c.w != 0;
+    }
     const unsigned long long done_now = P.counters[1];
     const unsigned long long finished = src == CW_SRC_CURRENT ? done_now - P.counters[4] : (unsigned long long)P.n_envs;
     const bool busy = finished >= CW_BUSY_FINISHED, storm = finished * 8ull >= (unsigned long long)P.n_envs;
-    render_pieces<RASTER, FPJ>(P, frames, src, __builtin_amdgcn_readfirstlane(storm ? period16_busy : period16),
+    const unsigned long long t_entry = render_pieces<RASTER, FPJ>(P, frames, src, __builtin_amdgcn_readfirstlane(storm ? period16_busy : period16),
                                __builtin_amdgcn_readfirstlane(!storm && (chunk & 1) ? (busy ? period16_busy : period16_head) - period16 : 0), env_lo, env_n);
-    if (src == CW_SRC_CURRENT && (chunk & 2) && blockIdx.x == 0 && threadIdx.x == 0) P.counters[4] = done_now;
+    if (src == CW_SRC_CURRENT && (chunk & 2) && blockIdx.x == 0 && threadIdx.x == 0) {
+        P.counters[4] = done_now;
+        if (chunk & 4) clk->storm = storm ? 1 : 0;
+    }
+    if (__builtin_amdgcn_readfirstlane((int)stamp)) {
+        __shared__ unsigned long long s_stamp[2][256 / CW_WAVE];
+        asm volatile("s_waitcnt vmcnt(0)" ::: "memory");
+        const unsigned long long t_exit = t_entry == ~0ull ? 0ull : __builtin_amdgcn_s_memrealtime();
+        const int w = __builtin_amdgcn_readfirstlane(threadIdx.x / CW_WAVE);
+        if ((threadIdx.x & (CW_WAVE - 1)) == 0) { s_stamp[0][w] = t_entry; s_stamp[1][w] = t_exit; }
+        __syncthreads();
+        if (threadIdx.x == 0) {
+            unsigned long long lo = s_stamp[0][0], hi = s_stamp[1][0];
+            for (int i = 1; i < 256 / CW_WAVE; i++) { lo = min(lo, s_stamp[0][i]); hi = max(hi, s_stamp[1][i]); }
+            if (hi) { atomicMin(&clk->t_min, lo); atomicMax(&clk->t_max, hi); }
+        }
+    }
 }
 #define CW_GATHER_MAX_S 9
 template <int NF>
@@ -1768,7 +1805,7 @@
     if (raster == 1) return fpj <= 2 ? cw_render_pieces_kernel<1, 2> : fpj <= 4 ? cw_render_pieces_kernel<1, 4> : fpj <= 8 ? cw_render_pieces_kernel<1, 8> : cw_render_pieces_kernel<1, 16>;
     return fpj <= 2 ? cw_render_pieces_kernel<0, 2> : fpj <= 4 ? cw_render_pieces_kernel<0, 4> : fpj <= 8 ? cw_render_pieces_kernel<0, 8> : cw_render_pieces_kernel<0, 16>;
 }
-static void cw_launch_sweep(const CwParams &P, const CwTuning &tn, uint8_t *frames, int src, hipStream_t st)
+static void cw_launch_sweep(const CwParams &P, const CwTuning &tn, uint8_t *frames, int src, hipStream_t st, int clock = 0)
 {
     int per = 0;
     const int n_chunks = cw_piece_chunks(P, tn, &per);
@@ -1784,7 +1821,7 @@
                 hipLaunchKernelGGL(cw_render_gather_kernel<8>, dim3(grid), dim3(256), 0, st, P, frames, src, tn.period16, c * per, env_n);
             continue;
         }
-        hipLaunchKernelGGL(k, dim3(cw_sweep_blocks(P, tn, pieces)), dim3(256), 0, st, P, frames, src, tn.period16, tn.period16_head, tn.period16_busy, (c == 0 ? 1 : 0) | (c == n_chunks - 1 ? 2 : 0), c * per, env_n);
+        hipLaunchKernelGGL(k, dim3(cw_sweep_blocks(P, tn, pieces)), dim3(256), 0, st, P, frames, src, tn.period16, tn.period16_head, tn.period16_busy, (c == 0 ? 1 : 0) | (c == n_chunks - 1 ? 2 : 0) | clock, c * per, env_n);
     }
 }
 
@@ -1817,14 +1854,14 @@
         const int epw = cw_envs_per_wave(n, tn.step_envs_per_wave);
         const int waves = (n + epw - 1) / epw;
         const int paint = obs_mode == 2 ? 1 : obs_mode == 1 ? 2 : 0;
-        hipLaunchKernelGGL(cw_step_fused_variant(paint, paint != 0 && P->terminal_img != nullptr), dim3(cw_wave_blocks(waves)), dim3(CW_RESET_WAVES * CW_WAVE),
-                           0, st, *P, actions, act_dtype, epw);
+        hipLaunchKernelGGL(cw_step_fused_variant(paint, paint != 0 && P->terminal_img != nullptr), dim3(cw_wave_blocks(waves) + (paint == 2 ? 1 : 0)),
+                           dim3(CW_RESET_WAVES * CW_WAVE), 0, st, *P, actions, act_dtype, epw);
     } else {
         hipLaunchKernelGGL(cw_step_kernel, dim3((n + 255) / 256), dim3(256), 0, st, *P, actions, act_dtype, obs_mode == 2 ? 1 : 0);
     }
     if (ev_all) (void)hipEventRecord(ev[1], st);
     if (ev) for (int k = 2; k < 5; k++) (void)hipEventRecord(ev[k], st);
-    if (obs_mode == 1) cw_launch_sweep(*P, tn, P->obs, CW_SRC_CURRENT, st);
+    if (obs_mode == 1) cw_launch_sweep(*P, tn, P->obs, CW_SRC_CURRENT, st, auto_reset && tn.guard ? 4 : 0);
     if (ev) (void)hipEventRecord(ev[5], st);
     return hipGetLastError();
 }
@@ -1939,7 +1976,7 @@
 
 hipError_t cwk_launch_sweep_calib(const CwParams *P, const CwTuning *T, hipStream_t st)
 {
-    cw_launch_sweep(*P, *T, P->obs, CW_SRC_CURRENT, st);
+    cw_launch_sweep(*P, *T, P->obs, CW_SRC_CURRENT, st, 8);
     return hipGetLastError();
 }
 
@@ -1950,6 +1987,22 @@
 hipError_t cwk_launch_idle(hipStream_t st)
 {
     hipLaunchKernelGGL(cw_idle_kernel, dim3(1), dim3(64), 0, st, 3);
+    return hipGetLastError();
+}
+
+__global__ void cw_stamps_collect_kernel(CwParams P, unsigned long long *out2)
+{
+    if (threadIdx.x == 0) {
+        cw_clock *const c = cw_clock_of(P);
+        if (out2) { out2[0] = c->t_min; out2[1] = c->t_max; }
+        c->t_min = ~0ull;
+        c->t_max = 0;
+    }
+    for (int i = 0; i < 3; i++) __builtin_amdgcn_s_sleep(127);
+}
+hipError_t cwk_launch_stamps_collect(const CwParams *P, unsigned long long *out2, hipStream_t st)
+{
+    hipLaunchKernelGGL(cw_stamps_collect_kernel, dim3(1), dim3(64), 0, st, *P, out2);
     return hipGetLastError();
 }
 
diff --git a/gym_craftingworld_amd/csrc/cw_layout.h b/gym_craftingworld_amd/csrc/cw_layout.h
--- a/gym_craftingworld_amd/csrc/cw_layout.h
+++ b/gym_craftingworld_amd/csrc/cw_layout.h
@@ -10,6 +10,7 @@
 
 #define CW_CODES_INITIAL 0x87654321u
 #define CW_CTL_QUEUED 0x100u
+#define CW_CLOCK_WORD 8
 #define CW_LA_DEPTH 4
 
 struct CwMenuDev {
@@ -32,6 +33,7 @@
     int small_blocks_per_cu = 4;
     long long small_launch_bytes = 320ll << 20;
     int step_envs_per_wave = 64;
+    int guard = 0;
     int reset_blocks_per_cu = 4;
 };
 
diff --git a/gym_craftingworld_amd/vec_env.py b/gym_craftingworld_amd/vec_env.py
--- a/gym_craftingworld_amd/vec_env.py
+++ b/gym_craftingworld_amd/vec_env.py
@@ -598,7 +598,12 @@
     def tuner_state(self):
         t = L.cw_tuner_state()
         L.check(self._lib.cw_tuner(self._h, C.byref(t)), 'cw_tuner', self._lib)
-        return {k: int(getattr(t, k)) for k, _ in t._fields_}
+        out = {k: int(getattr(t, k)) for k, _ in t._fields_}
+        c = L.cw_clock_info()
+        L.check(self._lib.cw_clock_state(self._h, C.byref(c)), 'cw_clock_state', self._lib)
+        out.update(guard_rate_milli=int(c.rate_milli), guard_rate_top_milli=int(c.rate_top_milli), guard_settle_left=int(c.settle_left), guard_probes=int(c.probes),
+                   clock_launches=int(c.launches), guard_samples=int(c.samples), last_sweep_ticks=int(c.last_sweep_ticks))
+        return out
 
     def compute_reward_batch(self, achieved_mask, desired_mask, subset=None):
         full = (1 << len(self.task_list)) - 1
diff --git a/include/craftingworld.h b/include/craftingworld.h
--- a/include/craftingworld.h
+++ b/include/craftingworld.h
@@ -158,6 +158,11 @@
     int32_t period16, period16_head, period16_busy, lookahead, resident, guard_slowdowns;
 } cw_tuner_state;
 int cw_tuner(const cw_engine *e, cw_tuner_state *out);
+typedef struct cw_clock_info {
+    int32_t guard_on, rate_milli, rate_top_milli, settle_left, probes;
+    uint32_t launches, samples, last_sweep_ticks;
+} cw_clock_info;
+int cw_clock_state(const cw_engine *e, cw_clock_info *out);
 
 int cw_buffers(cw_engine *e, cw_buffer_table *out);
 int cw_synchronize(cw_engine *e, cw_stream_t stream);
```

Result: no change. 318.1 million (-0.4%).
